# DerekGloudemans/3D-playground

Measured on AMD Instinct MI355X. Metric: training images/sec at 1920x1080, ResNet-50 3D-RetinaNet, higher is better.
Workload: dtype f32; 1 GPU; resnet50 directional 3D-RetinaNet, 1920x1080 synthetic frames, batch 8 per GPU, 10 GT boxes/image, fp32, fwd+loss+bwd+clip+Adam (BASELINE configs[1]); global_batch=8, parallelism=dp1

## Files before the change

3d-playground_amd/csrc/conv_wino.hip:

```cpp
#include "common.h"
#include "mfma_split.h"

__device__ __forceinline__ float4 f4(float s) { return make_float4(s, s, s, s); }
typedef float nt_f4 __attribute__((ext_vector_type(4)));
__device__ __forceinline__ float4 ld_stream(const float *p) {
    const nt_f4 v = __builtin_nontemporal_load(reinterpret_cast<const nt_f4 *>(p));
    return make_float4(v.x, v.y, v.z, v.w);
}
__device__ __forceinline__ void st_stream(float *p, float4 v) { *reinterpret_cast<float4 *>(p) = v; }
__device__ __forceinline__ float4 operator+(float4 a, float4 b) { return make_float4(a.x + b.x, a.y + b.y, a.z + b.z, a.w + b.w); }
__device__ __forceinline__ float4 operator-(float4 a, float4 b) { return make_float4(a.x - b.x, a.y - b.y, a.z - b.z, a.w - b.w); }
__device__ __forceinline__ float4 operator*(float s, float4 a) { return make_float4(s * a.x, s * a.y, s * a.z, s * a.w); }

__device__ __forceinline__ void bt6(const float4 d[6], float4 o[6]) {
    o[0] = 4.f * d[0] - 5.f * d[2] + d[4];
    o[1] = d[3] + d[4] - 4.f * (d[1] + d[2]);
    o[2] = 4.f * (d[1] - d[2]) - d[3] + d[4];
    o[3] = 2.f * (d[3] - d[1]) - d[2] + d[4];
    o[4] = 2.f * (d[1] - d[3]) - d[2] + d[4];
    o[5] = 4.f * d[1] - 5.f * d[3] + d[5];
}
__device__ __forceinline__ void at6(const float4 m[6], float4 o[4]) {
    const float4 s12 = m[1] + m[2], d12 = m[1] - m[2], s34 = m[3] + m[4], d34 = m[3] - m[4];
    o[0] = m[0] + s12 + s34;
    o[1] = d12 + 2.f * d34;
    o[2] = s12 + 4.f * s34;
    o[3] = d12 + 8.f * d34 + m[5];
}


struct WinoProblem { int N, H, W, TH, TW; };
struct WinoTable {
    int n;
    int64_t tile_end[RN_MAX_GROUP];
    WinoProblem p[RN_MAX_GROUP];
    const float *src[RN_MAX_GROUP];
    float *dst[RN_MAX_GROUP];
    const float *add[RN_MAX_GROUP];
    const float *mask[RN_MAX_GROUP];
    unsigned *sign[RN_MAX_GROUP];
    unsigned *amax[RN_MAX_GROUP];
};

#define WINO_GAIN_BT 7
#define WINO_GAIN_A 8
__device__ __forceinline__ void wino_tensor_word(const WinoTable &g, unsigned *tensor_amax, int gain) {
    if (tensor_amax == nullptr || blockIdx.x != 0 || threadIdx.x >= 64) return;
    int e = 0;
#pragma unroll
    for (int i = 0; i < RN_MAX_GROUP; ++i)
        if (i < g.n && g.amax[i] != nullptr) { const int ei = rn_amax_exp_all(g.amax[i], g.p[i].N); e = ei > e ? ei : e; }
    if (threadIdx.x == 0) atomicMax(tensor_amax, rn_amax_word_of_exp(e, gain));
}
__device__ __forceinline__ int wino_locate(const WinoTable &g, int64_t gt, int64_t &local) {
    int q = 0;
#pragma unroll
    for (int i = 0; i < RN_MAX_GROUP - 1; ++i) q += (i + 1 < g.n && gt >= g.tile_end[i]) ? 1 : 0;
    int64_t first = 0;
#pragma unroll
    for (int i = 1; i < RN_MAX_GROUP; ++i)
        if (q == i) first = g.tile_end[i - 1];
    local = gt - first;
    return q;
}

#define WINO_SELECT(q, g, pr, EXTRA)                          \
    WinoProblem pr = g.p[0];                                   \
    _Pragma("unroll") for (int i_ = 1; i_ < RN_MAX_GROUP; ++i_) \
        if (q == i_) { pr = g.p[i_]; EXTRA }

__global__ __launch_bounds__(256) void wino_in_kernel(const WinoTable g, float *__restrict__ V, int C, int64_t t0, int64_t Tpad,
                                                      unsigned *__restrict__ row_amax, unsigned *__restrict__ tensor_amax) {
    wino_tensor_word(g, tensor_amax, WINO_GAIN_BT);
    const int cq = C >> 2;
    const int64_t id = (int64_t)xcd_remap(blockIdx.x, gridDim.x) * 256 + threadIdx.x;
    const int64_t gt_raw = id / cq, t_last = g.tile_end[g.n - 1];
    const int64_t gt = gt_raw < t_last ? gt_raw : t_last - 1;
    const int c4 = (int)(id - gt_raw * cq) * 4;
    int64_t tile;
    const int q = wino_locate(g, gt, tile);
    const float *x = g.src[0];
    const unsigned *xw = g.amax[0];
    WINO_SELECT(q, g, pr, x = g.src[i_]; xw = g.amax[i_];)
    const int H = pr.H, W = pr.W, TW = pr.TW;
    const int n = (int)(tile / (pr.TH * TW));
    const int r = (int)(tile - (int64_t)n * pr.TH * TW);
    const int th = r / TW, tw = r - th * TW;
    const int h0 = 4 * th - 1, w0 = 4 * tw - 1;
    const float *xb = x + (int64_t)n * H * W * C + c4;
    if (row_amax != nullptr) {
        const int e_img = rn_amax_exp_lanes(xw != nullptr ? reinterpret_cast<const unsigned char *>(xw) + (int64_t)n * RN_AMAX_BYTES : nullptr);
        if (gt_raw < t_last && c4 == 0) row_amax[t0 + gt] = rn_amax_word_of_exp(e_img, WINO_GAIN_BT);
    }
    if (gt_raw >= t_last) return;
    float4 t[6][6];
#pragma unroll
    for (int j = 0; j < 6; ++j) {
        float4 d[6], o[6];
        const int w = w0 + j;
#pragma unroll
        for (int i = 0; i < 6; ++i) {
            const int h = h0 + i;
#ifdef RN_WINO_ABL
            const bool ok = (unsigned)h < (unsigned)H && (unsigned)w < (unsigned)W && i >= 1 && i <= 4 && j >= 1 && j <= 4;
#else
            const bool ok = (unsigned)h < (unsigned)H && (unsigned)w < (unsigned)W;
#endif
            d[i] = ok ? *reinterpret_cast<const float4 *>(xb + ((int64_t)h * W + w) * C) : f4(0.f);
        }
        bt6(d, o);
#pragma unroll
        for (int i = 0; i < 6; ++i) t[i][j] = o[i];
    }
    float *vb = V + (t0 + gt) * C + c4;
#pragma unroll
    for (int i = 0; i < 6; ++i) {
        float4 o[6];
        bt6(t[i], o);
#pragma unroll
        for (int j = 0; j < 6; ++j) st_stream(vb + (int64_t)(i * 6 + j) * Tpad * C, o[j]);
    }
}

template <bool PBITS, bool PADD, bool FLAGS = false>
__global__ __launch_bounds__(256, 2) void wino_out_kernel(const WinoTable g, const float *__restrict__ M, int Cout, int64_t t0,
                                                       int64_t Tpad, const float *__restrict__ scale,
                                                       const float *__restrict__ shift, int mask_mode, int act, int64_t y_bs,
                                                       const unsigned char *__restrict__ fin = nullptr,
                                                       unsigned char *__restrict__ fout = nullptr) {
    const int cq = Cout >> 2;
    const int64_t id = (int64_t)blockIdx.x * 256 + threadIdx.x;
    const int64_t gt = id / cq;
    float am = 0.f;
    unsigned *yam = nullptr;
    int n_img = 0;
    bool live = false;
    do {
    if (gt >= g.tile_end[g.n - 1]) break;
    live = true;
    const int c4 = (int)(id - gt * cq) * 4;
    int64_t tile;
    const int q = wino_locate(g, gt, tile);
    float *y = g.dst[0];
    const float *add = g.add[0], *mask = g.mask[0];
    unsigned *sign = g.sign[0];
    yam = g.amax[0];
    WINO_SELECT(q, g, pr, y = g.dst[i_]; add = g.add[i_]; mask = g.mask[i_]; sign = g.sign[i_]; yam = g.amax[i_];)
    n_img = (int)(tile / (pr.TH * pr.TW));
    const bool mbits = (mask_mode & RN_MASK_BITS) != 0;
    mask_mode &= 3;
    const int H = pr.H, W = pr.W, TW = pr.TW;
    const int n = (int)(tile / (pr.TH * TW));
    const int r = (int)(tile - (int64_t)n * pr.TH * TW);
    const int th = r / TW, tw = r - th * TW;
    const float *mb = M + (t0 + gt) * Cout + c4;
    float4 t[4][6];
    bool active = true;
    if constexpr (FLAGS) active = fin == nullptr || fin[t0 + gt] != 0;
    if (active) {
#pragma unroll
        for (int j = 0; j < 6; ++j) {
            float4 m[6], o[4];
#pragma unroll
            for (int i = 0; i < 6; ++i) m[i] = ld_stream(mb + (int64_t)(i * 6 + j) * Tpad * Cout);
            at6(m, o);
#pragma unroll
            for (int i = 0; i < 4; ++i) t[i][j] = o[i];
        }
    } else {
#pragma unroll
        for (int j = 0; j < 6; ++j)
#pragma unroll
            for (int i = 0; i < 4; ++i) t[i][j] = f4(0.f);
    }
    unsigned wake = 0u;
    float4 sc = f4(1.f), sh = f4(0.f);
    if (scale) sc = *reinterpret_cast<const float4 *>(scale + c4);
    if (shift) sh = *reinterpret_cast<const float4 *>(shift + c4);
    const int64_t ybs = y_bs ? y_bs : (int64_t)H * W * Cout;
#pragma unroll
    for (int i = 0; i < 4; ++i) {
        float4 o[4];
        at6(t[i], o);
        const int oh = 4 * th + i;
        if (oh >= H) break;
        unsigned mkw[4];
        float4 adv[4];
        if constexpr (PBITS || PADD) {
#pragma unroll
            for (int j = 0; j < 4; ++j) {
                const int owc = 4 * tw + j < W ? 4 * tw + j : W - 1;
                const int64_t off = (((int64_t)n * H + oh) * W + owc) * Cout + c4;
                if constexpr (PBITS) mkw[j] = reinterpret_cast<const unsigned *>(mask)[off >> 5] >> ((unsigned)off & 28u);
                if constexpr (PADD) adv[j] = *reinterpret_cast<const float4 *>(add + off);
            }
        }
#pragma unroll
        for (int j = 0; j < 4; ++j) {
            const int ow = 4 * tw + j;
            if (ow >= W) break;
            const int64_t off = (((int64_t)n * H + oh) * W + ow) * Cout + c4;
            const int64_t yoff = (int64_t)n * ybs + ((int64_t)oh * W + ow) * Cout + c4;
            float v[4] = {sc.x * o[j].x + sh.x, sc.y * o[j].y + sh.y, sc.z * o[j].z + sh.z, sc.w * o[j].w + sh.w};
            float mk[4] = {1.f, 1.f, 1.f, 1.f}, ad[4] = {0.f, 0.f, 0.f, 0.f};
            if constexpr (PBITS) {
                const unsigned nb = mkw[j];
                mk[0] = (nb & 1u) ? 1.f : 0.f; mk[1] = (nb & 2u) ? 1.f : 0.f; mk[2] = (nb & 4u) ? 1.f : 0.f; mk[3] = (nb & 8u) ? 1.f : 0.f;
            } else if (mask_mode != 0) { const float4 q4 = rn_mask_load4(mask, off, mbits); mk[0] = q4.x; mk[1] = q4.y; mk[2] = q4.z; mk[3] = q4.w; }
            if constexpr (PADD) { const float4 q4 = adv[j]; ad[0] = q4.x; ad[1] = q4.y; ad[2] = q4.z; ad[3] = q4.w; }
            else if (add) { const float4 q4 = *reinterpret_cast<const float4 *>(add + off); ad[0] = q4.x; ad[1] = q4.y; ad[2] = q4.z; ad[3] = q4.w; }
#pragma unroll
            for (int k = 0; k < 4; ++k) {
                float u = v[k];
                if (mask_mode == 1) u = mk[k] > 0.f ? u : 0.f;
                u += ad[k];
                if (act == 1) u = fmaxf(u, 0.f);
                else if (act == 2) u = 1.0f / (1.0f + expf(-u));
                if (mask_mode == 2) u = mk[k] > 0.f ? u : 0.f;
                v[k] = u;
            }
            *reinterpret_cast<float4 *>(y + yoff) = make_float4(v[0], v[1], v[2], v[3]);
            if (sign != nullptr) rn_sign_store(sign, off, v[0], v[1], v[2], v[3]);
            am = fmaxf(fmaxf(am, fmaxf(fabsf(v[0]), fabsf(v[1]))), fmaxf(fabsf(v[2]), fabsf(v[3])));
            if constexpr (FLAGS) {
                if (v[0] != 0.f || v[1] != 0.f || v[2] != 0.f || v[3] != 0.f) {
                    const unsigned rows = 2u | (i == 0 ? 1u : 0u) | (i == 3 ? 4u : 0u);
                    const unsigned cols = 2u | (j == 0 ? 1u : 0u) | (j == 3 ? 4u : 0u);
#pragma unroll
                    for (int a = 0; a < 3; ++a)
                        if (rows & (1u << a)) wake |= cols << (3 * a);
                }
            }
        }
    }
    if constexpr (FLAGS) {
        if (fout != nullptr && wake != 0u) {
#pragma unroll
            for (int a = 0; a < 3; ++a)
#pragma unroll
                for (int b = 0; b < 3; ++b) {
                    const int th2 = th + a - 1, tw2 = tw + b - 1;
                    if ((wake & (1u << (3 * a + b))) && (unsigned)th2 < (unsigned)pr.TH && (unsigned)tw2 < (unsigned)TW)
                        fout[t0 + gt + (int64_t)(a - 1) * TW + (b - 1)] = 1;
                }
        }
    }
    } while (0);
    if (live) rn_amax_note(yam, n_img, am);
}

__global__ void wino_weight_kernel(const float *__restrict__ w, float *__restrict__ U, int Cout, int Cin, int mode,
                                   const float *__restrict__ scale, int rows, int Kpad) {
    const int64_t id = (int64_t)blockIdx.x * 256 + threadIdx.x;
    if (id >= (int64_t)rows * Kpad) return;
    const int row = (int)(id / Kpad), k = (int)(id - (int64_t)row * Kpad);
    const int kdim = mode == 0 ? Cin : Cout;
    float g[3][3];
#pragma unroll
    for (int r = 0; r < 3; ++r)
#pragma unroll
        for (int s = 0; s < 3; ++s) {
            float v = 0.f;
            if (k < kdim) {
                if (mode == 0) v = w[(((int64_t)row * Cin + k) * 3 + r) * 3 + s];
                else v = w[(((int64_t)k * Cin + row) * 3 + (2 - r)) * 3 + (2 - s)] * (scale ? scale[k] : 1.f);
            }
            g[r][s] = v;
        }
    float t[6][3];
#pragma unroll
    for (int s = 0; s < 3; ++s) {
        const float a = g[0][s], b = g[1][s], c = g[2][s];
        t[0][s] = a * (1.f / 4.f);
        t[1][s] = -(a + b + c) * (1.f / 6.f);
        t[2][s] = (b - a - c) * (1.f / 6.f);
        t[3][s] = a * (1.f / 24.f) + b * (1.f / 12.f) + c * (1.f / 6.f);
        t[4][s] = a * (1.f / 24.f) - b * (1.f / 12.f) + c * (1.f / 6.f);
        t[5][s] = c;
    }
#pragma unroll
    for (int i = 0; i < 6; ++i) {
        const float a = t[i][0], b = t[i][1], c = t[i][2];
        const float o[6] = {a * (1.f / 4.f), -(a + b + c) * (1.f / 6.f), (b - a - c) * (1.f / 6.f),
                            a * (1.f / 24.f) + b * (1.f / 12.f) + c * (1.f / 6.f),
                            a * (1.f / 24.f) - b * (1.f / 12.f) + c * (1.f / 6.f), c};
#pragma unroll
        for (int j = 0; j < 6; ++j) U[((int64_t)(i * 6 + j) * rows + row) * Kpad + k] = o[j];
    }
}

__device__ __forceinline__ void a6(const float4 v[4], float4 o[6]) {
    const float4 s02 = v[0] + v[2], s13 = v[1] + v[3];
    o[0] = v[0];
// ... 96 lines not shown
            return;
        }
    }
    float4 t[6][6];
    float4 tz[6][4];
#pragma unroll
    for (int j = 0; j < 6; ++j) {
        float4 d[6], o[6];
        const int w = w0 + j;
#pragma unroll
        for (int i = 0; i < 6; ++i) {
            const int h = h0 + i;
            const bool ok = (unsigned)h < (unsigned)H && (unsigned)w < (unsigned)W;
            d[i] = ok ? *reinterpret_cast<const float4 *>(xb + ((int64_t)h * W + w) * C) : f4(0.f);
        }
        bt6(d, o);
#pragma unroll
        for (int i = 0; i < 6; ++i) t[i][j] = o[i];
        if (j >= 1 && j <= 4) {
            float4 oz[6];
            a6(d + 1, oz);
#pragma unroll
            for (int a = 0; a < 6; ++a) tz[a][j - 1] = oz[a];
        }
    }
    float *zb = Z + (t0 + gt) * C + c4;
#pragma unroll
    for (int a = 0; a < 6; ++a) {
        float4 o[6];
        a6(tz[a], o);
#pragma unroll
        for (int b = 0; b < 6; ++b) st_stream(zb + (int64_t)(a * 6 + b) * Tpad * C, o[b]);
    }
    float *vb = V + (t0 + gt) * C + c4;
#pragma unroll
    for (int i = 0; i < 6; ++i) {
        float4 o[6];
        bt6(t[i], o);
#pragma unroll
        for (int j = 0; j < 6; ++j) st_stream(vb + (int64_t)(i * 6 + j) * Tpad * C, o[j]);
    }
}

__device__ __forceinline__ unsigned nz_bytes(unsigned w) {
    const unsigned t = (w | ((w & 0x7f7f7f7fu) + 0x7f7f7f7fu)) & 0x80808080u;
    return ((t >> 7) & 1u) | ((t >> 14) & 2u) | ((t >> 21) & 4u) | ((t >> 28) & 8u);
}
__global__ __launch_bounds__(256) void tile_lists_kernel(const unsigned char *__restrict__ flags, int Tpad, int *__restrict__ counts,
                                                         int *__restrict__ tiles, int *__restrict__ units, int *__restrict__ blocks) {
    __shared__ unsigned long long wsum[4];
    const int tid = threadIdx.x, lane = tid & 63, wave = tid >> 6;
    const int nb = Tpad >> 7;
    unsigned m[8];
    unsigned long long c = 0ull;
#pragma unroll
    for (int j = 0; j < 8; ++j) m[j] = 0u;
    if (tid < nb) {
        const uint4 *p = reinterpret_cast<const uint4 *>(flags) + 8 * tid;
        int ct = 0, cu = 0;
#pragma unroll
        for (int j = 0; j < 8; ++j) {
            const uint4 v = p[j];
            m[j] = nz_bytes(v.x) | (nz_bytes(v.y) << 4) | (nz_bytes(v.z) << 8) | (nz_bytes(v.w) << 12);
            ct += __builtin_popcount(m[j]);
            cu += m[j] != 0u;
        }
        c = (unsigned long long)ct | ((unsigned long long)cu << 20) | ((unsigned long long)(cu != 0) << 40);
    }
    unsigned long long s = c;
#pragma unroll
    for (int off = 1; off < 64; off <<= 1) {
        const unsigned long long t = __shfl_up(s, off, 64);
        if (lane >= off) s += t;
    }
    if (lane == 63) wsum[wave] = s;
    __syncthreads();
    unsigned long long base = 0ull, total = 0ull;
#pragma unroll
    for (int w = 0; w < 4; ++w) { base += w < wave ? wsum[w] : 0ull; total += wsum[w]; }
    s = s - c + base;
    if (tid == 0) {
        counts[0] = (int)(total & 0xfffffu); counts[1] = (int)((total >> 20) & 0xfffffu); counts[2] = (int)((total >> 40) & 0xfffffu);
    }
    int ot = (int)(s & 0xfffffu), ou = (int)((s >> 20) & 0xfffffu);
    const int ob = (int)((s >> 40) & 0xfffffu);
    if ((c >> 40) != 0ull) blocks[ob] = tid;
#pragma unroll
    for (int j = 0; j < 8; ++j) {
        unsigned mm = m[j];
        if (mm != 0u) units[ou++] = 8 * tid + j;
        while (mm != 0u) {
            tiles[ot++] = 128 * tid + 16 * j + __builtin_ctz(mm);
            mm &= mm - 1u;
        }
    }
}

__global__ void wino_dw_kernel(const float *__restrict__ dU, float *__restrict__ dw, int Cout, int Cin, int Ku, int Kpad) {
    const int64_t id = (int64_t)blockIdx.x * 256 + threadIdx.x;
    if (id >= (int64_t)Cout * Cin) return;
    const int co = (int)(id / Cin), ci = (int)(id - (int64_t)co * Cin);
    const float *u = dU + (int64_t)co * Ku + ci;
    const int64_t ps = (int64_t)Cout * Ku;
    float t[3][6];
#pragma unroll
    for (int j = 0; j < 6; ++j) {
        float v[6];
#pragma unroll
        for (int i = 0; i < 6; ++i) v[i] = u[(i * 6 + j) * ps];
        t[0][j] = v[0] * (1.f / 4.f) - (v[1] + v[2]) * (1.f / 6.f) + (v[3] + v[4]) * (1.f / 24.f);
        t[1][j] = (v[2] - v[1]) * (1.f / 6.f) + (v[3] - v[4]) * (1.f / 12.f);
        t[2][j] = (v[3] + v[4] - v[1] - v[2]) * (1.f / 6.f) + v[5];
    }
    float *o = dw + (int64_t)co * Kpad + ci;
#pragma unroll
    for (int r = 0; r < 3; ++r) {
        const float *v = t[r];
        o[(r * 3 + 0) * Cin] += v[0] * (1.f / 4.f) - (v[1] + v[2]) * (1.f / 6.f) + (v[3] + v[4]) * (1.f / 24.f);
        o[(r * 3 + 1) * Cin] += (v[2] - v[1]) * (1.f / 6.f) + (v[3] - v[4]) * (1.f / 12.f);
        o[(r * 3 + 2) * Cin] += (v[3] + v[4] - v[1] - v[2]) * (1.f / 6.f) + v[5];
    }
}

static int wino_table(const rn_wino_group *g, WinoTable &t) {
    if (!g || g->n < 1 || g->n > RN_MAX_GROUP) return RN_EINVAL;
    t.n = g->n;
    int64_t end = 0;
    for (int i = 0; i < RN_MAX_GROUP; ++i) {
        const int k = i < g->n ? i : g->n - 1;
        if (g->N[k] <= 0 || g->H[k] <= 0 || g->W[k] <= 0) return RN_EINVAL;
        t.p[i].N = g->N[k]; t.p[i].H = g->H[k]; t.p[i].W = g->W[k];
        t.p[i].TH = (g->H[k] + 3) / 4; t.p[i].TW = (g->W[k] + 3) / 4;
        if (i < g->n) end += (int64_t)g->N[k] * t.p[i].TH * t.p[i].TW;
        t.tile_end[i] = end;
        t.src[i] = g->src[k]; t.dst[i] = g->dst[k]; t.add[i] = g->add[k]; t.mask[i] = g->mask[k];
        t.sign[i] = reinterpret_cast<unsigned *>(g->sign[k]);
        t.amax[i] = reinterpret_cast<unsigned *>(g->amax[k]);
    }
    return RN_OK;
}

extern "C" int rn_wino_input_group(const rn_wino_group *g, float *V, int C, int64_t tile_offset, int64_t Tpad, int dy_form,
                                   void *row_amax, void *tensor_amax, void *stream) {
    WinoTable t;
    const int rc = wino_table(g, t);
    if (rc) return rc;
    if (C <= 0 || (C & 3) || tile_offset < 0 || tile_offset + t.tile_end[t.n - 1] > Tpad) return RN_EINVAL;
    for (int i = 0; i < t.n; ++i)
        if (!t.src[i]) return RN_EINVAL;
    const dim3 grid(rn_blocks(t.tile_end[t.n - 1] * (C >> 2), 256));
    if (dy_form && row_amax != nullptr) return RN_EINVAL;
    if (dy_form) hipLaunchKernelGGL(wino_dy_kernel, grid, dim3(256), 0, (hipStream_t)stream, t, V, C, tile_offset, Tpad,
                                    reinterpret_cast<unsigned *>(tensor_amax));
    else hipLaunchKernelGGL(wino_in_kernel, grid, dim3(256), 0, (hipStream_t)stream, t, V, C, tile_offset, Tpad,
                            reinterpret_cast<unsigned *>(row_amax), reinterpret_cast<unsigned *>(tensor_amax));
    RN_LAUNCH_CHECK();
    return RN_OK;
}

extern "C" int rn_wino_input_both_group_flags(const rn_wino_group *g, float *V, float *Z, int C, int64_t tile_offset, int64_t Tpad,
                                              void *v_row_amax, void *z_tensor_amax, const void *flags, void *stream) {
    WinoTable t;
    const int rc = wino_table(g, t);
    if (rc) return rc;
    if (!V || !Z || C <= 0 || (C & 3) || tile_offset < 0 || tile_offset + t.tile_end[t.n - 1] > Tpad) return RN_EINVAL;
    if (flags != nullptr && (((uintptr_t)flags & 15) || (Tpad & 15))) return RN_EINVAL;
    for (int i = 0; i < t.n; ++i)
        if (!t.src[i]) return RN_EINVAL;
    const dim3 grid(rn_blocks(t.tile_end[t.n - 1] * (C >> 2), 256));
    if (flags != nullptr)
        hipLaunchKernelGGL(wino_in_both_kernel<true>, grid, dim3(256), 0, (hipStream_t)stream, t, V, Z, C, tile_offset, Tpad,
                           reinterpret_cast<unsigned *>(v_row_amax), reinterpret_cast<unsigned *>(z_tensor_amax),
                           reinterpret_cast<const unsigned char *>(flags));
    else
        hipLaunchKernelGGL(wino_in_both_kernel<false>, grid, dim3(256), 0, (hipStream_t)stream, t, V, Z, C, tile_offset, Tpad,
                           reinterpret_cast<unsigned *>(v_row_amax), reinterpret_cast<unsigned *>(z_tensor_amax),
                           (const unsigned char *)nullptr);
    RN_LAUNCH_CHECK();
    return RN_OK;
}
extern "C" int rn_tile_lists(const void *flags, int64_t Tpad, void *counts, void *tiles, void *units, void *blocks, void *stream) {
    if (!flags || !counts || !tiles || !units || !blocks || Tpad <= 0 || (Tpad & 255) || Tpad > 256 * 128) return RN_EINVAL;
    if (((uintptr_t)flags & 15) || (((uintptr_t)counts | (uintptr_t)tiles | (uintptr_t)units | (uintptr_t)blocks) & 3)) return RN_EINVAL;
    hipLaunchKernelGGL(tile_lists_kernel, dim3(1), dim3(256), 0, (hipStream_t)stream, reinterpret_cast<const unsigned char *>(flags), (int)Tpad,
                       reinterpret_cast<int *>(counts), reinterpret_cast<int *>(tiles), reinterpret_cast<int *>(units),
                       reinterpret_cast<int *>(blocks));
    RN_LAUNCH_CHECK();
    return RN_OK;
}

extern "C" int rn_wino_input_both_group_lists(const rn_wino_group *g, float *V, float *Z, int C, int64_t tile_offset, int64_t Tpad,
                                              void *v_row_amax, void *z_tensor_amax, const void *flags, const void *units,
                                              const void *n_units, void *stream) {
    WinoTable t;
    const int rc = wino_table(g, t);
    if (rc) return rc;
    if (!V || !Z || C <= 0 || (C & 3) || tile_offset < 0 || tile_offset + t.tile_end[t.n - 1] > Tpad) return RN_EINVAL;
    if (!flags || !units || !n_units || ((uintptr_t)flags & 15) || ((uintptr_t)units & 3) || (Tpad & 15)) return RN_EINVAL;
    for (int i = 0; i < t.n; ++i)
        if (!t.src[i]) return RN_EINVAL;
    const dim3 gl(rn_blocks(t.tile_end[t.n - 1] * (C >> 2), 256));
    hipLaunchKernelGGL((wino_in_both_kernel<true, true>), gl, dim3(256), 0, (hipStream_t)stream, t, V, Z, C, tile_offset, Tpad,
                       reinterpret_cast<unsigned *>(v_row_amax), reinterpret_cast<unsigned *>(z_tensor_amax),
                       reinterpret_cast<const unsigned char *>(flags), reinterpret_cast<const int *>(units),
                       reinterpret_cast<const int *>(n_units));
    RN_LAUNCH_CHECK();
    return RN_OK;
}

extern "C" int rn_wino_input_both_group(const rn_wino_group *g, float *V, float *Z, int C, int64_t tile_offset, int64_t Tpad,
                                        void *v_row_amax, void *z_tensor_amax, void *stream) {
    return rn_wino_input_both_group_flags(g, V, Z, C, tile_offset, Tpad, v_row_amax, z_tensor_amax, nullptr, stream);
}

extern "C" int rn_wino_output_group_flags(const rn_wino_group *g, const float *M, int Cout, int64_t tile_offset, int64_t Tpad,
                                          const float *scale, const float *shift, int mask_mode, int act, int64_t y_batch_stride,
                                          const void *flags_in, void *flags_out, void *stream) {
    WinoTable t;
    const int rc = wino_table(g, t);
    if (rc) return rc;
    if (Cout <= 0 || (Cout & 3) || tile_offset < 0 || tile_offset + t.tile_end[t.n - 1] > Tpad) return RN_EINVAL;
    if (mask_mode < 0 || (mask_mode & ~(3 | RN_MASK_BITS)) || (mask_mode & 3) == 3 || mask_mode == RN_MASK_BITS) return RN_EINVAL;
    if (act < 0 || act > 2 || y_batch_stride < 0 || (y_batch_stride & 3)) return RN_EINVAL;
    for (int i = 0; i < t.n; ++i) {
        if (!t.dst[i] || (mask_mode != 0) != (t.mask[i] != nullptr)) return RN_EINVAL;
        if (((mask_mode & RN_MASK_BITS) || t.sign[i]) && (Cout & 31)) return RN_EINVAL;
        if (y_batch_stride && y_batch_stride < (int64_t)t.p[i].H * t.p[i].W * Cout) return RN_EINVAL;
    }
    const bool pbits = (mask_mode & RN_MASK_BITS) != 0;
    bool padd = true;
    for (int i = 0; i < t.n; ++i) padd = padd && t.add[i] != nullptr;
    const dim3 grid(rn_blocks(t.tile_end[t.n - 1] * (Cout >> 2), 256));
    const unsigned char *fin = reinterpret_cast<const unsigned char *>(flags_in);
    unsigned char *fout = reinterpret_cast<unsigned char *>(flags_out);
#define RN_WINO_OUT(B, A, F) hipLaunchKernelGGL((wino_out_kernel<B, A, F>), grid, dim3(256), 0, (hipStream_t)stream, t, M, Cout, tile_offset, Tpad, \
                                                scale, shift, mask_mode, act, y_batch_stride, fin, fout)
    if (fin != nullptr || fout != nullptr) {
        if (pbits && padd) RN_WINO_OUT(true, true, true);
        else if (pbits) RN_WINO_OUT(true, false, true);
        else if (padd) RN_WINO_OUT(false, true, true);
        else RN_WINO_OUT(false, false, true);
    } else if (pbits && padd) RN_WINO_OUT(true, true, false);
    else if (pbits) RN_WINO_OUT(true, false, false);
    else if (padd) RN_WINO_OUT(false, true, false);
    else RN_WINO_OUT(false, false, false);
#undef RN_WINO_OUT
    RN_LAUNCH_CHECK();
    return RN_OK;
}
extern "C" int rn_wino_output_group(const rn_wino_group *g, const float *M, int Cout, int64_t tile_offset, int64_t Tpad,
                                    const float *scale, const float *shift, int mask_mode, int act, int64_t y_batch_stride,
                                    void *stream) {
    return rn_wino_output_group_flags(g, M, Cout, tile_offset, Tpad, scale, shift, mask_mode, act, y_batch_stride, nullptr, nullptr, stream);
}

static rn_wino_group wino_single(const float *src, float *dst, const float *add, const float *mask, int N, int H, int W) {
    rn_wino_group g = {};
    g.n = 1; g.N[0] = N; g.H[0] = H; g.W[0] = W; g.src[0] = src; g.dst[0] = dst; g.add[0] = add; g.mask[0] = mask;
    return g;
}
extern "C" int rn_wino_input(const float *x, float *V, int N, int H, int W, int C, int64_t tile_offset, int64_t Tpad,
                             void *stream) {
    const rn_wino_group g = wino_single(x, nullptr, nullptr, nullptr, N, H, W);
    return rn_wino_input_group(&g, V, C, tile_offset, Tpad, 0, nullptr, nullptr, stream);
}
extern "C" int rn_wino_dy(const float *dy, float *Z, int N, int H, int W, int C, int64_t tile_offset, int64_t Tpad, void *stream) {
    const rn_wino_group g = wino_single(dy, nullptr, nullptr, nullptr, N, H, W);
    return rn_wino_input_group(&g, Z, C, tile_offset, Tpad, 1, nullptr, nullptr, stream);
}
extern "C" int rn_wino_output(const float *M, float *y, int N, int H, int W, int Cout, int64_t tile_offset, int64_t Tpad,
                              const float *scale, const float *shift, const float *add, const float *mask, int mask_mode,
                              int act, int64_t y_batch_stride, void *stream) {
    const rn_wino_group g = wino_single(nullptr, y, add, mask, N, H, W);
    return rn_wino_output_group(&g, M, Cout, tile_offset, Tpad, scale, shift, mask_mode, act, y_batch_stride, stream);
}

extern "C" int rn_wino_weights(const float *w, float *U, int Cout, int Cin, int mode, const float *scale, void *stream) {
    if (Cout <= 0 || Cin <= 0 || mode < 0 || mode > 1) return RN_EINVAL;
    const int rows = mode == 0 ? Cout : Cin;
    const int Kpad = ((mode == 0 ? Cin : Cout) + 31) / 32 * 32;
    hipLaunchKernelGGL(wino_weight_kernel, dim3(rn_blocks((int64_t)rows * Kpad, 256)), dim3(256), 0, (hipStream_t)stream, w, U,
                       Cout, Cin, mode, scale, rows, Kpad);
    RN_LAUNCH_CHECK();
    return RN_OK;
}

extern "C" int rn_wino_dw(const float *dU, float *dw, int Cout, int Cin, void *stream) {
    if (Cout <= 0 || Cin <= 0) return RN_EINVAL;
    const int Ku = (Cin + 31) / 32 * 32, Kpad = (9 * Cin + 31) / 32 * 32;
    hipLaunchKernelGGL(wino_dw_kernel, dim3(rn_blocks((int64_t)Cout * Cin, 256)), dim3(256), 0, (hipStream_t)stream, dU, dw, Cout,
                       Cin, Ku, Kpad);
    RN_LAUNCH_CHECK();
    return RN_OK;
}
```

3d-playground_amd/csrc/focal_loss.hip:

```cpp
#include <math.h>
#include <stdlib.h>

#include "common.h"

#ifndef FOCAL_NTHR
#define FOCAL_NTHR 256
#endif
#define NTHR FOCAL_NTHR
#define APT 4
#define TILE (NTHR * APT)
#define NWAVES (NTHR / 64)
#define UAPT 2
#define UNIT (64 * UAPT)
#define QCAP 256
#ifndef RN_FOCAL_WAVES_PER_SIMD
#define RN_FOCAL_WAVES_PER_SIMD 4
#endif
#define RN_FOCAL_WAVES_NOTE 4
#define RN_FOCAL_RESIDENT 768

static inline int focal_resident() {
    static const int v = [] { const char *e = getenv("RN_FOCAL_RESIDENT"); const int x = e ? atoi(e) : 0; return x >= 8 ? x : RN_FOCAL_RESIDENT; }();
    return v;
}
// ... 664 lines not shown
            un = u + stride;
            issue(un < units ? un : u, avA, xvA);
            process(u, avB, xvB);
            u = un;
            if (u >= units || qn > QCAP - UNIT) break;
        }
        drain();
    }
    if (!BWD) {
        sums[0] += (-0.75f * RN_LN2) * (neg2.x + neg2.y);
        block_sum4<NWAVES>(sums, s_red);
        if (threadIdx.x == 0) {
            unsigned long long *p64 = reinterpret_cast<unsigned long long *>(partials) + 2 * ((int64_t)j * G + g);
            const unsigned long long lo = ((unsigned long long)__float_as_uint(sums[1]) << 32) | __float_as_uint(sums[0]);
            const unsigned long long hi = ((unsigned long long)__float_as_uint(sums[3]) << 32) | __float_as_uint(sums[2]);
            (void)__hip_atomic_exchange(p64, lo, __ATOMIC_RELAXED, __HIP_MEMORY_SCOPE_AGENT);
            (void)__hip_atomic_exchange(p64 + 1, hi, __ATOMIC_RELAXED, __HIP_MEMORY_SCOPE_AGENT);
            asm volatile("s_waitcnt vmcnt(0)" ::: "memory");
            s_last = atomicAdd(counter + RN_WS_HEAD / 4 + j, 1u) == (unsigned)G - 1;
        }
        __syncthreads();
        if (s_last) {
            double *s_red = reinterpret_cast<double *>(&s_q[0][0][0]);
            const int B = (int)(gridDim.x / G);
            focal_finalize_image<DIR>(reinterpret_cast<const float4 *>(partials), G, j, ann, N, terms, s_red);
            if (threadIdx.x == 0) {
                __hip_atomic_store(counter + RN_WS_HEAD / 4 + j, 0u, __ATOMIC_RELAXED, __HIP_MEMORY_SCOPE_AGENT);
                s_last = atomicAdd(counter, 1u) == (unsigned)B - 1;
            }
            __syncthreads();
            if (s_last) {
                focal_finalize_batch<DIR>(B, terms, stats, losses, s_red, s_red + NWAVES * 4);
                if (threadIdx.x == 0) __hip_atomic_store(counter, 0u, __ATOMIC_RELAXED, __HIP_MEMORY_SCOPE_AGENT);
            }
        }
    }
}

static int check_args(int B, int64_t A, int C, int N) {
    if (B <= 0 || A <= 0 || C <= 0 || N < 0) return RN_EINVAL;
    if (N > RN_MAX_GT) return RN_ETOOMANY;
    if (B > 1024) return RN_EINVAL;
    if (A > 0x7fffffffLL) return RN_EINVAL;
    return RN_OK;
}

struct FocalWs {
    unsigned *counter;
    ImageStats *stats;
    double *terms;
    float *partials;
};
static inline FocalWs focal_ws(void *workspace, int B) {
    char *w = reinterpret_cast<char *>(workspace);
    FocalWs r;
    r.counter = reinterpret_cast<unsigned *>(w);
    const size_t head = RN_WS_HEAD + (size_t)focal_counter_bytes(B);
    r.stats = reinterpret_cast<ImageStats *>(w + head);
    r.terms = reinterpret_cast<double *>(w + head + (size_t)B * sizeof(ImageStats));
    r.partials = reinterpret_cast<float *>(w + head + (size_t)B * sizeof(ImageStats) + (size_t)B * RN_TERMS * sizeof(double));
    return r;
}

extern "C" int rn_focal_loss_fwd(const float *cls, const float *reg, const float *anchors, const float *ann, int B,
                                 int64_t A, int C, int N, int directional, void *workspace, float *losses,
                                 void *stream) {
    const int rc = check_args(B, A, C, N);
    if (rc) return rc;
    hipStream_t s = (hipStream_t)stream;
    const int G = focal_groups(B, A);
    const int units = (int)((A + UNIT - 1) / UNIT);
    const FocalWs ws = focal_ws(workspace, B);
    const dim3 grid((unsigned)(B * G)), block(NTHR);
    const float4 *anc = reinterpret_cast<const float4 *>(anchors);
    const int cq = C == 4 ? 1 : (C == 8 ? 2 : 0);
    const size_t raw_bytes = (size_t)(N > 0 ? N : 1) * (directional ? 27 : 5) * sizeof(float);
#define RN_FOCAL_FWD(DIR_, CQ_)                                                                                        \
    hipLaunchKernelGGL((focal_kernel<DIR_, false, CQ_>), grid, block, raw_bytes, s, cls, reg, anc, ann, A, C, N,        \
                       ws.partials, ws.stats, (float *)nullptr, (float *)nullptr, G, units, ws.counter, ws.terms, losses, \
                       (const float *)nullptr)
    if (directional) {
        if (cq == 2) RN_FOCAL_FWD(true, 2); else if (cq == 1) RN_FOCAL_FWD(true, 1); else RN_FOCAL_FWD(true, 0);
    } else {
        if (cq == 2) RN_FOCAL_FWD(false, 2); else if (cq == 1) RN_FOCAL_FWD(false, 1); else RN_FOCAL_FWD(false, 0);
    }
#undef RN_FOCAL_FWD
    RN_LAUNCH_CHECK();
    return RN_OK;
}

extern "C" int rn_focal_loss_bwd(const float *cls, const float *reg, const float *anchors, const float *ann, int B,
                                 int64_t A, int C, int N, int directional, const void *workspace,
                                 const float *grad_losses, float *dcls, float *dreg, void *stream) {
    const int rc = check_args(B, A, C, N);
    if (rc) return rc;
    hipStream_t s = (hipStream_t)stream;
    const int G = focal_groups(B, A);
    const int units = (int)((A + UNIT - 1) / UNIT);
    const FocalWs ws = focal_ws(const_cast<void *>(workspace), B);
    const dim3 grid((unsigned)(B * G)), block(NTHR);
    const float4 *anc = reinterpret_cast<const float4 *>(anchors);
    const int cq = C == 4 ? 1 : (C == 8 ? 2 : 0);
    const size_t raw_bytes = (size_t)(N > 0 ? N : 1) * (directional ? 27 : 5) * sizeof(float);
#define RN_FOCAL_BWD(DIR_, CQ_)                                                                                      \
    hipLaunchKernelGGL((focal_kernel<DIR_, true, CQ_>), grid, block, raw_bytes, s, cls, reg, anc, ann, A, C, N,       \
                       (float *)nullptr, ws.stats, dcls, dreg, G, units, (unsigned *)nullptr, (double *)nullptr,      \
                       (float *)nullptr, grad_losses)
    if (directional) {
        if (cq == 2) RN_FOCAL_BWD(true, 2); else if (cq == 1) RN_FOCAL_BWD(true, 1); else RN_FOCAL_BWD(true, 0);
    } else {
        if (cq == 2) RN_FOCAL_BWD(false, 2); else if (cq == 1) RN_FOCAL_BWD(false, 1); else RN_FOCAL_BWD(false, 0);
    }
#undef RN_FOCAL_BWD
    RN_LAUNCH_CHECK();
    return RN_OK;
}

template <bool DIR>
__global__ __launch_bounds__(NTHR) void assign_kernel(const float4 *__restrict__ anchors, const float *__restrict__ ann,
                                                      int64_t A, int N, float *__restrict__ iou_max,
                                                      int32_t *__restrict__ argmax, int32_t *__restrict__ state) {
    constexpr int COLS = DIR ? 27 : 5;
    __shared__ LabelLds L;
    const int j = blockIdx.y;
    load_labels<DIR>(ann + (int64_t)j * N * COLS, N, L);
    const int64_t ai = (int64_t)blockIdx.x * NTHR + threadIdx.x;
    if (ai >= A) return;
    float best = 0.f; int arg = -1; int st = 0;
    if (L.count > 0) {
        match_anchor(anchors[ai], L, best, arg);
        st = -1;
        if (best < 0.4f) st = 0;
        if (best >= 0.5f) st = 1;
    }
    iou_max[(int64_t)j * A + ai] = best;
    argmax[(int64_t)j * A + ai] = arg;
    state[(int64_t)j * A + ai] = st;
}

extern "C" int rn_assign(const float *anchors, const float *ann, int B, int64_t A, int N, int directional,
                         float *iou_max, int32_t *argmax, int32_t *state, void *stream) {
    const int rc = check_args(B, A, 1, N);
    if (rc) return rc;
    const dim3 grid((unsigned)((A + NTHR - 1) / NTHR), B), block(NTHR);
    const float4 *anc = reinterpret_cast<const float4 *>(anchors);
    if (directional)
        hipLaunchKernelGGL(assign_kernel<true>, grid, block, 0, (hipStream_t)stream, anc, ann, A, N, iou_max, argmax, state);
    else
        hipLaunchKernelGGL(assign_kernel<false>, grid, block, 0, (hipStream_t)stream, anc, ann, A, N, iou_max, argmax, state);
    RN_LAUNCH_CHECK();
    return RN_OK;
}

__global__ void pairwise_iou_kernel(const float4 *__restrict__ a, const float4 *__restrict__ b, float *__restrict__ out,
                                    int64_t A, int N) {
    const int64_t i = (int64_t)blockIdx.x * 256 + threadIdx.x;
    if (i >= A * N) return;
    const int64_t ai = i / N;
    const int n = (int)(i - ai * N);
    const float4 p = a[ai], q = b[n];
    const float area_b = (q.z - q.x) * (q.w - q.y);
    float iw = fminf(p.z, q.z) - fmaxf(p.x, q.x);
    float ih = fminf(p.w, q.w) - fmaxf(p.y, q.y);
    iw = fmaxf(iw, 0.f);
    ih = fmaxf(ih, 0.f);
    float ua = ((p.z - p.x) * (p.w - p.y) + area_b) - iw * ih;
    ua = fmaxf(ua, 1e-8f);
    out[i] = (iw * ih) / ua;
}

extern "C" int rn_pairwise_iou(const float *a, const float *b, float *iou, int64_t A, int N, void *stream) {
    if (A <= 0 || N <= 0) return RN_EINVAL;
    hipLaunchKernelGGL(pairwise_iou_kernel, dim3(rn_blocks(A * N, 256)), dim3(256), 0, (hipStream_t)stream,
                       reinterpret_cast<const float4 *>(a), reinterpret_cast<const float4 *>(b), iou, A, N);
    RN_LAUNCH_CHECK();
    return RN_OK;
}
```

3d-playground_amd/retinanet_mi355x/_hip.py:

```python
import ctypes
import os

import torch

_HERE = os.path.dirname(os.path.abspath(__file__))
LIB_PATH = os.environ.get("RN_LIB_PATH") or os.path.join(_HERE, "lib", "libretinanet_mi355x.so")
_lib = None

c_i32, c_i64, c_f32, c_f64, c_vp = ctypes.c_int, ctypes.c_int64, ctypes.c_float, ctypes.c_double, ctypes.c_void_p

SIGNATURES = {
    "rn_version": (ctypes.c_char_p, []),
    "rn_check_device": (c_i32, []),
    "rn_get_fp32_mfma": (c_i32, []),
    "rn_set_fp32_mfma": (c_i32, [c_i32]),
    "rn_get_option": (c_i32, [c_i32]),
    "rn_set_option": (c_i32, [c_i32, c_i32]),
    "rn_fp32_split_min_k": (c_i32, []),
    "rn_split_weights": (c_i32, [c_vp, c_vp, c_i64, c_i32, c_vp]),
    "rn_split_weights_f16": (c_i32, [c_vp, c_vp, c_vp, c_i64, c_i32, c_vp]),
    "rn_amax": (c_i32, [c_vp, c_i64, c_i32, c_vp, c_vp]),
    "rn_stream_capture_id": (c_i32, [c_vp, ctypes.POINTER(ctypes.c_ulonglong)]),
    "rn_anchor_count": (c_i64, [c_i32, c_i32]),
    "rn_anchor_base_boxes": (None, [c_vp]),
# ... 16 lines not shown
    "rn_space_to_state": (c_i32, [c_vp, c_vp, c_i64, c_vp]),
    "rn_state_to_im": (c_i32, [c_vp, c_vp, c_vp, c_vp, c_vp, c_i64, c_vp]),
    "rn_space_to_im": (c_i32, [c_vp, c_vp, c_vp, c_vp, c_vp, c_i64, c_vp]),
    "rn_im_to_space": (c_i32, [c_vp, c_vp, c_vp, c_vp, c_vp, c_vp, c_i64, c_vp]),
    "rn_im_to_state": (c_i32, [c_vp, c_vp, c_vp, c_vp, c_vp, c_vp, c_i64, c_vp]),
    "rn_parse_workspace_bytes": (c_i64, [c_i64]),
    "rn_parse_detections": (c_i32, [c_vp, c_vp, c_vp, c_vp, c_i64, c_vp, c_vp, c_vp, c_vp, c_i32, c_vp, c_f32, c_f32, c_f32,
                                    c_i32, c_i32, c_vp, c_vp, c_vp, c_vp, c_vp, c_vp, c_vp]),
    "rn_md_iou": (c_i32, [c_vp, c_vp, c_vp, c_i64, c_vp]),
    "rn_crop_boxes": (c_i32, [c_vp, c_vp, c_i32, c_f64, c_vp, c_vp, c_vp]),
    "rn_roi_align": (c_i32, [c_vp, c_i32, c_i32, c_i32, c_i32, c_vp, c_i32, c_i32, c_i32, c_vp, c_i32, c_vp]),
    "rn_crop_select": (c_i32, [c_vp] * 9 + [c_i32] * 4 + [c_f64, c_i32, c_f32, c_vp, c_vp, c_vp, c_vp]),
    "rn_kf_view": (c_i32, [c_vp, c_vp, c_vp, c_vp, c_i32, c_i32, c_vp, c_i32, c_vp]),
    "rn_kf_predict": (c_i32, [c_vp, c_vp, c_vp, c_vp, c_vp, c_vp, c_vp, c_i32, c_f64, c_i32, c_vp]),
    "rn_kf_update": (c_i32, [c_vp, c_vp, c_vp, c_vp, c_vp, c_vp, c_vp, c_i32, c_vp]),
    "rn_track_cost": (c_i32, [c_vp, c_i64, c_vp, c_i64, c_i64, c_i64, c_vp, c_vp]),
    "rn_lsap_workspace_bytes": (c_i64, [c_i64, c_i64]),
    "rn_linear_sum_assignment": (c_i32, [c_vp, c_i64, c_i64, c_f64, c_vp, c_vp, c_vp, c_vp, c_vp]),
    "rn_ts_bias_workspace_bytes": (c_i64, [c_i64, c_i64]),
    "rn_estimate_ts_bias": (c_i32, [c_vp, c_i64, c_vp, c_i64, c_vp, c_vp, c_i64, c_i64, c_vp, c_vp, c_i32, c_f64, c_f64, c_f32,
                                    c_vp, c_i64, c_vp, c_vp, c_vp, c_vp]),
    "rn_track_crop_prior": (c_i32, [c_vp] * 7 + [c_i32, c_vp, c_vp, c_vp, c_i32, c_vp]),
    "rn_fit_nearest": (c_i32, [c_vp, c_vp, c_vp, c_i64, c_i64, c_vp, c_vp, c_vp, c_vp]),
    "rn_residual_moments": (c_i32, [c_vp, c_i64, c_i32, c_vp, c_i32, c_vp, c_vp, c_vp, c_vp]),
    "rn_eval_select": (c_i32, [c_vp, c_vp, c_vp, c_i64, c_i64, c_i64, c_f32, c_i32, c_i32, c_i64, c_i32, c_vp, c_i64, c_vp, c_vp, c_vp]),
    "rn_eval_match": (c_i32, [c_vp, c_i64, c_vp, c_i64, c_i32, c_vp, c_vp, c_i64, c_f64, c_vp, c_vp, c_vp, c_vp]),
    "rn_eval_ap_workspace_bytes": (c_i64, [c_i64]),
    "rn_eval_ap": (c_i32, [c_vp, c_i64, c_vp, c_vp, c_vp, c_i32, c_vp, c_vp, c_vp, c_vp]),
    "rn_eval_corners": (c_i32, [c_vp, c_i64, c_i64, c_i32, c_i64, c_vp, c_vp, c_i64, c_vp, c_vp]),
    "rn_eval_cuboid_overlap": (c_i32, [c_vp, c_i64, c_vp, c_i64, c_i32, c_vp, c_vp, c_vp, c_i64, c_i32, c_vp, c_vp, c_vp]),
    "rn_eval_cuboid_assign": (c_i32, [c_vp, c_i64, c_vp, c_i64, c_i32, c_vp, c_i64, c_vp, c_vp, c_vp, c_i32, c_vp, c_vp, c_vp,
                                      c_vp, c_vp]),
    "rn_eval_cuboid_errors": (c_i32, [c_vp, c_i64, c_vp, c_i64, c_i32, c_vp, c_vp, c_vp, c_i64, c_vp, c_vp, c_vp, c_vp, c_vp,
                                      c_vp]),
    "rn_frame_ingest": (c_i32, [c_vp, c_i32, c_i32, c_i32, c_i32] + [c_f32] * 6 + [c_i32, c_vp, c_vp]),
    "rn_frame_ingest_half": (c_i32, [c_vp, c_i32, c_i32, c_i32, c_i32] + [c_f32] * 6 + [c_i32, c_vp, c_vp, c_vp]),
    "rn_parse_frame_timestamps": (c_i32, [c_vp, c_i32, c_i32, c_i32, c_i64, c_i64, c_i32, c_vp, c_i32] + [c_vp] * 9),
    "rn_augment_workspace_bytes": (c_i64, [c_i32, c_i32, c_i32]),
    "rn_augment_frames": (c_i32, [c_vp, c_i32, c_i32, c_i32, c_vp, c_vp, c_vp, c_vp, ctypes.c_uint64] + [c_f32] * 6 + [c_vp, c_vp, c_vp]),
    "rn_augment_crops_workspace_bytes": (c_i64, [c_i32, c_i32, c_i32]),
    "rn_augment_crops": (c_i32, [c_vp, c_i32, c_i32, c_i32, c_vp, c_vp, c_vp, c_vp, c_vp, c_i32, c_i32, c_i32, c_vp, c_vp, ctypes.c_uint64]
                         + [c_f32] * 6 + [c_vp, c_vp, c_vp]),
    "rn_mot_prepare": (c_i32, [c_vp, c_vp, c_vp, c_i64, c_vp, c_i64] + [c_vp] * 7),
    "rn_mot_iou": (c_i32, [c_vp] * 5 + [c_i64, c_i64, c_vp, c_vp]),
    "rn_mot_assign": (c_i32, [c_vp] * 5 + [c_i64] * 4 + [c_vp] * 5),
    "rn_mot_frame_metrics": (c_i32, [c_vp] * 5 + [c_i64, c_i64, c_vp, c_vp, c_vp, c_f64] + [c_vp] * 19),
    "rn_mot_workspace_bytes": (c_i64, [c_i64, c_i64]),
    "rn_mot_reduce": (c_i32, [c_i64, c_i64] + [c_vp] * 16 + [c_i64, c_i64, c_vp, c_vp, c_vp]),
    "rn_mot_assoc_workspace_bytes": (c_i64, [c_i64, c_i64]),
    "rn_mot_id_counts": (c_i32, [c_vp] * 5 + [c_i64] * 6 + [c_vp, c_vp, c_i64, c_i64, c_f64] + [c_vp] * 5),
    "rn_mot_id_assign": (c_i32, [c_vp, c_i64, c_i64, c_vp, c_vp, c_vp, c_vp]),
    "rn_mot_hota_align": (c_i32, [c_vp] * 5 + [c_i64] * 6 + [c_vp] * 5 + [c_i64] * 3 + [c_vp] * 5),
    "rn_mot_hota_assign": (c_i32, [c_vp] * 5 + [c_i64] * 6 + [c_vp, c_vp, c_i64, c_i64] + [c_vp] * 11),
    "rn_mot_hota_reduce": (c_i32, [c_vp] * 4 + [c_i64] * 6 + [c_vp] * 9 + [c_i64, c_i64, c_vp, c_vp, c_vp]),
    "rn_vanishing_points": (c_i32, [c_vp, c_i64, c_vp, c_i64, c_vp, c_vp, c_vp, c_vp]),
    "rn_hg_reproj_error": (c_i32, [c_vp, c_vp, c_vp, c_vp, c_vp, c_i64, c_i64, c_vp, c_vp]),
    "rn_hg_scale_z": (c_i32, [c_vp, c_vp, c_vp, c_vp, c_i64, c_f64, c_f64, c_i32, c_vp, c_vp, c_vp, c_vp]),
    "rn_fit_homography": (c_i32, [c_vp, c_vp, c_i64, c_vp, c_i64, c_i32, c_vp, c_vp, c_vp]),
    "rn_reinterp_mate": (c_i32, [c_vp, c_vp, c_i64, c_i64, c_vp, c_vp, c_vp]),
    "rn_reinterp_offsets": (c_i32, [c_vp, c_vp, c_i64, c_i64, c_vp, c_i64] + [c_vp] * 5),
    "rn_reinterp_rows": (c_i32, [c_vp] * 7 + [c_i64] * 4 + [c_vp] * 5),
    "rn_track_rows": (c_i32, [c_vp] * 5 + [c_i64, c_i64] + [c_vp] * 7),
    "rn_render_edges": (c_i32, [c_vp, c_vp, c_i64, c_i32, c_i32, c_vp, c_i32, c_i32, c_i32, c_vp]),
    "rn_render_rects": (c_i32, [c_vp, c_i64, c_vp, c_i64, c_vp, c_i32, c_i32, c_i32, c_vp]),
    "rn_render_text": (c_i32, [c_vp, c_i64, c_vp, c_i64, c_vp, c_vp, c_i64, c_vp, c_i32, c_i32, c_i32, c_vp]),
    "rn_render_compose": (c_i32, [c_vp] + [c_f32] * 6 + [c_vp, c_i32, c_vp, c_i32, c_i32, c_i32, c_i32, c_vp]),
    "rn_replay_boxes": (c_i32, [c_vp, c_i64, c_vp, c_vp, c_vp, c_i32, c_vp, c_vp, c_vp, c_vp, c_vp]),
    "rn_replay_compose": (c_i32, [c_vp, c_i32, c_vp, c_vp] + [c_i32] * 6 + [c_vp]),
    "rn_frame_absdiff": (c_i32, [c_vp, c_vp] + [c_i32] * 6 + [c_vp, c_vp, c_vp]),
    "rn_running_frame": (c_i32, [c_vp, c_vp, c_i64, c_i32, c_vp]),
    "rn_label_pair_samples": (c_i32, [c_vp, c_vp, c_i64, c_i32, c_i64, c_i32, c_i32, c_i32, c_vp, c_vp, c_vp, c_vp]),
    "rn_label_outliers": (c_i32, [c_vp, c_vp, c_vp, c_i64, c_i64, c_i64, c_i64, c_vp, c_vp, c_vp]),
    "rn_label_interpolate_workspace_bytes": (c_i64, [c_i64, c_i64]),
    "rn_label_interpolate": (c_i32, [c_vp] * 4 + [c_i64] * 3 + [c_i32, c_i64] + [c_vp] * 7),
    "rn_label_rebase": (c_i32, [c_vp, c_vp, c_i64] + [c_vp] * 4 + [c_i32, c_vp, c_i32, c_i32] + [c_vp] * 5),
    "rn_label_offset_y": (c_i32, [c_vp] * 4 + [c_i64, c_i32, c_vp, c_vp]),
    "rn_label_crop_windows": (c_i32, [c_vp, c_vp, c_i64, c_vp, c_vp, c_i32, c_f32, c_f32, c_f32] + [c_vp] * 6),
    "rn_label_best_anchor": (c_i32, [c_vp, c_vp, c_vp, c_i64, c_i32, c_i32, c_f32] + [c_vp] * 5),
    "rn_label_fit_box2d": (c_i32, [c_vp] * 5 + [c_i64, c_vp, c_vp, c_i32, c_vp, c_i32, c_i32] + [c_vp] * 5),
    "rn_spline_fit_workspace_bytes": (c_i64, [c_i64, c_i32]),
    "rn_label_box_weights": (c_i32, [c_vp, c_vp, c_i64, c_vp, c_vp, c_i32, c_vp, c_vp, c_vp]),
    "rn_spline_fit": (c_i32, [c_vp, c_i64, c_vp, c_i64, c_vp, c_vp, c_vp, c_i64, c_vp, c_i64, c_i32] + [c_vp] * 7),
    "rn_spline_select": (c_i32, [c_vp, c_i64] + [c_vp] * 4 + [c_i64, c_i64, c_i64, c_i32] + [c_vp] * 4 + [c_i32] + [c_vp] * 7),
    "rn_spline_eval": (c_i32, [c_vp, c_vp, c_vp, c_i64, c_i32, c_vp, c_vp, c_i64, c_vp, c_vp]),
    "rn_label_ts_shift": (c_i32, [c_vp, c_vp, c_vp, c_i64, c_i32, c_vp, c_vp, c_vp, c_i64, c_i64, c_vp, c_vp, c_vp, c_i32, c_i32,
                                  c_i32] + [c_vp] * 5),
    "rn_label_series_workspace_bytes": (c_i64, [c_i64]),
    "rn_label_series": (c_i32, [c_vp, c_vp, c_i64, c_i32, c_i64, c_i32, c_f64, c_f64, c_i32] + [c_vp] * 8),
    "rn_label_group_rmse": (c_i32, [c_vp, c_vp, c_i64, c_i64] + [c_vp] * 5),
    "rn_stitch_endpoints": (c_i32, [c_vp, c_vp, c_vp, c_i64, c_i64, c_i32, c_vp, c_vp, c_vp]),
    "rn_stitch_costs": (c_i32, [c_vp, c_i64] + [c_f64] * 7 + [c_vp, c_vp]),
    "rn_stitch_candidates": (c_i32, [c_vp, c_i64] + [c_f64] * 7 + [c_vp] * 4),
    "rn_stitch_compact": (c_i32, [c_vp, c_i64] + [c_f64] * 7 + [c_vp, c_vp, c_i64, c_vp, c_vp, c_vp]),
    "rn_stitch_assign_workspace_bytes": (c_i64, [c_i64]),
    "rn_stitch_assign": (c_i32, [c_vp, c_i64] + [c_f64] * 7 + [c_vp, c_vp, c_vp, c_i64] + [c_vp] * 6),
    "rn_stitch_chains": (c_i32, [c_vp, c_vp, c_i64] + [c_vp] * 6),
    "rn_stitch_fill_count": (c_i32, [c_vp, c_vp, c_i64, c_f64] + [c_vp] * 4),
    "rn_stitch_fill_rows": (c_i32, [c_vp, c_vp, c_vp, c_i64, c_i64, c_f64] + [c_vp] * 6),
    "rn_smooth_filter": (c_i32, [c_vp] * 5 + [c_f64, c_f64, c_i64, c_i64] + [c_vp] * 5),
    "rn_smooth_rts": (c_i32, [c_vp] * 5 + [c_f64, c_i64, c_i64] + [c_vp] * 4),
}

class ConvDesc(ctypes.Structure):
    _fields_ = [("N", c_i32), ("Hi", c_i32), ("Wi", c_i32), ("Cin", c_i32),
                ("Ho", c_i32), ("Wo", c_i32), ("Cout", c_i32),
                ("kh", c_i32), ("kw", c_i32),
                ("a", c_i32), ("b", c_i32), ("p", c_i32), ("p_w", c_i32), ("div_shift", c_i32),
                ("act", c_i32), ("add_mode", c_i32), ("Ha", c_i32), ("Wa", c_i32),
                ("mask_mode", c_i32), ("in_relu", c_i32),
                ("os", c_i32), ("oo_h", c_i32), ("oo_w", c_i32), ("Hy", c_i32), ("Wy", c_i32),
                ("add2_mode", c_i32), ("Ha2", c_i32), ("Wa2", c_i32), ("add2_batch_stride", c_i64),
                ("x_batch_stride", c_i64), ("y_batch_stride", c_i64), ("add_batch_stride", c_i64),
                ("w_batch_stride", c_i64), ("w_format", c_i32), ("sign_out", c_vp),
                ("x_amax", c_vp), ("y_amax", c_vp), ("w_unscale", c_vp), ("x_amax_img_stride", c_i32), ("x_amax_row_stride", c_i32),
                ("row_active", c_vp), ("row_list", c_vp), ("row_list_n", c_vp), ("row_list_grid", c_i32)]


RN_MAX_GROUP = 5


class ConvGroup(ctypes.Structure):
    _fields_ = [("n", c_i32), ("tile_end", c_i32 * RN_MAX_GROUP), ("d", ConvDesc * RN_MAX_GROUP),
                ("x", c_vp * RN_MAX_GROUP), ("y", c_vp * RN_MAX_GROUP), ("add", c_vp * RN_MAX_GROUP),
                ("mask", c_vp * RN_MAX_GROUP)]


class PrepJob(ctypes.Structure):
    _fields_ = [("kind", c_i32)] + [(n, c_i32) for n in ("Cout", "Cin", "kh", "kw", "kw_pad", "c_pad", "mode", "r0", "nr", "s0",
                                                          "ns", "rows", "Kpad")] + \
               [("eps", c_f32), ("src", c_vp), ("dst", c_vp), ("scale", c_vp), ("gamma", c_vp), ("beta", c_vp), ("mean", c_vp),
                ("var", c_vp), ("bn_scale", c_vp), ("bn_shift", c_vp), ("bn_rstd", c_vp)]


class UnpackJob(ctypes.Structure):
    _fields_ = [("dw", c_vp), ("w_packed", c_vp), ("dweight", c_vp)] + \
               [(n, c_i32) for n in ("Cout", "Cin", "kh", "kw", "kw_pad", "c_pad", "Kpad")] + \
               [("scale", c_vp), ("mean", c_vp), ("rstd", c_vp), ("colsum", c_vp), ("dgamma", c_vp), ("dbeta", c_vp)]


class WinoGroup(ctypes.Structure):
    _fields_ = [("n", c_i32), ("N", c_i32 * RN_MAX_GROUP), ("H", c_i32 * RN_MAX_GROUP), ("W", c_i32 * RN_MAX_GROUP),
                ("src", c_vp * RN_MAX_GROUP), ("dst", c_vp * RN_MAX_GROUP), ("add", c_vp * RN_MAX_GROUP),
                ("mask", c_vp * RN_MAX_GROUP), ("sign", c_vp * RN_MAX_GROUP), ("amax", c_vp * RN_MAX_GROUP)]


SIGNATURES.update({
    "rn_unpack_batched": (c_i32, [c_vp, c_vp, c_i32, c_vp]),
    "rn_prep_batched": (c_i32, [c_vp, c_vp, c_i32, c_vp]),
    "rn_wino_input_group": (c_i32, [ctypes.POINTER(WinoGroup), c_vp, c_i32, c_i64, c_i64, c_i32, c_vp, c_vp, c_vp]),
    "rn_wino_input_both_group": (c_i32, [ctypes.POINTER(WinoGroup), c_vp, c_vp, c_i32, c_i64, c_i64, c_vp, c_vp, c_vp]),
    "rn_wino_input_both_group_flags": (c_i32, [ctypes.POINTER(WinoGroup), c_vp, c_vp, c_i32, c_i64, c_i64, c_vp, c_vp, c_vp, c_vp]),
    "rn_tile_lists": (c_i32, [c_vp, c_i64, c_vp, c_vp, c_vp, c_vp, c_vp]),
    "rn_wino_input_both_group_lists": (c_i32, [ctypes.POINTER(WinoGroup), c_vp, c_vp, c_i32, c_i64, c_i64, c_vp, c_vp, c_vp, c_vp, c_vp, c_vp]),
    "rn_wino_output_group_flags": (c_i32, [ctypes.POINTER(WinoGroup), c_vp, c_i32, c_i64, c_i64, c_vp, c_vp, c_i32, c_i32, c_i64, c_vp, c_vp, c_vp]),
    "rn_wino_output_group": (c_i32, [ctypes.POINTER(WinoGroup), c_vp, c_i32, c_i64, c_i64, c_vp, c_vp, c_i32, c_i32, c_i64, c_vp]),
    "rn_conv_igemm_grouped": (c_i32, [ctypes.POINTER(ConvGroup), c_vp, c_vp, c_vp, c_vp]),
    "rn_conv_igemm": (c_i32, [ctypes.POINTER(ConvDesc), c_vp, c_vp, c_vp, c_vp, c_vp, c_vp, c_vp, c_vp, c_vp]),
    "rn_conv_splitk_workspace_bytes": (c_i64, [ctypes.POINTER(ConvDesc)]),
    "rn_conv_igemm_wants_f16": (c_i32, [ctypes.POINTER(ConvDesc)]),
    "rn_conv_igemm_splitk": (c_i32, [ctypes.POINTER(ConvDesc)] + [c_vp] * 10),
    "rn_conv_wgrad": (c_i32, [c_vp, c_i32, c_vp, c_vp, c_vp] + [c_i32] * 12 + [c_vp]),
    "rn_pack_weights": (c_i32, [c_vp, c_vp] + [c_i32] * 7 + [c_vp] + [c_i32] * 4 + [c_vp]),
    "rn_unpack_wgrad": (c_i32, [c_vp, c_vp, c_vp] + [c_i32] * 6 + [c_vp] * 7),
    "rn_bn_fold": (c_i32, [c_vp, c_vp, c_vp, c_vp, c_f32, c_i32, c_vp, c_vp, c_vp, c_vp]),
    "rn_nchw_to_nhwc4": (c_i32, [c_vp, c_vp, c_i32, c_i32, c_i32, c_vp, c_vp]),
    "rn_maxpool_fwd": (c_i32, [c_vp, c_vp, c_vp] + [c_i32] * 6 + [c_vp]),
    "rn_maxpool_bwd": (c_i32, [c_vp, c_vp, c_vp, c_vp] + [c_i32] * 7 + [c_vp, c_vp]),
    "rn_colsum": (c_i32, [c_vp, c_i64, c_i32, c_i32, c_vp, c_i32, c_vp, c_vp]),
    "rn_colsum_workspace_bytes": (c_i64, [c_i64, c_i32]),
    "rn_upsample_add_bwd": (c_i32, [c_vp, c_vp] + [c_i32] * 6 + [c_vp, c_vp]),
    "rn_relu_mask": (c_i32, [c_vp, c_vp, c_i64, c_vp]),
    "rn_sigmoid_bwd_pad": (c_i32, [c_vp, c_vp, c_vp, c_i32, c_i64, c_i32, c_i32, c_i64, c_vp, c_vp]),
    "rn_sigmoid_bwd_pad_flags": (c_i32, [c_vp, c_vp, c_vp, c_i32, c_i32, c_i32, c_i32, c_i32, c_i64, c_vp, c_vp, c_vp]),
    "rn_add_inplace": (c_i32, [c_vp, c_vp, c_i64, c_i64, c_vp, c_vp]),
    "rn_wino_input": (c_i32, [c_vp, c_vp, c_i32, c_i32, c_i32, c_i32, c_i64, c_i64, c_vp]),
    "rn_wino_output": (c_i32, [c_vp, c_vp, c_i32, c_i32, c_i32, c_i32, c_i64, c_i64, c_vp, c_vp, c_vp, c_vp, c_i32, c_i32, c_i64, c_vp]),
    "rn_wino_weights": (c_i32, [c_vp, c_vp, c_i32, c_i32, c_i32, c_vp, c_vp]),
    "rn_wino_dy": (c_i32, [c_vp, c_vp, c_i32, c_i32, c_i32, c_i32, c_i64, c_i64, c_vp]),
    "rn_wino_dw": (c_i32, [c_vp, c_vp, c_i32, c_i32, c_vp]),
    "rn_conv_wgrad_batched": (c_i32, [c_vp, c_i32, c_vp, c_vp, c_vp, c_i32, c_i64, c_i64, c_i64, c_i32] + [c_i32] * 12 + [c_vp, c_i32, c_vp, c_i32, c_vp]),
    "rn_conv_wgrad_batched_det": (c_i32, [c_vp, c_i32, c_vp, c_vp, c_vp, c_i32, c_i64, c_i64, c_i64, c_i32] + [c_i32] * 12 + [c_vp, c_i32, c_vp, c_i32, c_vp, c_i64, c_vp]),
    "rn_conv_wgrad_batched_flags": (c_i32, [c_vp, c_i32, c_vp, c_vp, c_vp, c_i32, c_i64, c_i64, c_i64, c_i32] + [c_i32] * 12 + [c_vp, c_i32, c_vp, c_i32, c_vp, c_vp, c_i64, c_vp]),
    "rn_conv_wgrad_det_workspace_bytes": (c_i64, [c_i32, c_i32, c_i64] + [c_i32] * 9),
    "rn_conv_wgrad_plan": (c_i32, [c_i32, c_i32, c_i64, c_i64, c_i64, c_i32] + [c_i32] * 12 + [c_i32, c_i32, c_i32, c_vp]),
    "rn_f32_to_bf16": (c_i32, [c_vp, c_vp, c_i64, c_vp]),
    "rn_bf16_to_f32": (c_i32, [c_vp, c_vp, c_i64, c_vp]),
    "rn_conv_igemm_bf16": (c_i32, [ctypes.POINTER(ConvDesc), c_vp, c_vp, c_vp, c_i32, c_vp, c_vp, c_vp, c_vp, c_vp]),
    "rn_conv_igemm_bf16_grouped": (c_i32, [ctypes.POINTER(ConvGroup), c_vp, c_i32, c_vp, c_vp, c_vp]),
    "rn_conv_igemm_bf16_tile_rows": (c_i32, [ctypes.POINTER(ConvGroup), c_i32]),
    "rn_maxpool_fwd_fp8out": (c_i32, [c_vp, c_vp] + [c_i32] * 6 + [c_f32, c_vp]),
    "rn_conv_igemm_fp8_tile_rows": (c_i32, [ctypes.POINTER(ConvGroup), c_i32]),
    "rn_conv_igemm_fp8_tile": (c_i32, [ctypes.POINTER(ConvDesc), c_i32]),
    "rn_conv_igemm_bf16_tile": (c_i32, [ctypes.POINTER(ConvDesc), c_i32]),
    "rn_fp8_quantize": (c_i32, [c_vp, c_vp, c_i64, c_f32, c_vp]),
    "rn_fp8_dequantize": (c_i32, [c_vp, c_vp, c_i64, c_f32, c_vp]),
    "rn_fp8_to_bf16": (c_i32, [c_vp, c_vp, c_i64, c_f32, c_vp]),
    "rn_bf16_to_fp8": (c_i32, [c_vp, c_vp, c_i64, c_f32, c_vp]),
    "rn_fp8_quantize_rows": (c_i32, [c_vp, c_vp, c_vp, c_i64, c_i32, c_vp]),
    "rn_conv_igemm_fp8": (c_i32, [ctypes.POINTER(ConvDesc), c_vp, c_vp, c_vp, c_i32, c_vp, c_vp, c_vp, c_f32, c_f32, c_vp]),
    "rn_conv_igemm_fp8_grouped": (c_i32, [ctypes.POINTER(ConvGroup), c_vp, c_i32, c_vp, c_vp, c_f32, c_f32, c_vp]),
    "rn_conv_wgrad_bf16": (c_i32, [c_vp, c_i32, c_vp, c_vp, c_vp] + [c_i32] * 11 + [c_vp]),
    "rn_conv_wgrad_bf16_grouped": (c_i32, [c_i32, ctypes.POINTER(c_vp), c_i32, ctypes.POINTER(c_vp), c_vp, c_vp, c_i32,
                                           ctypes.POINTER(c_i32), ctypes.POINTER(c_i32)] + [c_i32] * 6 + [c_vp]),
    "rn_maxpool_fwd_bf16out": (c_i32, [c_vp, c_vp, c_vp] + [c_i32] * 6 + [c_vp]),
    "rn_maxpool_bwd_bf16in": (c_i32, [c_vp, c_vp, c_vp, c_vp] + [c_i32] * 7 + [c_vp]),
    "rn_upsample_add_bwd_bf16": (c_i32, [c_vp, c_vp] + [c_i32] * 6 + [c_vp]),
    "rn_sigmoid_bwd_pad_bf16": (c_i32, [c_vp, c_vp, c_vp, c_i32, c_i64, c_i32, c_i32, c_i64, c_vp]),
    "rn_relu_bf16": (c_i32, [c_vp, c_vp, c_i64, c_vp]),
    "rn_opt_workspace_bytes": (c_i64, [c_i32]),
    "rn_opt_clip_adam": (c_i32, [c_vp, c_vp, c_i32, c_f32, c_f32, c_f32, c_f32, c_f32, c_i32, c_i32, c_vp, c_vp, c_vp]),
    "rn_opt_clip_adam_dev": (c_i32, [c_vp, c_vp, c_i32, c_f32, c_f32, c_f32, c_f32, c_f32, c_vp, c_i32, c_vp, c_vp, c_vp]),
    "rn_opt_clip_adam_hp": (c_i32, [c_vp, c_vp, c_i32, c_vp, c_vp, c_i32, c_vp, c_vp, c_vp]),
})


RN_ERRORS = {10001: "RN_EINVAL (bad size / unsupported shape)",
             10002: "RN_ETOOMANY (more than RN_MAX_GT=256 label rows per image)"}


def load():
    global _lib
    if _lib is None:
        if not os.path.exists(LIB_PATH):
            raise RuntimeError(
                "libretinanet_mi355x.so is missing (%s): build it with `python -c 'import __graft_entry__ as g; "
                "g.build()'` or `make -C 3d-playground_amd/csrc`.  There is no CPU fallback." % LIB_PATH)
        lib = ctypes.CDLL(LIB_PATH)
        for name, (res, args) in SIGNATURES.items():
            fn = getattr(lib, name)
            fn.restype = res
            fn.argtypes = args
        _lib = lib
    return _lib


def check(rc, what):
    if rc != 0:
        raise RuntimeError("%s failed: %s" % (what, RN_ERRORS.get(rc, "hipError_t %d" % rc)))


def need_gpu(*tensors):
    for t in tensors:
        if t is not None and not t.is_cuda:
            raise RuntimeError("retinanet_mi355x ops run on an MI355X only: got a %s tensor (no CPU fallback)" % t.device)


def ptr(t):
    return None if t is None else t.data_ptr()


def stream():
    return torch.cuda.current_stream().cuda_stream


def call(name, *args, device=None):
    fn = getattr(load(), name)
    args = [a.data_ptr() if isinstance(a, torch.Tensor) else a for a in args]
    if device is None:
        return check(fn(*args, stream()), name)
    with torch.cuda.device(device):
        check(fn(*args, stream()), name)


def f32c(t):
    if t.dtype != torch.float32:
        t = t.float()
    return t if t.is_contiguous() else t.contiguous()
```

3d-playground_amd/retinanet_mi355x/conv.py:

```python
import ctypes
import os

import torch

from . import _hip, prof

ConvDesc = _hip.ConvDesc

ACT_NONE, ACT_RELU, ACT_SIGMOID = 0, 1, 2


def kpad(kh, kw, c):
    return (kh * kw * c + 31) // 32 * 32


def out_size(n, k, stride, pad):
    return (n + 2 * pad - k) // stride + 1


def pack_weights(weight, mode=0, scale=None, kw_pad=None, c_pad=None, taps=None, presplit=True):
    lib = _hip.load()
    w = _hip.f32c(weight.detach())
    _hip.need_gpu(w, scale)
    cout, cin, kh, kw = w.shape
# ... 199 lines not shown
    cid = ctypes.c_ulonglong(0)
    _hip.check(_hip.load().rn_stream_capture_id(stream, ctypes.byref(cid)), "rn_stream_capture_id")
    return cid.value


def _amax_chunk_key(device):
    stream = torch.cuda.current_stream(device).cuda_stream
    return (device, stream, capture_id(stream) if stream else 0)


def _amax_alloc(device, nwords):
    key = _amax_chunk_key(device)
    nwords = (nwords + 7) // 8 * 8
    c = _AMAX_CHUNK.get(key)
    if c is None:
        for k in [k for k in _AMAX_CHUNK if k[:2] == key[:2] and k[2] not in (0, key[2])]:
            del _AMAX_CHUNK[k]
    if c is None or c[1] + nwords > c[0].numel():
        c = _AMAX_CHUNK[key] = [torch.zeros(max(1 << 18, nwords), dtype=torch.int32, device=device), 0]
    c[1] += nwords
    return c[0][c[1] - nwords:c[1]]


def amax_slot(device, n=1):
    return _amax_alloc(device, n * AMAX_SUB)


def amax_single(device):
    return _amax_alloc(device, 1)[:1]


def amax_attach(t, words):
    t._rn_amax = (words, t._version)
    return words


def amax_words(t):
    a = getattr(t, "_rn_amax", None)
    if a is not None and a[1] == t._version and a[0].numel() == t.shape[0] * AMAX_SUB:
        return a[0]
    assert t.is_contiguous() and t.dtype == torch.float32
    words = amax_slot(t.device, t.shape[0])
    if t.numel():
        _hip.check(_hip.load().rn_amax(t.data_ptr(), t.numel() // t.shape[0], t.shape[0], words.data_ptr(), _hip.stream()), "rn_amax")
    return amax_attach(t, words)


def amax_carry(view, src):
    w = getattr(src, "_rn_amax_words", None)
    if w is not None and w.numel() == view.shape[0] * AMAX_SUB:
        amax_attach(view, w)
    return view


def amax_drop(t):
    if hasattr(t, "_rn_amax"):
        del t._rn_amax


def want_amax():
    return get_fp32_mfma() == "split3"


OPT_SPLITK, OPT_DETERMINISTIC, OPT_MF16, OPT_MF16_MIN, OPT_WGRAD_ONCE, OPT_BF16_P8, OPT_FP8_P8 = range(7)


def set_option(option, value):
    _hip.check(_hip.load().rn_set_option(option, int(value)), "rn_set_option")


def get_option(option):
    return int(_hip.load().rn_get_option(option))


def set_deterministic(on=True):
    set_option(OPT_DETERMINISTIC, on)


def _wgrad_call(lib, dev, dy_ptr, ldy, x_ptr, dw_ptr, cs_ptr, nbatch, dy_bs, x_bs, dw_bs, cs_batch, geom, amax=(None, None), flags=None):
    cnt = lambda a: 0 if a is None else (-1 if a.numel() == 1 else a.numel() // AMAX_SUB)
    am = (_hip.ptr(amax[0]), cnt(amax[0]), _hip.ptr(amax[1]), cnt(amax[1]))
    if flags is not None:
        ws, nb = None, 0
        if lib.rn_get_option(OPT_DETERMINISTIC):
            N, Hi, Wi, Cin, Ho, Wo, Cout, kh, kw = geom[:9]
            nb = lib.rn_conv_wgrad_det_workspace_bytes(ldy, nbatch, dw_bs, N, Hi, Wi, Cin, Ho, Wo, Cout, kh, kw)
            if nb < 0:
                return 1
            ws = torch.empty(nb, dtype=torch.uint8, device=dev)
        return lib.rn_conv_wgrad_batched_flags(dy_ptr, ldy, x_ptr, dw_ptr, cs_ptr, nbatch, dy_bs, x_bs, dw_bs, cs_batch, *geom, *am,
                                               flags.data_ptr(), _hip.ptr(ws), nb, _hip.stream())
    if not lib.rn_get_option(OPT_DETERMINISTIC):
        return lib.rn_conv_wgrad_batched(dy_ptr, ldy, x_ptr, dw_ptr, cs_ptr, nbatch, dy_bs, x_bs, dw_bs, cs_batch, *geom, *am, _hip.stream())
    N, Hi, Wi, Cin, Ho, Wo, Cout, kh, kw = geom[:9]
    nb = lib.rn_conv_wgrad_det_workspace_bytes(ldy, nbatch, dw_bs, N, Hi, Wi, Cin, Ho, Wo, Cout, kh, kw)
    if nb < 0:
        return 1
    ws = torch.empty(nb, dtype=torch.uint8, device=dev)
    return lib.rn_conv_wgrad_batched_det(dy_ptr, ldy, x_ptr, dw_ptr, cs_ptr, nbatch, dy_bs, x_bs, dw_bs, cs_batch, *geom, *am,
                                         ws.data_ptr(), nb, _hip.stream())


WGRAD_PLAN_FIELDS = ("shape", "tiles", "splits", "per_split", "xcd_map", "grid", "kernel", "arith")


def wgrad_plan(ldy, nbatch, dy_bs, x_bs, dw_bs, cs_batch, geom, have_amax=False, have_flags=False, det=None):
    out = (ctypes.c_int32 * 8)()
    det = get_option(OPT_DETERMINISTIC) if det is None else det
    rc = _hip.load().rn_conv_wgrad_plan(ldy, nbatch, dy_bs, x_bs, dw_bs, cs_batch, *geom, int(have_amax), int(have_flags), int(det), out)
    return dict(zip(WGRAD_PLAN_FIELDS, out)) if rc == 0 else None


def wino_weights(weight, mode=0, scale=None):
    lib = _hip.load()
    w = _hip.f32c(weight.detach())
    _hip.need_gpu(w, scale)
    cout, cin, kh, kw = w.shape
    assert kh == 3 and kw == 3
    rows, k = (cout, cin) if mode == 0 else (cin, cout)
    U = torch.empty((36, rows, (k + 31) // 32 * 32), dtype=torch.float32, device=w.device)
    _hip.check(lib.rn_wino_weights(w.data_ptr(), U.data_ptr(), cout, cin, mode, _hip.ptr(scale), _hip.stream()),
               "rn_wino_weights")
    return _maybe_split(U, rows=rows, cin=U.shape[2], taps=1)


_WINO_WS = {}
_WINO_ODD_PLANES = os.environ.get("RN_WINO_ODD_PLANES", "1") != "0"


def wino_tpad(T):
    n = (T + 255) // 256
    if _WINO_ODD_PLANES and n % 2 == 0:
        n += 1
    return n * 256


def _wino_group(xs, srcs=None, dsts=None, adds=None, masks=None, mask_bits=False, signs=None, amaxs=None):
    g = _hip.WinoGroup()
    g.n = len(xs)
    for i, x in enumerate(xs):
        g.N[i], g.H[i], g.W[i] = x.shape[0], x.shape[1], x.shape[2]
        g.src[i] = None if srcs is None else srcs[i].data_ptr()
        g.dst[i] = None if dsts is None else dsts[i].data_ptr()
        g.add[i] = None if adds is None or adds[i] is None else adds[i].data_ptr()
        if masks is None or masks[i] is None:
            g.mask[i] = None
        else:
            g.mask[i] = masks[i]._rn_sign.data_ptr() if mask_bits else masks[i].data_ptr()
        g.sign[i] = None if signs is None or signs[i] is None else signs[i].data_ptr()
        g.amax[i] = None if amaxs is None or amaxs[i] is None else amaxs[i].data_ptr()
    return g


def _wino_transform_in(xs, V, C, Tpad, dy_form, want_rows=False, want_tensor=False):
    lib = _hip.load()
    off = 0
    am = want_amax() and (want_rows or want_tensor)
    rows = torch.zeros(Tpad, dtype=torch.int32, device=V.device) if am and want_rows else None
    tword = amax_single(V.device) if am and want_tensor else None
    for k in range(0, len(xs), _hip.RN_MAX_GROUP):
        part = xs[k:k + _hip.RN_MAX_GROUP]
        t = sum(x.shape[0] * ((x.shape[1] + 3) // 4) * ((x.shape[2] + 3) // 4) for x in part)
        g = _wino_group(part, srcs=part, amaxs=[amax_words(x) for x in part] if am else None)
        nb = 4.0 * (sum(x.numel() for x in part) + 36 * t * C)
        _hip.check(prof.timed("wino_input", nb, lambda: lib.rn_wino_input_group(
            ctypes.byref(g), V.data_ptr(), C, off, Tpad, dy_form, _hip.ptr(rows), _hip.ptr(tword), _hip.stream())), "rn_wino_input_group")
        off += t
    return rows, tword


def _wino_workspace(device, floats_v, floats_m):
    key = (device, torch.cuda.current_stream(device).cuda_stream)
    ws = _WINO_WS.get(key)
    if ws is None or ws[0].numel() < floats_v or ws[1].numel() < floats_m:
        ws = (torch.empty(max(floats_v, ws[0].numel() if ws else 0), dtype=torch.float32, device=device),
              torch.empty(max(floats_m, ws[1].numel() if ws else 0), dtype=torch.float32, device=device))
        _WINO_WS[key] = ws
    return ws


def tile_flags(device, T):
    return torch.zeros(wino_tpad(T), dtype=torch.uint8, device=device)


class TileLists:
    __slots__ = ("flags", "buf", "counts", "tiles", "units", "blocks", "grid")

    def lengths(self):
        return tuple(int(v) for v in self.counts[:3].tolist())


def tile_lists_numel(Tpad):
    return 4 + Tpad + Tpad // 16 + Tpad // 128


def tile_lists(flags, Tpad=None, buf=None, grid=0):
    lib = _hip.load()
    Tpad = flags.numel() if Tpad is None else Tpad
    assert flags.dtype == torch.uint8 and flags.numel() >= Tpad and Tpad % 256 == 0
    n = tile_lists_numel(Tpad)
    if buf is None:
        buf = torch.empty(n, dtype=torch.int32, device=flags.device)
    assert buf.dtype == torch.int32 and buf.numel() >= n and buf.is_contiguous()
    tl = TileLists()
    tl.flags, tl.buf, tl.grid = flags, buf, int(grid)
    nb, nu = Tpad // 128, Tpad // 16
    tl.counts, tl.blocks, tl.units, tl.tiles = buf[:4], buf[4:4 + nb], buf[4 + nb:4 + nb + nu], buf[4 + nb + nu:n]
    _hip.check(lib.rn_tile_lists(flags.data_ptr(), Tpad, tl.counts.data_ptr(), tl.tiles.data_ptr(), tl.units.data_ptr(),
                                 tl.blocks.data_ptr(), _hip.stream()), "rn_tile_lists")
    return tl


def wino_flags_ok(T, C, cout):
    lib = _hip.load()
    return bool(get_fp32_mfma() != "native" and lib.rn_get_option(OPT_WGRAD_ONCE) and C > 64 and cout > 64 and T < 32000)


def wino_conv_group(xs, U, outs=None, scale=None, shift=None, act=ACT_NONE, adds=None, masks=None, mask_mode=2,
                    flops=0.0, keep_v=False, y_batch_stride=0, V_in=None, V_ready=None, sign=False, flags_out=None):
    lib = _hip.load()
    dev = xs[0].device
    C = xs[0].shape[3]
    cout = U.shape[1]
    tiles = [x.shape[0] * ((x.shape[1] + 3) // 4) * ((x.shape[2] + 3) // 4) for x in xs]
    T = sum(tiles)
    Tpad = wino_tpad(T)
    V, M = _wino_workspace(dev, 0 if keep_v else 36 * Tpad * C, 36 * Tpad * cout)
    shapes = tuple(tuple(x.shape) for x in xs)
    reuse = keep_v and V_in is not None and V_in[1] == shapes and V_in[0].numel() == 36 * Tpad * C
    ready = not keep_v and isinstance(V_ready, tuple) and V_ready[1] == shapes and V_ready[0].numel() >= 36 * Tpad * C
    if ready:
        V, reuse = V_ready[0], True
    elif reuse:
        V = V_in[0]
    elif keep_v:
        V = torch.empty(36 * Tpad * C, dtype=torch.float32, device=dev)
    assert all(x.is_contiguous() for x in xs)
    v_am = (None, None)
    if reuse:
        src = V_ready if ready else V_in
        v_am = src[2] if len(src) > 2 and src[2] is not None else (None, None)
    else:
        v_am = _wino_transform_in(xs, V, C, Tpad, 0, want_rows=True, want_tensor=keep_v)
    flags = V_ready[3] if ready and len(V_ready) > 3 else None
    lists = V_ready[4] if ready and len(V_ready) > 4 else None
    if flags_out is not None:
        assert flags_out.dtype == torch.uint8 and flags_out.numel() >= Tpad and len(xs) <= _hip.RN_MAX_GROUP
    Vv = V[:36 * Tpad * C].view(36, 1, Tpad, C)
    Mv = M[:36 * Tpad * cout].view(36, 1, Tpad, cout)
    Uv = _carry_split(U, U.view(36 * cout, U.shape[2]))
    if want_amax() and v_am[0] is None:
        Uv = U.view(36 * cout, U.shape[2])
    conv_igemm(Vv, Uv, Mv, (1, Tpad, cout, 1, 1, 1, 1, 0, 0), flops=2.0 * 36 * T * cout * C, w_batch_stride=cout * U.shape[2],
               x_amax=v_am[0], x_amax_rows=True, row_active=flags, row_list=lists)
    if outs is None:
        outs = [torch.empty((x.shape[0], x.shape[1], x.shape[2], cout), dtype=torch.float32, device=dev) for x in xs]
    off = 0
    for k in range(0, len(xs), _hip.RN_MAX_GROUP):
        sl = slice(k, k + _hip.RN_MAX_GROUP)
        part, t = xs[sl], sum(tiles[sl])
        pa = None if adds is None else adds[sl]
        pm = None if masks is None else masks[sl]
        has_mask = pm is not None and pm[0] is not None
        mbits = has_mask and BITMASKS and all(getattr(m, "_rn_sign", None) is not None for m in pm)
        for o in outs[sl]:
            amax_drop(o)
        signs = [_sign_words(o, sign and not y_batch_stride) for o in outs[sl]]
        yams = [amax_slot(dev, o.shape[0]) for o in outs[sl]] if want_amax() and not y_batch_stride else None
        g = _wino_group(part, dsts=outs[sl], adds=pa, masks=pm, mask_bits=mbits, signs=signs, amaxs=yams)
        nops = 1 + (pa is not None and pa[0] is not None) + (1.0 / 32 if mbits else 1.0) * has_mask + (1.0 / 32 if signs[0] is not None else 0.0)
        nb = 4.0 * (36 * t * cout + nops * sum(x.shape[0] * x.shape[1] * x.shape[2] for x in part) * cout)
        mm = (mask_mode | (MASK_BITS if mbits else 0)) if has_mask else 0
        if flags is not None or flags_out is not None:
            _hip.check(prof.timed("wino_output", nb, lambda: lib.rn_wino_output_group_flags(
                ctypes.byref(g), M.data_ptr(), cout, off, Tpad, _hip.ptr(scale), _hip.ptr(shift), mm,
                act, y_batch_stride, _hip.ptr(flags), _hip.ptr(flags_out), _hip.stream())), "rn_wino_output_group_flags")
        else:
            _hip.check(prof.timed("wino_output", nb, lambda: lib.rn_wino_output_group(
                ctypes.byref(g), M.data_ptr(), cout, off, Tpad, _hip.ptr(scale), _hip.ptr(shift), mm,
                act, y_batch_stride, _hip.stream())), "rn_wino_output_group")
        if yams is not None:
            for o, w_ in zip(outs[sl], yams):
                amax_attach(o, w_)
        off += t
    return (outs, (V, tuple(tuple(x.shape) for x in xs), v_am)) if keep_v else outs


_WINO_Z = {}
SIDE_HELD = {}


def side_release(side=None):
    if side is None:
        SIDE_HELD.clear()
    else:
        SIDE_HELD.pop(side.cuda_stream, None)


def _wino_z_buffer(device, floats):
    cur = torch.cuda.current_stream(device)
    st = _WINO_Z.setdefault((device, cur.cuda_stream), {"bufs": [None, None], "ev": [None, None], "i": 0})
    k = st["i"]
    st["i"] ^= 1
    if st["bufs"][k] is None or st["bufs"][k].numel() < floats:
        st["bufs"][k] = torch.empty(floats, dtype=torch.float32, device=device)
    if st["ev"][k] is not None:
        cur.wait_event(st["ev"][k])
    return st, k


def wino_wgrad_group(gs, xs, dw, colsum, flops=0.0, V=None, dU=None, fuse_dgrad_input=False, side=None, flags=None, lists=None):
    lib = _hip.load()
    dev = xs[0].device
    C, cout = xs[0].shape[3], gs[0].shape[3]
    zst = None
    tiles = [x.shape[0] * ((x.shape[1] + 3) // 4) * ((x.shape[2] + 3) // 4) for x in xs]
    T = sum(tiles)
    Tpad = wino_tpad(T)
    have_v = V is not None and V[1] == tuple(tuple(x.shape) for x in xs) and V[0].numel() == 36 * Tpad * C
    v_tw = V[2][1] if have_v and len(V) > 2 and V[2] is not None else None
    V = V[0] if have_v else None
    Vw, Z = _wino_workspace(dev, 0 if have_v else 36 * Tpad * C, 36 * Tpad * cout)
    if not have_v:
        V = Vw
    assert all(g.shape[:3] == x.shape[:3] and g.is_contiguous() and x.is_contiguous() for g, x in zip(gs, xs))
    if not have_v:
        v_tw = _wino_transform_in(xs, V, C, Tpad, 0, want_tensor=True)[1]
    v_dy, z_tw = None, None
    if fuse_dgrad_input and have_v and len(gs) <= _hip.RN_MAX_GROUP:
        Vd, Z = _wino_workspace(dev, 36 * Tpad * cout, 36 * Tpad * cout)
        if side is not None:
            zst, zk = _wino_z_buffer(dev, 36 * Tpad * cout)
            Z = zst["bufs"][zk]
        am_on = want_amax()
        g = _wino_group(gs, srcs=gs, amaxs=[amax_words(t) for t in gs] if am_on else None)
        vd_rows = torch.zeros(Tpad, dtype=torch.int32, device=dev) if am_on else None
        z_tw = amax_single(dev) if am_on else None
        nb = 4.0 * (sum(t.numel() for t in gs) + 2 * 36 * T * cout)
        if flags is not None and not wino_flags_ok(T, C, cout):
            flags = None
        if flags is not None:
            assert flags.dtype == torch.uint8 and flags.numel() >= Tpad
        if flags is None or lists is None or lists is False:
            lists = None
        elif not isinstance(lists, TileLists):
            lists = tile_lists(flags, Tpad, buf=None if lists is True else lists)
        if lists is not None:
            assert lists.flags.data_ptr() == flags.data_ptr()
            _hip.check(prof.timed("wino_input", nb, lambda: lib.rn_wino_input_both_group_lists(
                ctypes.byref(g), Vd.data_ptr(), Z.data_ptr(), cout, 0, Tpad, _hip.ptr(vd_rows), _hip.ptr(z_tw), flags.data_ptr(),
                lists.units.data_ptr(), lists.counts.data_ptr() + 4, _hip.stream())), "rn_wino_input_both_group_lists")
        else:
            _hip.check(prof.timed("wino_input", nb, lambda: lib.rn_wino_input_both_group_flags(
                ctypes.byref(g), Vd.data_ptr(), Z.data_ptr(), cout, 0, Tpad, _hip.ptr(vd_rows), _hip.ptr(z_tw), _hip.ptr(flags),
                _hip.stream())), "rn_wino_input_both_group_flags")
        v_dy = (Vd, tuple(tuple(t.shape) for t in gs), (vd_rows, None)) + ((flags,) if flags is not None else ()) \
            + ((lists,) if lists is not None else ())
    else:
        flags = None
        z_tw = _wino_transform_in(gs, Z, cout, Tpad, 1, want_tensor=True)[1]
    am = (z_tw, v_tw) if (want_amax() and z_tw is not None and v_tw is not None) else (None, None)
    ku = (C + 31) // 32 * 32
    if dU is None or tuple(dU.shape) != (36, cout, ku):
        dU = torch.zeros((36, cout, ku), dtype=torch.float32, device=dev)
    def reductions():
        rc = prof.timed("conv_wgrad" + (" winograd T%d %d->%d" % (T, C, cout) if prof.BY_SHAPE else ""), 2.0 * 36 * T * cout * C, lambda: _wgrad_call(
            lib, dev, Z.data_ptr(), cout, V.data_ptr(), dU.data_ptr(), _hip.ptr(colsum), 36, Tpad * cout, Tpad * C, cout * ku, 7,
            (1, 1, T, C, 1, T, cout, 1, 1, 1, 0, 0), amax=am, flags=flags))
        _hip.check(rc, "rn_conv_wgrad_batched")
        _hip.check(lib.rn_wino_dw(dU.data_ptr(), dw.data_ptr(), cout, C, _hip.stream()), "rn_wino_dw")
    if zst is None:
        reductions()
    else:
        side.wait_event(torch.cuda.current_stream(dev).record_event())
        with torch.cuda.stream(side):
            reductions()
            zst["ev"][zk] = side.record_event()
        SIDE_HELD.setdefault(side.cuda_stream, []).append((V, dU, flags, lists) + tuple(am))
    return v_dy


def conv_igemm_grouped(problems, w_packed, scale=None, shift=None, act=ACT_NONE, flops=0.0):
    lib = _hip.load()
    g = _hip.ConvGroup()
    g.n = len(problems)
    total = 0
    wptr, wfmt, wus = None, None, None
    yams = []
    for i, pr in enumerate(problems):
        x, geom = pr["x"], pr["geom"]
        add, mask = pr.get("add"), pr.get("mask")
        mask_ptr, mmode = _mask_operand(mask, pr.get("mask_mode", 2))
        d = _make_desc(x, geom, act, 1 if add is not None else 0, (0, 0), mmode, False, None, pr.get("y_batch_stride"), None, None)
        if wfmt is None:
            wptr, wfmt, wus = _w_operand(w_packed, d)
        d.w_format, d.w_unscale = wfmt, wus
        if wfmt == 3:
            d.x_amax, d.x_amax_img_stride, d.x_amax_row_stride = amax_words(x).data_ptr(), 1, 0
        amax_drop(pr["y"])
        bits = _sign_words(pr["y"], pr.get("sign", False) and pr.get("y_batch_stride") is None)
        d.sign_out = None if bits is None else bits.data_ptr()
        yam = amax_slot(x.device, x.shape[0]) if want_amax() and pr.get("y_batch_stride") is None else None
        yams.append(yam)
        d.y_amax = None if yam is None else yam.data_ptr()
        g.d[i] = d
        M = d.N * d.Ho * d.Wo
        total += (M + 255) // 256 if d.Cout <= 64 else ((M + 127) // 128) * ((d.Cout + 127) // 128)
        g.tile_end[i] = total
        g.x[i], g.y[i], g.add[i], g.mask[i] = x.data_ptr(), pr["y"].data_ptr(), _hip.ptr(add), mask_ptr
    kind = "conv_igemm_4x1" if problems[0]["geom"][2] <= 64 else "conv_igemm_2x2"
    if prof.BY_SHAPE:
        kind += " grouped %d->%d k%d" % (g.d[0].Cin, g.d[0].Cout, g.d[0].kh)
    nb = 0.0
    if prof.ACTIVE is not None:
        nb = {0: 4.0, 1: 6.0, 3: 4.0}[wfmt] * w_packed.numel()
        for pr in problems:
            dd = pr["geom"]
            out_el = pr["x"].shape[0] * dd[0] * dd[1] * dd[2]
            nb += 4.0 * (pr["x"].numel() + out_el * (1 + (pr.get("add") is not None) + (pr.get("mask") is not None)))
    rc = prof.timed(kind, flops, lambda: lib.rn_conv_igemm_grouped(
        ctypes.byref(g), wptr, _hip.ptr(scale), _hip.ptr(shift), _hip.stream()), nb)
    _hip.check(rc, "rn_conv_igemm_grouped")
    for pr, yam in zip(problems, yams):
        if yam is not None:
            amax_attach(pr["y"], yam)


def fprop(x, w_packed, cout, k, stride, pad, kw_pad=None, **kw):
    N, Hi, Wi, _ = x.shape
    Ho, Wo = out_size(Hi, k, stride, pad), out_size(Wi, k, stride, pad)
    y = torch.empty((N, Ho, Wo, cout), dtype=torch.float32, device=x.device)
    return conv_igemm(x, w_packed, y, (Ho, Wo, cout, k, k if kw_pad is None else kw_pad, stride, 1, -pad, 0), **kw)


def dgrad(dy, w_packed_dgrad, in_hw, cin, k, stride, pad, **kw):
    N = dy.shape[0]
    Hi, Wi = in_hw
    dx = torch.empty((N, Hi, Wi, cin), dtype=torch.float32, device=dy.device)
    return conv_igemm(dy, w_packed_dgrad, dx, (Hi, Wi, cin, k, k, 1, -1, pad, stride.bit_length() - 1), **kw)


def s2_classes(k, pad):
    out = []
    for ph in (0, 1):
        r0 = (ph + pad) % 2
        nr = len(range(r0, k, 2))
        for pw in (0, 1):
            s0 = (pw + pad) % 2
            ns = len(range(s0, k, 2))
            if nr and ns:
                out.append((ph, pw, (r0, nr, s0, ns), ((ph + pad - r0) // 2, (pw + pad - s0) // 2)))
    return out


def dgrad_s2_classes(dy, class_weights, in_hw, cin, k, pad, flops=0.0, **kw):
    N, Ho, Wo, _ = dy.shape
    Hi, Wi = in_hw
    dx = torch.empty((N, Hi, Wi, cin), dtype=torch.float32, device=dy.device)
    classes = s2_classes(k, pad)
    if len(classes) < 4:
        dx.zero_()
    total_taps = sum(c[2][1] * c[2][3] for c in classes)
    slot = amax_slot(dy.device, N) if want_amax() else None
    for (ph, pw, (r0, nr, s0, ns), (dh0, dw0)), wc in zip(classes, class_weights):
        gh, gw = (Hi - ph + 1) // 2, (Wi - pw + 1) // 2
        if gh <= 0 or gw <= 0:
            continue
        conv_igemm(dy, wc, dx, (gh, gw, cin, nr, ns, 1, -1, (dh0, dw0), 0), out_map=(2, ph, pw, Hi, Wi),
                   flops=flops * nr * ns / total_taps, amax=slot, **kw)
    if slot is not None:
        amax_attach(dx, slot)
    return dx


def wgrad(dy, x, dw, cout, k, stride, pad, kw_pad=None, in_relu=False, flops=0.0, colsum=None):
    lib = _hip.load()
    N, Ho, Wo, ldy = dy.shape
    _, Hi, Wi, Cin = x.shape
    kind = "conv_wgrad" + (" %dx%dx%d %d->%d k%d s%d" % (N, Ho, Wo, Cin, cout, k, stride) if prof.BY_SHAPE else "")
    am = (amax_words(dy), amax_words(x)) if want_amax() and dy.is_contiguous() and x.is_contiguous() else (None, None)
    rc = prof.timed(kind, flops, lambda: _wgrad_call(
        lib, dy.device, dy.data_ptr(), ldy, x.data_ptr(), dw.data_ptr(), _hip.ptr(colsum), 1, 0, 0, 0, 0,
        (N, Hi, Wi, Cin, Ho, Wo, cout, k, k if kw_pad is None else kw_pad, stride, pad, int(in_relu)), amax=am))
    _hip.check(rc, "rn_conv_wgrad")
    return dw


def unpack_wgrad(dw, w_packed, weight_shape, kw_pad=None, c_pad=None, scale=None, mean=None, rstd=None, colsum=None,
                 want_bn=False, out=None):
    lib = _hip.load()
    cout, cin, kh, kw = weight_shape
    kw_pad = kw if kw_pad is None else kw_pad
    c_pad = (cin + 3) // 4 * 4 if c_pad is None else c_pad
    if out is not None:
        dweight, dgamma, dbeta = out
        assert tuple(dweight.shape) == tuple(weight_shape) and dweight.is_contiguous() and dweight.dtype == torch.float32
        assert (dgamma is not None) == bool(want_bn) and (dbeta is not None) == (colsum is not None)
    else:
        dweight = torch.empty(weight_shape, dtype=torch.float32, device=dw.device)
        dgamma = torch.empty(cout, dtype=torch.float32, device=dw.device) if want_bn else None
        dbeta = torch.empty(cout, dtype=torch.float32, device=dw.device) if colsum is not None else None
    _hip.check(lib.rn_unpack_wgrad(dw.data_ptr(), _hip.ptr(w_packed), dweight.data_ptr(), cout, cin, kh, kw, kw_pad,
                                   c_pad, _hip.ptr(scale), _hip.ptr(mean), _hip.ptr(rstd), _hip.ptr(colsum),
                                   _hip.ptr(dgamma), _hip.ptr(dbeta), _hip.stream()), "rn_unpack_wgrad")
    return dweight, dgamma, dbeta


def bn_fold(gamma, beta, mean, var, eps=1e-5):
    lib = _hip.load()
    C = gamma.numel()
    out = torch.empty((3, C), dtype=torch.float32, device=gamma.device)
# ... 407 lines not shown
```

3d-playground_amd/retinanet_mi355x/engine.py:

```python
import os

import torch

from . import _hip, arch, conv as cv, ops, prof


FUSE_DY = os.environ.get("RN_WINO_FUSE_DY", "1") != "0"
SPARSE_REG = os.environ.get("RN_SPARSE_REG", "1") != "0"
SPARSE_REG_LISTS = os.environ.get("RN_SPARSE_REG_LISTS", "1") != "0"
GROUPED_WGRAD_BF16 = os.environ.get("RN_GROUPED_WGRAD_BF16", "1") != "0"
S2_SHORTCUT_COMPACT = os.environ.get("RN_S2_SHORTCUT_COMPACT", "1") != "0"
STEM_BF16_PRODUCTS = os.environ.get("RN_STEM_BF16_PRODUCTS", "1") != "0"


def _qscale(t):
    return getattr(t, "_rn_scale", None) or getattr(t, "_rn_qscale", None)


def _as_fp8(t):
    if t is None or t.dtype == torch.uint8:
        return t
    q = getattr(t, "_rn_q8", None)
    if q is None:
        sc = _qscale(t)
        assert sc, "a tensor entering an fp8 layer needs its calibrated scale (Layer.fwd tags its outputs)"
        q = t._rn_q8 = cv.fp8_quantize(t, sc) if t.dtype == torch.float32 else cv.bf16_to_fp8(t, sc)
    return q


def _as_f32(t):
    if t is None or t.dtype == torch.float32:
        return t
    y = cv.fp8_dequantize(t) if t.dtype == torch.uint8 else cv.to_f32(t)
    y._rn_qscale = _qscale(t)
    return y


def _as_bf16(t):
    if t is None or t.dtype == torch.bfloat16:
        return t
    y = cv.fp8_to_bf16(t) if t.dtype == torch.uint8 else cv.to_bf16(t)
    y._rn_qscale = _qscale(t)
    return y


_AS = {"fp8": _as_fp8, "bf16": _as_bf16, "fp32": _as_f32}


class Layer:

    def __init__(self, spec, kw_pad=None, cin_pad=None, bf16=False, fp8=False):
        self.spec = spec
        self.bf16 = bf16
        self.fp8 = fp8
        self.out_scale = 1.0
        self.calib = None
        self.kw_pad = spec.k if kw_pad is None else kw_pad
        self.cin_pad = spec.cin if cin_pad is None else cin_pad
        self.cout_pad = (spec.cout + 31) // 32 * 32 if spec.cout % (8 if bf16 else 4) else spec.cout
        self.wino_ok = spec.k == 3 and spec.stride == 1 and spec.pad == 1 and spec.cin % 4 == 0 and spec.cout % 4 == 0
        self.wino_layer = self.wino_ok and min(spec.cin, spec.cout) >= 64 and max(spec.cin, spec.cout) >= 128 and not bf16
        self.wino_active = False
        self.sign = False
        self.keep_v = True
        self._cache = None
        self.reset()

    def reset(self):
        self.wf = self.wd = self.scale = self.shift = self.rstd = self.mean = None
        self.dw = self.cs = None
        self.uf = self.ud = None
        self.wf16 = self.wd16 = None
        self.saved_v = None
        self.dy_v = None

    def prepare(self, P, cache):
        s = self.spec
        self._cache = cache
        w = P[s.name + ".weight"]
        self.weight = w
        self.wf = cache.get(("wf", s.name), w, lambda: cv.pack_weights(w, 0, kw_pad=self.kw_pad, c_pad=self.cin_pad))
        if s.bn:
            g, b = P[s.bn + ".weight"], P[s.bn + ".bias"]
            self.mean = P[s.bn + ".running_mean"]
            self.scale, self.shift, self.rstd = cache.get(
                ("bn", s.bn), (g, b), lambda: cv.bn_fold(g, b, self.mean, P[s.bn + ".running_var"], arch.BN_EPS))
        else:
            self.scale = self.rstd = self.mean = None
            self.shift = P[s.name + ".bias"].detach() if s.bias else None
        self.wd = None
        self.dw = self.cs = None
        self.uf = self.ud = None
        self.wd16 = None
        self.wf16 = cache.get(("wf16", s.name), w, lambda: cv.to_bf16(self.wf)) if self.bf16 else None
        if self.fp8:
            self.wq, sw = cache.get(("wq", s.name), w, lambda: cv.fp8_quantize_weights(self.wf))
            self.wscale = cache.get(("wqs", s.name), (w,) + ((P[s.bn + ".weight"], P[s.bn + ".running_var"]) if s.bn else ()),
                                    lambda: (sw * self.scale) if self.scale is not None else sw)
            self._fp8_scales = {}

    def adopt(self, P, cache, wf, bn, wd, wino=None, wf16=None, wd16=None):
        s = self.spec
        self._cache = cache
        self.weight = P[s.name + ".weight"]
        self.wf = wf
        if s.bn:
            self.mean = P[s.bn + ".running_mean"]
            self.scale, self.shift, self.rstd = bn[0], bn[1], bn[2]
        else:
            self.scale = self.rstd = self.mean = None
            self.shift = P[s.name + ".bias"].detach() if s.bias else None
        self.wd = wd
        self.dw = self.cs = None
        self.uf, self.ud = wino if wino is not None else (None, None)
        self.wd16 = wd16
        self.wf16 = wf16 if wf16 is not None else (cv.to_bf16(self.wf) if self.bf16 else None)
        if self.fp8:
            self.wq, sw = cv.fp8_quantize_weights(self.wf)
            self.wscale = (sw * self.scale) if self.scale is not None else sw
            self._fp8_scales = {}

    def wino_weights(self, mode):
        if mode == 0:
            if self.uf is None:
                self.uf = self._cache.get(("uf", self.spec.name), self.weight, lambda: cv.wino_weights(self.weight, 0)) \
                    if self._cache is not None else cv.wino_weights(self.weight, 0)
            return self.uf
        if self.ud is None:
            self.ud = cv.wino_weights(self.weight, 1, scale=self.scale)
        return self.ud

    def dgrad_weights16(self):
        if self.wd16 is None:
            wd = self.dgrad_weights()
            self.wd16 = [cv.to_bf16(t) for t in wd] if isinstance(wd, list) else cv.to_bf16(wd)
        return self.wd16

    def dgrad_weights(self):
        if self.wd is None:
            s = self.spec
            if s.stride == 2 and s.k > 1:
                self.wd = [cv.pack_weights(self.weight, 1, scale=self.scale, c_pad=self.cout_pad, taps=c[2])
                           for c in cv.s2_classes(s.k, s.pad)]
            else:
                self.wd = cv.pack_weights(self.weight, 1, scale=self.scale, c_pad=self.cout_pad)
        return self.wd

    def fwd(self, x, act=cv.ACT_NONE, add=None, add_mode=0, add_hw=(0, 0), out=None, y_batch_stride=None, in_relu=False, sign=None):
        s = self.spec
        sign = (self.sign and act == cv.ACT_RELU) if sign is None else (sign and self.sign)
        N, Hi, Wi, _ = x.shape
        Ho, Wo = cv.out_size(Hi, s.k, s.stride, s.pad), cv.out_size(Wi, s.k, s.stride, s.pad)
        mode = self.mode()
        if self.fp8:
            x, add = _AS[mode](x), _AS[mode](add)
        if mode == "fp8":
            assert not in_relu, "fp8: the caller applies the input ReLU"
            return self._fwd_fp8(x, (Ho, Wo), act, add, add_mode, add_hw, out, y_batch_stride)
        if mode == "bf16":
            assert not in_relu, "bf16: the caller applies the input ReLU (cv.relu_bf16)"
            if out is None:
                out = torch.empty((N, Ho, Wo, s.cout), dtype=torch.bfloat16, device=x.device)
            cv.conv_igemm_bf16(x, self.wf16, out, (Ho, Wo, s.cout, s.k, self.kw_pad, s.stride, 1, -s.pad, 0),
                               scale=self.scale, shift=self.shift, add=add, add_mode=add_mode, add_hw=add_hw, act=act,
                               y_batch_stride=y_batch_stride, flops=self.flops(N, Ho, Wo), sign=sign)
            out._rn_qscale = self.out_scale
            return out
        if self.wino_active and out is None and add is None and not in_relu and y_batch_stride is None \
                and act in (cv.ACT_NONE, cv.ACT_RELU) and x.is_contiguous():
            r = cv.wino_conv_group([x], self.wino_weights(0), scale=self.scale, shift=self.shift, act=act, keep_v=self.keep_v, sign=sign)
            ys, self.saved_v = r if self.keep_v else (r, None)
            return ys[0]
        if out is None:
            out = torch.empty((N, Ho, Wo, s.cout), dtype=torch.float32, device=x.device)
        cv.conv_igemm(x, self.wf, out, (Ho, Wo, s.cout, s.k, self.kw_pad, s.stride, 1, -s.pad, 0), scale=self.scale,
                      shift=self.shift, add=add, add_mode=add_mode, add_hw=add_hw, act=act,
                      y_batch_stride=y_batch_stride, in_relu=in_relu, flops=self.flops(N, Ho, Wo), sign=sign,
                      bf16_products=getattr(self, "bf16_products", False))
        self._tap(out if y_batch_stride is None else None)
        out._rn_qscale = self.out_scale
        return out

    def mode(self):
        return getattr(self, "fwd_mode", None) or ("fp8" if self.fp8 else ("bf16" if self.bf16 else "fp32"))

    def _tap(self, out):
        if self.calib is not None and out is not None:
            self.calib[self.spec.name] = max(self.calib.get(self.spec.name, 0.0), float(out.abs().max()))

    def _fwd_fp8(self, x, out_hw, act, add, add_mode, add_hw, out, y_batch_stride):
        s = self.spec
        Ho, Wo = out_hw
        sx = float(x._rn_scale)
        scale = self._fp8_scales.get(sx)
        if scale is None:
            scale = self._fp8_scales[sx] = (self.wscale * sx).contiguous()
        if out is None:
            out = torch.empty((x.shape[0], Ho, Wo, s.cout), dtype=torch.uint8, device=x.device)
        return cv.conv_igemm_fp8(x, self.wq, out, (Ho, Wo, s.cout, s.k, self.kw_pad, s.stride, 1, -s.pad, 0), scale, shift=self.shift,
                                 add=add, add_mode=add_mode, add_hw=add_hw, act=act, y_batch_stride=y_batch_stride,
                                 out_scale=self.out_scale, flops=self.flops(x.shape[0], Ho, Wo))

    def fwd_group(self, xs, act=cv.ACT_NONE, outs=None, y_batch_stride=None, wino=False, shared_v=None):
        s = self.spec
        mode = self.mode()
        if self.fp8:
            xs = [_AS[mode](x) for x in xs]
        if mode == "fp8":
            scales = {float(x._rn_scale) for x in xs}
            if len(scales) > 1 or len(xs) > _hip.RN_MAX_GROUP:
                return [self._fwd_fp8(x, (x.shape[1], x.shape[2]), act, None, 0, (0, 0), None if outs is None else outs[i], y_batch_stride)
                        for i, x in enumerate(xs)]
            sx = scales.pop()
            scale = self._fp8_scales.get(sx)
            if scale is None:
                scale = self._fp8_scales[sx] = (self.wscale * sx).contiguous()
            probs, ys, fl = [], [], 0.0
            for i, x in enumerate(xs):
                N, Hi, Wi, _ = x.shape
                y = outs[i] if outs is not None else torch.empty((N, Hi, Wi, s.cout), dtype=torch.uint8, device=x.device)
                ys.append(y)
                fl += self.flops(N, Hi, Wi)
                probs.append({"x": x, "y": y, "geom": (Hi, Wi, s.cout, s.k, self.kw_pad, 1, 1, -s.pad, 0), "y_batch_stride": y_batch_stride})
            cv.conv_igemm_fp8_grouped(probs, self.wq, scale, shift=self.shift, act=act, out_scale=self.out_scale, flops=fl)
            return ys
        if mode == "bf16":
            probs, ys, fl = [], [], 0.0
            for i, x in enumerate(xs):
                N, Hi, Wi, _ = x.shape
                y = outs[i] if outs is not None else torch.empty((N, Hi, Wi, s.cout), dtype=torch.bfloat16, device=x.device)
                ys.append(y)
                fl += self.flops(N, Hi, Wi)
                probs.append({"x": x, "y": y, "geom": (Hi, Wi, s.cout, s.k, self.kw_pad, 1, 1, -s.pad, 0),
                              "y_batch_stride": y_batch_stride, "sign": self.sign and act == cv.ACT_RELU})
            cv.conv_igemm_bf16_grouped(probs, self.wf16, scale=self.scale, shift=self.shift, act=act, flops=fl)
            for y in ys:
                y._rn_qscale = self.out_scale
            return ys
        if (wino or self.wino_active) and self.wino_ok and (outs is None or y_batch_stride is not None):
            fl = sum(self.flops(x.shape[0], x.shape[1], x.shape[2]) for x in xs)
            r = cv.wino_conv_group(xs, self.wino_weights(0), outs=outs, scale=self.scale, shift=self.shift, act=act, flops=fl,
                                   keep_v=self.keep_v, y_batch_stride=y_batch_stride or 0, V_in=shared_v if self.keep_v else None,
                                   sign=self.sign and act == cv.ACT_RELU)
            ys, self.saved_v = r if self.keep_v else (r, None)
            return ys
        probs, ys, fl = [], [], 0.0
        for i, x in enumerate(xs):
            N, Hi, Wi, _ = x.shape
            Ho, Wo = cv.out_size(Hi, s.k, s.stride, s.pad), cv.out_size(Wi, s.k, s.stride, s.pad)
            y = outs[i] if outs is not None else torch.empty((N, Ho, Wo, s.cout), dtype=torch.float32, device=x.device)
            ys.append(y)
            fl += self.flops(N, Ho, Wo)
            probs.append({"x": x, "y": y, "geom": (Ho, Wo, s.cout, s.k, self.kw_pad, s.stride, 1, -s.pad, 0),
                          "y_batch_stride": y_batch_stride, "sign": self.sign and act == cv.ACT_RELU})
        cv.conv_igemm_grouped(probs, self.wf, scale=self.scale, shift=self.shift, act=act, flops=fl)
        if outs is None:
            for y in ys:
                self._tap(y)
                y._rn_qscale = self.out_scale
        return ys

    def bwd_data_group(self, gs, in_hws, adds=None, masks=None, wino=False, flags_out=None):
        s = self.spec
        assert s.stride == 1
        self.flags_out_done = False
        if self.bf16:
            probs, outs, fl = [], [], 0.0
            for i, g in enumerate(gs):
                Hi, Wi = in_hws[i]
                dx = torch.empty((g.shape[0], Hi, Wi, s.cin), dtype=torch.bfloat16, device=g.device)
                outs.append(dx)
                fl += self.flops(g.shape[0], g.shape[1], g.shape[2])
                probs.append({"x": g, "y": dx, "geom": (Hi, Wi, s.cin, s.k, s.k, 1, -1, s.pad, 0),
                              "add": None if adds is None else adds[i], "mask": None if masks is None else masks[i]})
            cv.conv_igemm_bf16_grouped(probs, self.dgrad_weights16(), flops=fl)
            return outs
        if (wino or self.wino_active) and self.wino_ok and all(g.shape[3] == s.cout for g in gs):
            fl = sum(self.flops(g.shape[0], g.shape[1], g.shape[2]) for g in gs)
            ready, self.dy_v = getattr(self, "dy_v", None), None
            self.flags_out_done = flags_out is not None
            return cv.wino_conv_group(gs, self.wino_weights(1), adds=adds, masks=masks, mask_mode=2, flops=fl, V_ready=ready,
                                      flags_out=flags_out)
        probs, outs, fl = [], [], 0.0
        for i, g in enumerate(gs):
            N = g.shape[0]
            Hi, Wi = in_hws[i]
            dx = torch.empty((N, Hi, Wi, s.cin), dtype=torch.float32, device=g.device)
            outs.append(dx)
            fl += self.flops(N, g.shape[1], g.shape[2])
            probs.append({"x": g, "y": dx, "geom": (Hi, Wi, s.cin, s.k, s.k, 1, -1, s.pad, 0),
                          "add": None if adds is None else adds[i], "mask": None if masks is None else masks[i]})
        cv.conv_igemm_grouped(probs, self.dgrad_weights(), flops=fl)
        return outs

    def flops(self, N, Ho, Wo):
        s = self.spec
        return 2.0 * N * Ho * Wo * s.cout * s.cin * s.k * s.k

    def bwd_params(self, g, x, in_relu=False, side=None):
        s = self.spec
        if self.dw is None:
            self.dw = torch.zeros_like(self.wf)
            self.cs = torch.zeros(s.cout, dtype=torch.float32, device=g.device)
        if self.bf16:
            assert not in_relu
            cv.wgrad_bf16(g, x, self.dw, s.cout, s.k, s.stride, s.pad, flops=self.flops(g.shape[0], g.shape[1], g.shape[2]),
                          colsum=self.cs)
            return
        if self.wino_active and not in_relu and g.shape[3] == s.cout and g.is_contiguous() and x.is_contiguous():
            du, self.du = getattr(self, "du", None), None
            self.dy_v = cv.wino_wgrad_group([g], [x], self.dw, self.cs, V=self.saved_v, dU=du, fuse_dgrad_input=FUSE_DY, side=side)
            self.saved_v = None
            return
        cv.wgrad(g, x, self.dw, s.cout, s.k, s.stride, s.pad, kw_pad=self.kw_pad, in_relu=in_relu,
                 flops=self.flops(g.shape[0], g.shape[1], g.shape[2]), colsum=self.cs)

    def bwd_params_group(self, gs, xs, wino=False, side=None, flags=None, lists=None):
        s = self.spec
        if (wino or self.wino_active) and self.wino_ok and all(g.shape[3] == s.cout and g.is_contiguous() for g in gs):
            if self.dw is None:
                self.dw = torch.zeros_like(self.wf)
                self.cs = torch.zeros(s.cout, dtype=torch.float32, device=gs[0].device)
            fl = sum(self.flops(g.shape[0], g.shape[1], g.shape[2]) for g in gs)
            du, self.du = getattr(self, "du", None), None
            self.dy_v = cv.wino_wgrad_group(gs, xs, self.dw, self.cs, flops=fl, V=self.saved_v, dU=du, fuse_dgrad_input=FUSE_DY, side=side,
                                            flags=flags, lists=lists)
            self.saved_v = None
            return
        if self.bf16 and GROUPED_WGRAD_BF16 and 1 < len(gs) <= 5 and all(g.is_contiguous() and x.is_contiguous() for g, x in zip(gs, xs)) \
                and len({g.shape[3] for g in gs}) == 1:
            if self.dw is None:
                self.dw = torch.zeros_like(self.wf)
                self.cs = torch.zeros(s.cout, dtype=torch.float32, device=gs[0].device)
            fl = sum(self.flops(g.shape[0], g.shape[1], g.shape[2]) for g in gs)
            cv.wgrad_bf16_grouped(gs, xs, self.dw, s.cout, s.k, s.stride, s.pad, flops=fl, colsum=self.cs)
            return
        for g, x in zip(gs, xs):
            self.bwd_params(g, x)

    def bwd_data(self, g, in_hw, add=None, mask=None, mask_mode=2, add2=None):
        s = self.spec
        if self.bf16:
            assert add2 is None
            kw = dict(add=add, add_mode=1 if add is not None else 0, mask=mask, mask_mode=mask_mode,
                      flops=self.flops(g.shape[0], g.shape[1], g.shape[2]))
            if s.stride == 2 and s.k > 1:
                return cv.dgrad_s2_classes_bf16(g, self.dgrad_weights16(), in_hw, s.cin, s.k, s.pad, **kw)
            if s.stride == 2 and s.k == 1 and s.pad == 0 and mask is None and S2_SHORTCUT_COMPACT:
                Hi, Wi = in_hw
                N, Ho, Wo, _ = g.shape
                if add is None:
                    dx = torch.zeros((N, Hi, Wi, s.cin), dtype=torch.bfloat16, device=g.device)
                else:
                    assert add.shape == (N, Hi, Wi, s.cin) and add.dtype == torch.bfloat16 and add.is_contiguous()
                    dx = add
                return cv.conv_igemm_bf16(g, self.dgrad_weights16(), dx, (Ho, Wo, s.cin, 1, 1, 1, -1, 0, 0), out_map=(2, 0, 0, Hi, Wi),
                                          add=add, add_mode=1 if add is not None else 0, flops=kw["flops"])
            return cv.dgrad_any_bf16(g, self.dgrad_weights16(), in_hw, s.cin, s.k, s.stride, s.pad, **kw)
        if self.wino_active and add2 is None and g.shape[3] == s.cout and g.is_contiguous():
            ready, self.dy_v = getattr(self, "dy_v", None), None
            return cv.wino_conv_group([g], self.wino_weights(1), adds=None if add is None else [add],
                                      masks=None if mask is None else [mask], mask_mode=mask_mode, V_ready=ready)[0]
        kw = dict(add=add, add_mode=1 if add is not None else 0, mask=mask, mask_mode=mask_mode,
                  flops=self.flops(g.shape[0], g.shape[1], g.shape[2]))
        if s.stride == 2 and s.k > 1:
            assert add2 is None
            return cv.dgrad_s2_classes(g, self.dgrad_weights(), in_hw, s.cin, s.k, s.pad, **kw)
        return cv.dgrad(g, self.dgrad_weights(), in_hw, s.cin, s.k, s.stride, s.pad, add2=add2, **kw)

    def bwd_data_compact(self, g):
        s = self.spec
        assert s.k == 1 and s.stride == 2
        N, Ho, Wo, _ = g.shape
        out = torch.empty((N, Ho, Wo, s.cin), dtype=torch.float32, device=g.device)
        return cv.conv_igemm(g, self.dgrad_weights(), out, (Ho, Wo, s.cin, 1, 1, 1, -1, 0, 0), flops=self.flops(N, Ho, Wo))

    def grad_names(self):
        s = self.spec
        if s.bn:
            return [s.name + ".weight", s.bn + ".weight", s.bn + ".bias"]
        return [s.name + ".weight"] + ([s.name + ".bias"] if s.bias else [])

    def finish(self, out=None):
        s = self.spec
        dst = None
        if out is not None:
            names = self.grad_names()
            dst = (out[names[0]], out[names[1]] if s.bn else None, out[names[-1]] if len(names) > 1 else None)
        dweight, dgamma, dbeta = cv.unpack_wgrad(
            self.dw, self.wf, tuple(self.weight.shape), kw_pad=self.kw_pad, c_pad=self.cin_pad, scale=self.scale,
            mean=self.mean, rstd=self.rstd, colsum=self.cs, want_bn=bool(s.bn), out=dst)
        out = {s.name + ".weight": dweight}
        if s.bn:
            out[s.bn + ".weight"] = dgamma
            out[s.bn + ".bias"] = dbeta
        elif s.bias:
# ... 258 lines not shown

        for name, L in self.layers.items():
            s = L.spec
            w = P[s.name + ".weight"]
            assert w.dtype == torch.float32 and w.is_contiguous() and w.is_cuda
            cout, cin, kh, kw = w.shape
            b = bufs[name] = {}
            b["wf"] = torch.empty((cout, (kh * L.kw_pad * L.cin_pad + 31) // 32 * 32), dtype=torch.float32, device=dev)
            add(0, pack_job(w, b["wf"], 0, L.kw_pad, L.cin_pad, None), b["wf"].numel())
            split_job(b["wf"], force=getattr(L, "bf16_products", False), f16=(cout, L.cin_pad, kh * L.kw_pad))
            if L.bf16:
                b["wf16"] = cast_job(b["wf"])
            scale = None
            if s.bn:
                bn = b["bn"] = torch.empty((3, cout), dtype=torch.float32, device=dev)
                j = _hip.PrepJob()
                j.kind, j.Cout, j.eps = 0, cout, arch.BN_EPS
                j.gamma, j.beta = P[s.bn + ".weight"].data_ptr(), P[s.bn + ".bias"].data_ptr()
                j.mean, j.var = P[s.bn + ".running_mean"].data_ptr(), P[s.bn + ".running_var"].data_ptr()
                j.bn_scale, j.bn_shift, j.bn_rstd = bn[0].data_ptr(), bn[1].data_ptr(), bn[2].data_ptr()
                add(0, j, cout)
                scale = bn[0]
            if self.use_wino and L.wino_layer:
                uf = torch.empty((36, cout, (cin + 31) // 32 * 32), dtype=torch.float32, device=dev)
                ud = torch.empty((36, cin, (cout + 31) // 32 * 32), dtype=torch.float32, device=dev)
                for which, mode, dst in ((0, 0, uf), (1, 1, ud)):
                    j = _hip.PrepJob()
                    j.kind, j.Cout, j.Cin, j.mode = 2, cout, cin, mode
                    j.rows, j.Kpad = dst.shape[1], dst.shape[2]
                    j.src, j.dst, j.scale = w.data_ptr(), dst.data_ptr(), None if (mode == 0 or scale is None) else scale.data_ptr()
                    add(which, j, dst.shape[1] * dst.shape[2])
                    split_job(dst, f16=(dst.shape[1], dst.shape[2], 1))
                b["wino"] = (uf, ud)
                continue
            if name == "conv1":
                continue
            if s.stride == 2 and s.k > 1:
                b["wd"] = []
                for c in cv.s2_classes(s.k, s.pad):
                    r0, nr, s0, ns = c[2]
                    d = torch.empty((cin, (nr * ns * L.cout_pad + 31) // 32 * 32), dtype=torch.float32, device=dev)
                    add(1, pack_job(w, d, 2, kw, L.cout_pad, scale, c[2]), d.numel())
                    split_job(d, f16=(cin, L.cout_pad, nr * ns))
                    b["wd"].append(d)
                if L.bf16:
                    b["wd16"] = [cast_job(d) for d in b["wd"]]
            else:
                d = b["wd"] = torch.empty((cin, (kh * kw * L.cout_pad + 31) // 32 * 32), dtype=torch.float32, device=dev)
                add(1, pack_job(w, d, 1, kw, L.cout_pad, scale), d.numel())
                split_job(d, f16=(cin, L.cout_pad, kh * kw))
                if L.bf16:
                    b["wd16"] = cast_job(d)
        out = []
        for jobs, chunks in launches:
            if not jobs:
                continue
            arr = (_hip.PrepJob * len(jobs))(*jobs)
            jt = torch.frombuffer(bytearray(bytes(arr)), dtype=torch.uint8).to(dev)
            ct = torch.tensor(chunks, dtype=torch.int32).to(dev)
            out.append((jt, ct, len(chunks)))
        return {"key": key, "launches": out, "bufs": bufs}

    def _unpack_bucket(self, index, layers, views):
        key = tuple((L.dw.data_ptr(), L.wf.data_ptr(), views[L.grad_names()[0]].data_ptr(), _hip.ptr(L.scale) or 0, _hip.ptr(L.mean) or 0)
                    for L in layers)
        cache = self.__dict__.setdefault("_unpack_tables", {})
        hit = cache.get(index)
        if hit is None or hit[0] != key:
            jobs, chunks = [], []
            for L in layers:
                s, names = L.spec, L.grad_names()
                cout, cin, kh, kw = L.weight.shape
                j = _hip.UnpackJob()
                j.dw, j.w_packed, j.dweight = L.dw.data_ptr(), L.wf.data_ptr(), views[names[0]].data_ptr()
                j.Cout, j.Cin, j.kh, j.kw, j.kw_pad, j.c_pad, j.Kpad = cout, cin, kh, kw, L.kw_pad, L.cin_pad, L.wf.shape[1]
                j.scale, j.mean, j.rstd, j.colsum = _hip.ptr(L.scale), _hip.ptr(L.mean), _hip.ptr(L.rstd), L.cs.data_ptr()
                j.dgamma = views[names[1]].data_ptr() if s.bn else None
                j.dbeta = views[names[-1]].data_ptr() if len(names) > 1 else None
                chunks.extend((len(jobs), co) for co in range(cout))
                jobs.append(j)
            arr = (_hip.UnpackJob * len(jobs))(*jobs)
            dev = layers[0].dw.device
            hit = cache[index] = (key, torch.frombuffer(bytearray(bytes(arr)), dtype=torch.uint8).to(dev),
                                  torch.tensor(chunks, dtype=torch.int32).to(dev), len(chunks))
        _hip.check(_hip.load().rn_unpack_batched(hit[1].data_ptr(), hit[2].data_ptr(), hit[3], _hip.stream()), "rn_unpack_batched")
        for L in layers:
            L.dw = L.cs = L.wd = L.uf = L.ud = L.saved_v = L.dy_v = None

    def _zero_grad_accumulators(self, device, flag_bytes=0, flag_arrays=0):
        wino = self.use_wino and not self.bwd16
        sizes = []
        for L in self.layers.values():
            s = L.spec
            du = 36 * s.cout * ((s.cin + 31) // 32 * 32) if (wino and L.wino_layer) else 0
            sizes.append((L, L.wf.numel(), (s.cout + 3) // 4 * 4, du))
        total = (sum(a + b + c for _, a, b, c in sizes) + 3) // 4 * 4
        acc_floats = total
        total += flag_arrays * flag_bytes // 4
        arena = getattr(self, "_arena", None)
        if arena is None or arena.numel() != total or arena.device != device:
            arena = self._arena = torch.empty(total, dtype=torch.float32, device=device)
        arena.zero_()
        o = 0
        for L, a, b, c in sizes:
            L.dw = arena[o:o + a].view_as(L.wf)
            L.cs = arena[o + a:o + a + L.spec.cout]
            L.du = arena[o + a + b:o + a + b + c].view(36, L.spec.cout, -1) if c else None
            o += a + b + c
        fb = arena[acc_floats:].view(torch.uint8)
        self._reg_flags = [fb[i * flag_bytes:(i + 1) * flag_bytes] for i in range(flag_arrays)]
        n = cv.tile_lists_numel(flag_bytes) if flag_arrays else 0
        bufs = getattr(self, "_reg_list_bufs", None)
        if flag_arrays and (bufs is None or len(bufs) != flag_arrays or bufs[0].numel() != n or bufs[0].device != device):
            bufs = self._reg_list_bufs = [torch.empty(n, dtype=torch.int32, device=device) for _ in range(flag_arrays)]
        self._reg_lists = bufs if flag_arrays else []

    def calibrate(self, P, frames, margin=1.0):
        if self.fp8 or self.bf16:
            raise RuntimeError("calibrate with the fp32 engine (ResNet.calibrate_fp8 switches to it): the magnitudes are recorded "
                               "by the fp32 direct kernels' path only")
        rec = {}
        wino_eval, self.wino_eval = self.wino_eval, False
        for L in self.layers.values():
            L.calib = rec
        self.calib = rec
        try:
            with torch.no_grad():
                self.forward(P, frames, save=False)
        finally:
            for L in self.layers.values():
                L.calib = None
            self.calib = None
            self.wino_eval = wino_eval
        missing = [n for n in self.fp8_scale_names() if n not in rec]
        assert not missing, "calibration pass did not record %s" % missing
        return {k: v * margin for k, v in rec.items()}

    def fp8_scale_names(self):
        return ["pool"] + [n for n in self.layers if n != "conv1" and not n.endswith(".output")]

    def set_fp8_layers(self, fp8=None, other="fp32"):
        assert self.fp8 and other in ("fp32", "bf16")
        pick = (lambda n: True) if fp8 is None else (fp8 if callable(fp8) else (lambda n, names=set(fp8): n in names))
        self._fp8_explicit = True
        on = []
        for n, L in self.layers.items():
            if n == "conv1":
                continue
            L.fwd_mode = "fp8" if pick(n) else other
            if L.fwd_mode == "fp8":
                on.append(n)
        return on

    def forward(self, P, img, save, x4=None):
        Ls = self.layers
        if save and os.environ.get("RN_BATCHED_PREP", "1") != "0":
            self._prepare_training(P)
        else:
            self._prepare(P)
        if self.fp8:
            if save and not self.fp8_trainable:
                raise RuntimeError("the fp8 training step (fp8 forward, bf16 gradients) is built for the bottleneck networks "
                                   "(resnet50/101/152), like the bf16 schedule")
            if not self.fp8_scales:
                raise RuntimeError("the fp8 engine needs activation scales: net.calibrate_fp8(frames) first")
            missing = [n_ for n_ in self.fp8_scale_names() if not self.fp8_scales.get(n_, 0.0) > 0.0]
            if missing:
                raise RuntimeError("fp8 activation scales are missing (or zero) for %d tensors, e.g. %s: run net.calibrate_fp8(frames) "
                                   "on representative frames" % (len(missing), ", ".join(missing[:4])))
            if getattr(self, "_fp8_explicit", None) is None:
                stream = (lambda n_: n_.endswith(".conv3") or ".downsample." in n_ or n_.startswith("fpn.") or n_ == "regressionModel.conv4") \
                    if self.fp8_policy == "stream_bf16" else (lambda n_: False)
                for n_, L in Ls.items():
                    if n_ != "conv1":
                        L.fwd_mode = "bf16" if stream(n_) else "fp8"
            if save and any(L.mode() == "fp32" for n_, L in Ls.items() if n_ != "conv1"):
                raise RuntimeError("the fp8 training step saves e4m3 / bf16 activations for the bf16 gradient kernels: no fp32-format layers")
            for n_, L in Ls.items():
                L.out_scale = max(self.fp8_scales.get(n_, 0.0), 1e-30) / cv.FP8_MAX
            pyr = ("fpn.P3_2", "fpn.P4_2", "fpn.P5_2", "fpn.P6", "fpn.P7_2")
            common = max(Ls[n_].out_scale for n_ in pyr)
            for n_ in pyr:
                Ls[n_].out_scale = common
        for L in Ls.values():
            L.wino_active = bool((save or self.wino_eval) and self.use_wino and L.wino_layer and not self.bf16 and not self.fp8)
            L.keep_v = bool(save)
            L.sign = bool(save) and not L.fp8 and (not L.bf16 or cv.BITMASKS_BF16)
        if x4 is None:
            _hip.need_gpu(img)
            x4 = cv.nchw_to_nhwc4(img)
        else:
            _hip.need_gpu(x4)
        B, H, W, _ = x4.shape
        S = {} if save else None
        stem = Ls["conv1"].fwd(x4, act=cv.ACT_RELU)
        pool = cv.maxpool_fwd_bf16 if self.bf16 else cv.maxpool_fwd
        if self.fp8 and not save and getattr(self, "calib", None) is None:
            x = cv.maxpool_fwd_fp8(stem, max(self.fp8_scales.get("pool", 0.0), 1e-30) / cv.FP8_MAX)
        else:
            if save:
                x, pool_arg = pool(stem, want_argmax=True)
                S["x4"], S["stem"], S["pool_arg"] = x4, stem, pool_arg
            else:
                x = pool(stem)
            if getattr(self, "calib", None) is not None:
                self.calib["pool"] = max(self.calib.get("pool", 0.0), float(x.abs().max()))
            if self.fp8:
                x = cv.fp8_quantize(x, max(self.fp8_scales.get("pool", 0.0), 1e-30) / cv.FP8_MAX)
        if save:
            S["blocks"] = []
        feats = {}
        for pre, roles in self.blocks:
            xin = x
            t1 = roles["conv1"].fwd(xin, act=cv.ACT_RELU)
            res = roles["down"].fwd(xin) if "down" in roles else xin
            if self.kind == "basic":
                t2 = None
                x = roles["conv2"].fwd(t1, act=cv.ACT_RELU, add=res, add_mode=1)
            else:
                t2 = roles["conv2"].fwd(t1, act=cv.ACT_RELU)
                x = roles["conv3"].fwd(t2, act=cv.ACT_RELU, add=res, add_mode=1)
            if save:
                S["blocks"].append((xin, t1, t2, x))
            feats[pre.split(".")[0]] = x
        c3, c4, c5 = feats["layer2"], feats["layer3"], feats["layer4"]
        p5lat = Ls["fpn.P5_1"].fwd(c5)
        p5 = Ls["fpn.P5_2"].fwd(p5lat)
        p4sum = Ls["fpn.P4_1"].fwd(c4, add=p5lat, add_mode=2, add_hw=(p5lat.shape[1], p5lat.shape[2]))
        p4 = Ls["fpn.P4_2"].fwd(p4sum)
        p3sum = Ls["fpn.P3_1"].fwd(c3, add=p4sum, add_mode=2, add_hw=(p4sum.shape[1], p4sum.shape[2]))
        p3 = Ls["fpn.P3_2"].fwd(p3sum)
        p6 = Ls["fpn.P6"].fwd(c5, sign=True)
        p6r = cv.relu_bf16(p6) if self.bf16 else None
        if self.fp8:
            p6r = torch.relu(_as_f32(p6))
            p6r._rn_qscale = _qscale(p6)
        p7 = Ls["fpn.P7_2"].fwd(p6r) if (self.bf16 or self.fp8) else Ls["fpn.P7_2"].fwd(p6, in_relu=True)
        pyramid = [p3, p4, p5, p6, p7]
        if save:
            S["fpn"] = (c3, c4, c5, p5lat, p4sum, p3sum, p6)
            S["p6r"] = p6r
            S["pyramid"] = pyramid
        counts = [f.shape[1] * f.shape[2] * arch.NUM_ANCHORS for f in pyramid]
        A = sum(counts)
        reg = torch.empty((B, A, self.n_reg), dtype=torch.float32, device=x4.device)
        cls = torch.empty((B, A, self.num_classes), dtype=torch.float32, device=x4.device)
        if save:
            S["towers"] = {"regressionModel": [], "classificationModel": []}
            S["counts"] = counts
        side = self.tower_streams(x4.device)
        main = torch.cuda.current_stream(x4.device)
        v_ready = None
        if side is not None:
            fork = main.record_event()
        for ti, (prefix, out, width, act) in enumerate((("regressionModel", reg, self.n_reg, cv.ACT_NONE),
                                                        ("classificationModel", cls, self.num_classes, cv.ACT_SIGMOID))):
            if side is not None:
                side[ti].wait_event(fork)
                if ti == 1 and v_ready is not None:
                    side[ti].wait_event(v_ready)
            with torch.cuda.stream(side[ti] if side is not None else main):
                ts = pyramid
                acts = []
                for i in range(1, 5):
                    first = Ls["regressionModel.conv1"]
                    shared = first.saved_v if (i == 1 and prefix == "classificationModel") else None
                    ts = Ls["%s.conv%d" % (prefix, i)].fwd_group(ts, act=cv.ACT_RELU, wino=save and self.use_wino and not self.bf16 and not self.fp8,
                                                                 shared_v=shared)
                    acts.append(ts)
                    if side is not None and ti == 0 and i == 1:
                        v_ready = side[0].record_event()
                views, off = [], 0
                for cnt in counts:
                    views.append(out.view(B, -1)[:, off * width:])
                    off += cnt
                Ls[prefix + ".output"].fwd_group(ts, act=act, outs=views, y_batch_stride=A * width)
            if save:
                S["towers"][prefix] = [[acts[i][li] for i in range(4)] for li in range(5)]
        if side is not None:
            main.wait_stream(side[0])
            main.wait_stream(side[1])
        if save:
            S["wino_v"] = {n: L.saved_v for n, L in Ls.items() if L.saved_v is not None}
        for L in Ls.values():
            L.saved_v = None
        return reg, cls, S

    def backward(self, S, dreg, dcls, cls):
        Ls = self.layers
        grads = {}
        sparse_reg = SPARSE_REG and self.use_wino and not self.bwd16 and not self.bf16 and not self.fp8 and dreg.is_cuda
        reg_tiles = [dreg.shape[0] * ((f.shape[1] + 3) // 4) * ((f.shape[2] + 3) // 4) for f in S["pyramid"]]
        self._zero_grad_accumulators(dreg.device, cv.wino_tpad(sum(reg_tiles)) if sparse_reg else 0, 5 if sparse_reg else 0)
        for L in Ls.values():
            L.saved_v = L.dy_v = None
        for n, v in S.pop("wino_v", {}).items():
            Ls[n].saved_v = v

        flat = views = None
        next_bucket = 0
        if self.flat_bucket_bytes:
            flat, views = self._flat_views(dreg.device)
            buckets = self._flat["buckets"]

        batched = flat is not None and self.grad_hook is None and os.environ.get("RN_BATCHED_UNPACK", "1") != "0"
        pending = []

        main0 = torch.cuda.current_stream(dreg.device) if dreg.is_cuda else None
        wss = self.wgrad_streams(dreg.device) if batched else None
        wg_count = 0
        held = []

        def join():
            for ws in wss or ():
                main0.wait_stream(ws)
                cv.side_release(ws)
            held.clear()

        def aside(fn, tensors):
            nonlocal wg_count
            ws = wss[wg_count % len(wss)]
            wg_count += 1
            if cv.want_amax():
                for t in tensors:
                    if t.dtype == torch.float32 and t.is_contiguous():
                        cv.amax_words(t)
            ws.wait_event(torch.cuda.current_stream(dreg.device).record_event())
            with torch.cuda.stream(ws):
                fn()
            held.append(tuple(tensors) + tuple(getattr(t, "_rn_amax", (None,))[0] for t in tensors))

        def wg(L, g, x, in_relu=False):
            if wss is None:
                L.bwd_params(g, x, in_relu=in_relu)
            elif L.wino_active and not L.bf16:
                L.bwd_params(g, x, in_relu=in_relu, side=wss[0] if os.environ.get("RN_WGRAD_WINO", "1") != "0" else None)
            else:
                aside(lambda: L.bwd_params(g, x, in_relu=in_relu), (g, x))

        def wg_group(L, gs, xs, wino=False, flags=None, lists=None):
            if wss is None or os.environ.get("RN_WGRAD_TOWERS", "0") == "0":
                L.bwd_params_group(gs, xs, wino=wino, flags=flags, lists=lists)
            elif wino or L.wino_active:
                L.bwd_params_group(gs, xs, wino=wino, side=wss[0], flags=flags, lists=lists)
            else:
                aside(lambda: L.bwd_params_group(gs, xs), tuple(gs) + tuple(xs))

        def done(layer):
            nonlocal next_bucket
            if batched:
                pending.append(layer)
                grads.update({n: views[n] for n in layer.grad_names()})
            else:
                g = layer.finish(views)
                grads.update(g)
                if self.grad_hook is not None:
                    self.grad_hook(g)
            if flat is not None and layer.spec.name == buckets[next_bucket][2]:
                if batched:
                    join()
                    self._unpack_bucket(next_bucket, pending, views)
                    pending.clear()
                if self.bucket_hook is not None:
                    self.bucket_hook(next_bucket, flat[buckets[next_bucket][0]:buckets[next_bucket][1]])
                next_bucket += 1

        ACT = _as_bf16 if self.fp8 else (lambda t: t)
        pyramid, counts = [ACT(t) for t in S["pyramid"]], S["counts"]
        B = dreg.shape[0]
        A = dreg.shape[1]
        dpyr = [None] * 5
        hws = [(f.shape[1], f.shape[2]) for f in pyramid]
        side = self.tower_streams(dreg.device)
        main = torch.cuda.current_stream(dreg.device)
        if side is not None:
            fork = main.record_event()
        retired = []
        for ti, (prefix, dout, width, sig) in enumerate((("regressionModel", dreg, self.n_reg, None),
                                                         ("classificationModel", dcls, self.num_classes, cls))):
            Lout = Ls[prefix + ".output"]
            tower = [Ls["%s.conv%d" % (prefix, i)] for i in range(1, 5)]
            if side is not None:
                side[ti].wait_event(fork)
            with torch.cuda.stream(side[ti] if side is not None else main):
                acts = [[ACT(t) for t in lvl] for lvl in S["towers"][prefix]]
                F = self._reg_flags if (ti == 0 and sparse_reg and Lout.wino_active) else None
                fl = F[0] if F else None
                LB = self._reg_lists if (F and SPARSE_REG_LISTS) else None
                lb = lambda k, fl_: LB[k] if (LB and fl_ is not None) else None
                gs, off, t_off = [], 0, 0
                for li, ((Hh, Ww), cnt) in enumerate(zip(hws, counts)):
                    byte_off = 4 * off * width
                    g = cv.sigmoid_bwd_pad(dout.data_ptr() + byte_off, None if sig is None else sig.data_ptr() + byte_off,
                                           B, Hh * Ww, arch.NUM_ANCHORS * width, Lout.cout_pad, A * width, dout.device,
                                           bf16=self.bwd16, hw=(Hh, Ww), flags=None if fl is None else fl[t_off:t_off + reg_tiles[li]])
                    gs.append(cv.amax_carry(g.view(B, Hh, Ww, Lout.cout_pad), g))
                    off += cnt
                    t_off += reg_tiles[li]
                wg_group(Lout, gs, [acts[li][3] for li in range(5)], flags=fl, lists=lb(0, fl))
                nxt = F[1] if fl is not None else None
                gs = Lout.bwd_data_group(gs, hws, masks=[acts[li][3] for li in range(5)], flags_out=nxt)
                fl = nxt if Lout.flags_out_done else None
                for i in (3, 2, 1):
                    wg_group(tower[i], gs, [acts[li][i - 1] for li in range(5)], wino=self.use_wino and not self.bwd16, flags=fl,
                             lists=lb(4 - i, fl))
                    nxt = F[5 - i] if fl is not None else None
                    gs = tower[i].bwd_data_group(gs, hws, masks=[acts[li][i - 1] for li in range(5)], wino=self.use_wino and not self.bwd16,
                                                 flags_out=nxt)
                    fl = nxt if tower[i].flags_out_done else None
                wg_group(tower[0], gs, pyramid, wino=self.use_wino and not self.bwd16, flags=fl, lists=lb(4, fl))
                first = dpyr[0] is None
                if side is not None and not first:
                    side[ti].wait_stream(side[0])
                dpyr = tower[0].bwd_data_group(gs, hws, adds=None if first else dpyr, wino=self.use_wino and not self.bwd16)
            S["towers"][prefix] = None
            retired.append(Lout)
            retired.extend(reversed(tower))
        if side is not None:
            main.wait_stream(side[0])
            main.wait_stream(side[1])
        for L in retired:
            done(L)
        c3, c4, c5, p5lat, p4sum, p3sum, p6 = (ACT(t) for t in S["fpn"])
        dp3, dp4, dp5, dp6, dp7 = dpyr
        hw = lambda t: (t.shape[1], t.shape[2])
        L = Ls["fpn.P7_2"]
        if self.bwd16:
            wg(L, dp7, ACT(S["p6r"]))
        else:
            wg(L, dp7, p6, in_relu=True)
        dp6 = L.bwd_data(dp7, hw(p6), add=dp6, mask=p6, mask_mode=1)
        done(L)
        L = Ls["fpn.P6"]
        wg(L, dp6, c5)
        dc5 = L.bwd_data(dp6, hw(c5))
        done(L)
        L = Ls["fpn.P3_2"]
        wg(L, dp3, p3sum)
        dp3sum = L.bwd_data(dp3, hw(p3sum))
        done(L)
        L = Ls["fpn.P3_1"]
        wg(L, dp3sum, c3)
        dc3 = L.bwd_data(dp3sum, hw(c3))
        done(L)
        L = Ls["fpn.P4_2"]
# ... 62 lines not shown
```

3d-playground_amd/retinanet_mi355x/modules.py:

```python
import math

import torch
import torch.nn as nn

from . import _hip, arch, engine, ops, torch_ops


class BasicBlock(nn.Module):
    expansion = 1

    def __init__(self, inplanes, planes, stride=1, downsample=None):
        super().__init__()
        self.conv1 = nn.Conv2d(inplanes, planes, 3, stride, 1, bias=False)
        self.bn1 = nn.BatchNorm2d(planes)
        self.relu = nn.ReLU(inplace=True)
        self.conv2 = nn.Conv2d(planes, planes, 3, 1, 1, bias=False)
        self.bn2 = nn.BatchNorm2d(planes)
        self.downsample = downsample
        self.stride = stride


class Bottleneck(nn.Module):
    expansion = 4

    def __init__(self, inplanes, planes, stride=1, downsample=None):
        super().__init__()
        self.conv1 = nn.Conv2d(inplanes, planes, 1, bias=False)
        self.bn1 = nn.BatchNorm2d(planes)
        self.conv2 = nn.Conv2d(planes, planes, 3, stride, 1, bias=False)
        self.bn2 = nn.BatchNorm2d(planes)
        self.conv3 = nn.Conv2d(planes, planes * 4, 1, bias=False)
        self.bn3 = nn.BatchNorm2d(planes * 4)
        self.relu = nn.ReLU(inplace=True)
        self.downsample = downsample
        self.stride = stride


class PyramidFeatures(nn.Module):
    def __init__(self, C3_size, C4_size, C5_size, feature_size=256):
        super().__init__()
        self.P5_1 = nn.Conv2d(C5_size, feature_size, 1, 1, 0)
        self.P5_upsampled = nn.Upsample(scale_factor=2, mode="nearest")
        self.P5_2 = nn.Conv2d(feature_size, feature_size, 3, 1, 1)
        self.P4_1 = nn.Conv2d(C4_size, feature_size, 1, 1, 0)
        self.P4_upsampled = nn.Upsample(scale_factor=2, mode="nearest")
        self.P4_2 = nn.Conv2d(feature_size, feature_size, 3, 1, 1)
        self.P3_1 = nn.Conv2d(C3_size, feature_size, 1, 1, 0)
        self.P3_2 = nn.Conv2d(feature_size, feature_size, 3, 1, 1)
        self.P6 = nn.Conv2d(C5_size, feature_size, 3, 2, 1)
        self.P7_1 = nn.ReLU()
        self.P7_2 = nn.Conv2d(feature_size, feature_size, 3, 2, 1)


class _Tower(nn.Module):
    def __init__(self, num_features_in, n_out, feature_size):
        super().__init__()
        for i in range(1, 5):
            setattr(self, "conv%d" % i, nn.Conv2d(num_features_in if i == 1 else feature_size, feature_size, 3, padding=1))
            setattr(self, "act%d" % i, nn.ReLU())
        self.output = nn.Conv2d(feature_size, n_out, 3, padding=1)


class RegressionModel(_Tower):
    def __init__(self, num_features_in, num_anchors=9, feature_size=256, n_outputs=8):
        super().__init__(num_features_in, num_anchors * n_outputs, feature_size)
        self.n_outputs = n_outputs


class ClassificationModel(_Tower):
    def __init__(self, num_features_in, num_anchors=9, num_classes=80, prior=0.01, feature_size=256):
        super().__init__(num_features_in, num_anchors * num_classes, feature_size)
        self.num_classes = num_classes
        self.num_anchors = num_anchors
        self.output_act = nn.Sigmoid()


class Anchors(nn.Module):
    def __init__(self, pyramid_levels=None, strides=None, sizes=None, ratios=None, scales=None):
        super().__init__()
        if not (pyramid_levels is None and strides is None and sizes is None and ratios is None and scales is None):
            raise NotImplementedError("the reference ignores every non-default argument except by crashing "
                                      "(D/anchors.py:9-19 only assigns the attributes in the None branches)")
        self.pyramid_levels = [3, 4, 5, 6, 7]
        self.strides = [2 ** x for x in self.pyramid_levels]
        self.sizes = [2 ** (x + 2) for x in self.pyramid_levels]

    def forward(self, image):
        if not image.is_cuda:
            raise RuntimeError("anchors are generated on the MI355X (no CPU fallback); got device %s" % image.device)
        return torch.ops.retinanet_mi355x.anchors(image.shape[2], image.shape[3], image.device)


class BBoxTransform(nn.Module):
    def __init__(self, mean=None, std=None, directional=True):
        super().__init__()
        if mean is not None or std is not None:
            raise NotImplementedError("custom mean/std: the directional transform never reads them (D/utils.py:102-149) "
                                      "and every caller of the 2D one uses the defaults (R/model.py:196)")
        self.directional = directional

    def forward(self, boxes, regression):
        if self.directional:
            return torch.ops.retinanet_mi355x.decode_dir(boxes, regression)
        return torch.ops.retinanet_mi355x.decode_2d(boxes, regression, False, 0, 0)


class ClipBoxes(nn.Module):
    def __init__(self, width=None, height=None):
        super().__init__()

    def forward(self, boxes, img):
        ops.clip_boxes_check(boxes)
        torch.ops.retinanet_mi355x.clip_boxes_(boxes, img.shape[2], img.shape[3])
        return boxes


class FocalLoss(nn.Module):
    def __init__(self, directional=True):
        super().__init__()
        self.directional = directional

    def forward(self, classifications, regressions, anchors, annotations):
        return torch_ops.focal_loss(classifications, regressions, anchors, annotations, self.directional)


def calc_iou(a, b):
    return torch.ops.retinanet_mi355x.pairwise_iou(a, b)


class _NetFn(torch.autograd.Function):

    @staticmethod
    def forward(ctx, net, img, ann, *params):
        eng = net._engine
        P = net._tensor_dict()
        reg, cls, S = eng.forward(P, img, save=True)
        anc = eng.anchors(img.shape[2], img.shape[3], img.device)
        lib = _hip.load()
        ann_c = _hip.f32c(ann)
        B, A, C = cls.shape
        ws = ops.focal_workspace(B, A, img.device)
        losses = torch.empty(3, dtype=torch.float32, device=img.device)
        _hip.check(lib.rn_focal_loss_fwd(cls.data_ptr(), reg.data_ptr(), anc.data_ptr(), _hip.ptr(ann_c), B, A, C,
                                         ann_c.shape[1], int(net.directional), ws.data_ptr(), losses.data_ptr(),
                                         _hip.stream()), "rn_focal_loss_fwd")
        ctx.net, ctx.S, ctx.pack = net, S, (reg, cls, anc, ann_c, ws)
        return losses[0:1], losses[1:2], losses[2:3]

    @staticmethod
    def backward(ctx, g_cls, g_reg, g_vp):
        net, S = ctx.net, ctx.S
        reg, cls, anc, ann_c, ws = ctx.pack
        ctx.S = ctx.pack = None
        lib = _hip.load()
        B, A, C = cls.shape
        g = torch.cat([t.reshape(1).float() for t in (g_cls, g_reg, g_vp)])
        dcls, dreg = torch.empty_like(cls), torch.empty_like(reg)
        _hip.check(lib.rn_focal_loss_bwd(cls.data_ptr(), reg.data_ptr(), anc.data_ptr(), _hip.ptr(ann_c), B, A, C,
                                         ann_c.shape[1], int(net.directional), ws.data_ptr(), g.data_ptr(),
                                         dcls.data_ptr(), dreg.data_ptr(), _hip.stream()), "rn_focal_loss_bwd")
        red = net.__dict__.get("_reducer")
        eng = net._engine
        if red is not None:
            red.backward_begins()
        grads = eng.backward(S, dreg, dcls, cls)
        if red is not None:
            red.finalize_flat(eng._flat["arena"])
        return (None, None, None) + tuple(grads[n] for n in eng.param_names)


class ResNet(nn.Module):

    def __init__(self, num_classes, block, layers, directional=True):
        self.inplanes = 64
        super().__init__()
        self.directional = directional
        self.ingest_swap_rb = False
        self.ingest_mean, self.ingest_std = ops.IMAGENET_MEAN, ops.IMAGENET_STD
        self.conv1 = nn.Conv2d(3, 64, kernel_size=7, stride=2, padding=3, bias=False)
        self.bn1 = nn.BatchNorm2d(64)
        self.relu = nn.ReLU(inplace=True)
        self.maxpool = nn.MaxPool2d(kernel_size=3, stride=2, padding=1)
        self.layer1 = self._make_layer(block, 64, layers[0])
        self.layer2 = self._make_layer(block, 128, layers[1], stride=2)
        self.layer3 = self._make_layer(block, 256, layers[2], stride=2)
        self.layer4 = self._make_layer(block, 512, layers[3], stride=2)
        e = block.expansion
        self.fpn = PyramidFeatures(128 * e, 256 * e, 512 * e)
        n_reg = 12 if directional else 4
        self.regressionModel = RegressionModel(256, n_outputs=n_reg)
        self.classificationModel = ClassificationModel(256, num_classes=num_classes)
        self.anchors = Anchors()
        self.regressBoxes = BBoxTransform(directional=directional)
        self.clipBoxes = ClipBoxes()
        self.focalLoss = FocalLoss(directional=directional)
        for m in self.modules():
            if isinstance(m, nn.Conv2d):
                n = m.kernel_size[0] * m.kernel_size[1] * m.out_channels
                m.weight.data.normal_(0, math.sqrt(2. / n))
            elif isinstance(m, nn.BatchNorm2d):
                m.weight.data.fill_(1)
                m.bias.data.zero_()
        prior = 0.01
        self.classificationModel.output.weight.data.fill_(0)
        self.classificationModel.output.bias.data.fill_(-math.log((1.0 - prior) / prior))
        self.regressionModel.output.weight.data.fill_(0)
        self.regressionModel.output.bias.data.fill_(0)
        self.freeze_bn()
        arch_name = {(BasicBlock, (2, 2, 2, 2)): "resnet18", (BasicBlock, (3, 4, 6, 3)): "resnet34",
                     (Bottleneck, (3, 4, 6, 3)): "resnet50", (Bottleneck, (3, 4, 23, 3)): "resnet101",
                     (Bottleneck, (3, 8, 36, 3)): "resnet152"}.get((block, tuple(layers)))
        if arch_name is None:
            raise ValueError("Block type %s / layers %s not understood" % (block, layers))
        self.__dict__["_arch_name"] = arch_name
        self.__dict__["_engine"] = engine.Engine(arch_name, num_classes, n_reg)

    def _make_layer(self, block, planes, blocks, stride=1):
        downsample = None
        if stride != 1 or self.inplanes != planes * block.expansion:
            downsample = nn.Sequential(
                nn.Conv2d(self.inplanes, planes * block.expansion, kernel_size=1, stride=stride, bias=False),
                nn.BatchNorm2d(planes * block.expansion))
        layers = [block(self.inplanes, planes, stride, downsample)]
        self.inplanes = planes * block.expansion
        for _ in range(1, blocks):
            layers.append(block(self.inplanes, planes))
        return nn.Sequential(*layers)

    def freeze_bn(self):
        for layer in self.modules():
            if isinstance(layer, nn.BatchNorm2d):
                layer.eval()

    def set_gradient_reducer(self, reducer):
        self.__dict__["_reducer"] = reducer
        if reducer is not None:
            reducer.attach(self._engine)
        else:
            self._engine.bucket_hook = None
            self._engine.set_flat_grads(None)

    def set_compute_dtype(self, dtype):
        old = self._engine
        eng = engine.Engine(self._arch_name, old.num_classes, old.n_reg, dtype=dtype)
        eng.set_flat_grads(old.flat_bucket_bytes, old.flat_tail_bytes)
        eng.bucket_hook = old.bucket_hook
        eng.fp8_scales = getattr(old, "fp8_scales", None)
        self.__dict__["_engine"] = eng
        return self

    def calibrate_fp8(self, frames, margin=1.0):
        if self._engine.fp8 or self._engine.bf16:
            self.set_compute_dtype("fp32")
        scales = self._engine.calibrate(self._tensor_dict(), frames, margin)
        self.set_compute_dtype("fp8")
        self._engine.fp8_scales = scales
        return scales

    def use_flat_gradients(self, on=True):
        self._engine.set_flat_grads((32 << 20) if on else None)

    def _replicate_for_data_parallel(self):
        raise RuntimeError(
            "this drop-in does not run under torch.nn.DataParallel: its HIP engine keeps per-device state and would be "
            "shared by the replica threads.  Use one process per GPU instead: retinanet_mi355x.ddp.init_from_env() + "
            "net.set_gradient_reducer(ddp.GradReducer()) (see INTEGRATION.md, 'Multi-GPU').")

    def load_state_dict(self, state_dict, strict=True, **kwargs):
        keys = list(state_dict.keys())
        if keys and all(k.startswith("module.") for k in keys):
            stripped = type(state_dict)()
            for k in keys:
                stripped[k[len("module."):]] = state_dict[k]
            meta = getattr(state_dict, "_metadata", None)
            if meta is not None:
                stripped._metadata = type(meta)((k[len("module."):] if k.startswith("module.") else ("" if k == "module" else k), v)
                                                for k, v in meta.items())
            state_dict = stripped
        return super().load_state_dict(state_dict, strict=strict, **kwargs)

    def _tensor_dict(self):
        d = dict(self.named_parameters())
        d.update(dict(self.named_buffers()))
        return d

    def forward(self, inputs, LOCALIZE=False, MULTI_FRAME=False):
        eng = self._engine
        if self.training:
            img_batch, annotations = inputs
            ops.check_labels(annotations, self.directional)
            P = dict(self.named_parameters())
            params = [P[n] for n in eng.param_names]
# ... 50 lines not shown
```

include/retinanet_mi355x.h:

```cpp
#ifndef RETINANET_MI355X_H
#define RETINANET_MI355X_H

#include <stdint.h>

#ifdef __cplusplus
extern "C" {
#endif

#define RN_OK 0
#define RN_EINVAL 10001
#define RN_ETOOMANY 10002
#define RN_MAX_GT 256
#define RN_LEVELS 5

const char *rn_version(void);
int rn_check_device(void);

int64_t rn_anchor_count(int height, int width);
void rn_anchor_base_boxes(double out[RN_LEVELS * 9 * 4]);
int rn_anchors_fwd(float *out, int height, int width, void *stream);

int rn_pairwise_iou(const float *a, const float *b, float *iou, int64_t A, int N, void *stream);

int64_t rn_focal_workspace_bytes(int B, int64_t A);
// ... 186 lines not shown
    int Ho, Wo, Cout;
    int kh, kw;
    int a, b, p, p_w, div_shift;
    int act;
    int add_mode;
    int Ha, Wa;
    int mask_mode;
    int in_relu;
    int os, oo_h, oo_w, Hy, Wy;
    int add2_mode;
    int Ha2, Wa2;
    int64_t add2_batch_stride;
    int64_t x_batch_stride, y_batch_stride, add_batch_stride;
    int64_t w_batch_stride;
    int w_format;
    void *sign_out;
    const void *x_amax;
    void *y_amax;
    const float *w_unscale;
    int x_amax_img_stride, x_amax_row_stride;
    const void *row_active;
    const void *row_list;
    const void *row_list_n;
    int row_list_grid;
} rn_conv_desc;
#define RN_MASK_BITS 4

#define RN_FP32_NATIVE 0
#define RN_FP32_SPLIT 1
#define RN_FP32_SPLIT3 2
#define RN_FP32_DEFAULT RN_FP32_SPLIT3
int rn_get_fp32_mfma(void);
int rn_set_fp32_mfma(int mode);
#define RN_OPT_SPLITK 0
#define RN_OPT_DETERMINISTIC 1
#define RN_OPT_MF16 2
#define RN_OPT_MF16_MIN 3
#define RN_OPT_WGRAD_ONCE 4
#define RN_OPT_BF16_P8 5
#define RN_OPT_FP8_P8 6
#define RN_OPT_COUNT 7
int rn_get_option(int option);
int rn_set_option(int option, int value);
int rn_fp32_split_min_k(void);
int rn_split_weights(const float *w_packed, void *w_split, int64_t rows, int Kpad, void *stream);
int rn_split_weights_f16(const float *w_packed, void *w_split, float *row_unscale, int64_t rows, int Kpad, void *stream);
int rn_amax(const float *x, int64_t per_image, int n_images, void *amax, void *stream);
int rn_stream_capture_id(void *stream, unsigned long long *id);
int rn_conv_igemm_wants_f16(const rn_conv_desc *d);

int rn_conv_igemm(const rn_conv_desc *d, const float *x, const float *w_packed, float *y,
                  const float *scale, const float *shift, const float *add, const float *mask, const float *add2,
                  void *stream);

int64_t rn_conv_splitk_workspace_bytes(const rn_conv_desc *d);
int rn_conv_igemm_splitk(const rn_conv_desc *d, const float *x, const float *w_packed, float *y, const float *scale,
                         const float *shift, const float *add, const float *mask, const float *add2, void *workspace,
                         void *stream);

#define RN_MAX_GROUP 5
typedef struct rn_conv_group {
    int n;
    int tile_end[RN_MAX_GROUP];
    rn_conv_desc d[RN_MAX_GROUP];
    const float *x[RN_MAX_GROUP];
    float *y[RN_MAX_GROUP];
    const float *add[RN_MAX_GROUP];
    const float *mask[RN_MAX_GROUP];
} rn_conv_group;
int rn_conv_igemm_grouped(const rn_conv_group *g, const float *w_packed, const float *scale, const float *shift,
                          void *stream);

int rn_conv_wgrad(const float *dy, int ldy, const float *x, float *dw, float *colsum, int N, int Hi, int Wi,
                  int Cin, int Ho, int Wo, int Cout, int kh, int kw, int stride, int pad, int in_relu, void *stream);
int rn_conv_wgrad_batched(const float *dy, int ldy, const float *x, float *dw, float *colsum, int nbatch,
                          int64_t dy_bstride, int64_t x_bstride, int64_t dw_bstride, int colsum_batch, int N, int Hi, int Wi,
                          int Cin, int Ho, int Wo, int Cout, int kh, int kw, int stride, int pad, int in_relu,
                          const void *dy_amax, int dy_amax_n, const void *x_amax, int x_amax_n, void *stream);
int64_t rn_conv_wgrad_det_workspace_bytes(int ldy, int nbatch, int64_t dw_bstride, int N, int Hi, int Wi, int Cin, int Ho, int Wo,
                                          int Cout, int kh, int kw);
int rn_conv_wgrad_batched_det(const float *dy, int ldy, const float *x, float *dw, float *colsum, int nbatch,
                              int64_t dy_bstride, int64_t x_bstride, int64_t dw_bstride, int colsum_batch, int N, int Hi, int Wi,
                              int Cin, int Ho, int Wo, int Cout, int kh, int kw, int stride, int pad, int in_relu,
                              const void *dy_amax, int dy_amax_n, const void *x_amax, int x_amax_n, void *workspace, int64_t workspace_bytes,
                              void *stream);
int rn_conv_wgrad_batched_flags(const float *dy, int ldy, const float *x, float *dw, float *colsum, int nbatch,
                                int64_t dy_bstride, int64_t x_bstride, int64_t dw_bstride, int colsum_batch, int N, int Hi, int Wi,
                                int Cin, int Ho, int Wo, int Cout, int kh, int kw, int stride, int pad, int in_relu,
                                const void *dy_amax, int dy_amax_n, const void *x_amax, int x_amax_n, const void *k_active,
                                void *workspace, int64_t workspace_bytes, void *stream);
int rn_conv_wgrad_plan(int ldy, int nbatch, int64_t dy_bstride, int64_t x_bstride, int64_t dw_bstride, int colsum_batch, int N, int Hi,
                       int Wi, int Cin, int Ho, int Wo, int Cout, int kh, int kw, int stride, int pad, int in_relu, int have_amax,
                       int have_flags, int det, int32_t *out);

int rn_f32_to_bf16(const float *src, void *dst, int64_t n, void *stream);
int rn_bf16_to_f32(const void *src, float *dst, int64_t n, void *stream);
int rn_conv_igemm_bf16(const rn_conv_desc *d, const void *x, const void *w_packed, void *y, int y_is_f32,
                       const float *scale, const float *shift, const void *add, const void *mask, void *stream);
int rn_conv_igemm_bf16_grouped(const rn_conv_group *g, const void *w_packed, int y_is_f32, const float *scale,
                               const float *shift, void *stream);
int rn_conv_igemm_bf16_tile_rows(const rn_conv_group *g, int y_is_f32);
int rn_fp8_quantize(const float *src, void *dst, int64_t n, float inv_scale, void *stream);
int rn_maxpool_fwd_fp8out(const float *x, void *y, int N, int H, int W, int C, int Ho, int Wo, float inv_scale, void *stream);
int rn_fp8_dequantize(const void *src, float *dst, int64_t n, float scale, void *stream);
int rn_fp8_to_bf16(const void *src, void *dst, int64_t n, float scale, void *stream);
int rn_bf16_to_fp8(const void *src, void *dst, int64_t n, float inv_scale, void *stream);
int rn_fp8_quantize_rows(const float *w_packed, void *w_q, float *row_scale, int64_t rows, int Kpad, void *stream);
int rn_conv_igemm_fp8(const rn_conv_desc *d, const void *x_q, const void *w_q, void *y, int y_is_f32, const float *scale,
                      const float *shift, const void *add_q, float add_scale, float out_inv_scale, void *stream);
int rn_conv_igemm_fp8_tile_rows(const rn_conv_group *g, int y_is_f32);
int rn_conv_igemm_fp8_tile(const rn_conv_desc *d, int y_is_f32);
int rn_conv_igemm_bf16_tile(const rn_conv_desc *d, int y_is_f32);
int rn_conv_igemm_fp8_grouped(const rn_conv_group *g, const void *w_q, int y_is_f32, const float *scale, const float *shift,
                              float add_scale, float out_inv_scale, void *stream);

int rn_conv_wgrad_bf16(const void *dy, int ldy, const void *x, float *dw, float *colsum, int N, int Hi, int Wi, int Cin,
                       int Ho, int Wo, int Cout, int kh, int kw, int stride, int pad, void *stream);
int rn_conv_wgrad_bf16_grouped(int n, const void *const *dy, int ldy, const void *const *x, float *dw, float *colsum, int N,
                               const int *Hi, const int *Wi, int Cin, int Cout, int kh, int kw, int stride, int pad, void *stream);

int rn_maxpool_fwd_bf16out(const float *x, void *y, uint8_t *argmax, int N, int H, int W, int C, int Ho, int Wo, void *stream);
int rn_maxpool_bwd_bf16in(const float *x, const void *dy, const uint8_t *argmax, float *dx, int N, int H, int W, int C, int Ho,
                          int Wo, int relu_mask, void *stream);
int rn_upsample_add_bwd_bf16(const void *src, void *dst, int N, int Hs, int Ws, int Hd, int Wd, int C, void *stream);
int rn_sigmoid_bwd_pad_bf16(const float *dy, const float *s, void *out, int B, int64_t rows_per_image, int C, int ld,
                            int64_t src_batch_stride, void *stream);
int rn_relu_bf16(const void *src, void *dst, int64_t n, void *stream);

typedef struct rn_wino_group {
    int n;
    int N[RN_MAX_GROUP], H[RN_MAX_GROUP], W[RN_MAX_GROUP];
    const float *src[RN_MAX_GROUP];
    float *dst[RN_MAX_GROUP];
    const float *add[RN_MAX_GROUP];
    const float *mask[RN_MAX_GROUP];
    void *sign[RN_MAX_GROUP];
    void *amax[RN_MAX_GROUP];
} rn_wino_group;
int rn_wino_input_group(const rn_wino_group *g, float *V, int C, int64_t tile_offset, int64_t Tpad, int dy_form,
                        void *row_amax, void *tensor_amax, void *stream);
int rn_wino_input_both_group(const rn_wino_group *g, float *V, float *Z, int C, int64_t tile_offset, int64_t Tpad,
                             void *v_row_amax, void *z_tensor_amax, void *stream);
int rn_wino_output_group(const rn_wino_group *g, const float *M, int Cout, int64_t tile_offset, int64_t Tpad,
                         const float *scale, const float *shift, int mask_mode, int act, int64_t y_batch_stride, void *stream);
int rn_wino_input_both_group_flags(const rn_wino_group *g, float *V, float *Z, int C, int64_t tile_offset, int64_t Tpad,
                                   void *v_row_amax, void *z_tensor_amax, const void *flags, void *stream);
int rn_wino_output_group_flags(const rn_wino_group *g, const float *M, int Cout, int64_t tile_offset, int64_t Tpad,
                               const float *scale, const float *shift, int mask_mode, int act, int64_t y_batch_stride,
                               const void *flags_in, void *flags_out, void *stream);
int rn_tile_lists(const void *flags, int64_t Tpad, void *counts, void *tiles, void *units, void *blocks, void *stream);
int rn_wino_input_both_group_lists(const rn_wino_group *g, float *V, float *Z, int C, int64_t tile_offset, int64_t Tpad,
                                   void *v_row_amax, void *z_tensor_amax, const void *flags, const void *units, const void *n_units,
                                   void *stream);
int rn_wino_input(const float *x, float *V, int N, int H, int W, int C, int64_t tile_offset, int64_t Tpad, void *stream);
int rn_wino_output(const float *M, float *y, int N, int H, int W, int Cout, int64_t tile_offset, int64_t Tpad,
                   const float *scale, const float *shift, const float *add, const float *mask, int mask_mode, int act,
                   int64_t y_batch_stride, void *stream);
int rn_wino_weights(const float *w, float *U, int Cout, int Cin, int mode, const float *scale, void *stream);
int rn_wino_dy(const float *dy, float *Z, int N, int H, int W, int C, int64_t tile_offset, int64_t Tpad, void *stream);
int rn_wino_dw(const float *dU, float *dw, int Cout, int Cin, void *stream);

typedef struct rn_prep_job {
    int kind;
    int Cout, Cin, kh, kw, kw_pad, c_pad, mode, r0, nr, s0, ns, rows, Kpad;
    float eps;
    const float *src;
    float *dst;
    const float *scale;
    const float *gamma, *beta, *mean, *var;
    float *bn_scale, *bn_shift, *bn_rstd;
} rn_prep_job;
int rn_prep_batched(const rn_prep_job *jobs_dev, const int32_t *chunks_dev, int nchunks, void *stream);

int rn_pack_weights(const float *src, float *dst, int Cout, int Cin, int kh, int kw, int kw_pad, int c_pad,
                    int mode, const float *scale, int r0, int nr, int s0, int ns, void *stream);
int rn_unpack_wgrad(const float *dw, const float *w_packed, float *dweight, int Cout, int Cin, int kh, int kw,
                    int kw_pad, int c_pad, const float *scale, const float *mean, const float *rstd,
                    const float *colsum, float *dgamma, float *dbeta, void *stream);

typedef struct rn_unpack_job {
    const float *dw, *w_packed;
    float *dweight;
    int Cout, Cin, kh, kw, kw_pad, c_pad, Kpad;
    const float *scale, *mean, *rstd, *colsum;
    float *dgamma, *dbeta;
} rn_unpack_job;
int rn_unpack_batched(const rn_unpack_job *jobs_dev, const int32_t *chunks_dev, int nchunks, void *stream);

int rn_bn_fold(const float *gamma, const float *beta, const float *mean, const float *var, float eps, int C,
               float *scale, float *shift, float *rstd, void *stream);

int rn_nchw_to_nhwc4(const float *src, float *dst, int N, int H, int W, void *amax, void *stream);
int rn_maxpool_fwd(const float *x, float *y, uint8_t *argmax, int N, int H, int W, int C, int Ho, int Wo, void *stream);
int rn_maxpool_bwd(const float *x, const float *dy, const uint8_t *argmax, float *dx, int N, int H, int W, int C,
                   int Ho, int Wo, int relu_mask, void *amax, void *stream);
int rn_colsum(const float *g, int64_t rows, int C, int ld, float *out, int accumulate, void *workspace, void *stream);
int64_t rn_colsum_workspace_bytes(int64_t rows, int C);
int rn_upsample_add_bwd(const float *src, float *dst, int N, int Hs, int Ws, int Hd, int Wd, int C, void *amax, void *stream);
int rn_relu_mask(float *g, const float *z, int64_t n, void *stream);
int rn_sigmoid_bwd_pad(const float *dy, const float *s, float *out, int B, int64_t rows_per_image, int C, int ld,
                       int64_t src_batch_stride, void *amax, void *stream);
int rn_sigmoid_bwd_pad_flags(const float *dy, const float *s, float *out, int B, int H, int W, int C, int ld,
                             int64_t src_batch_stride, void *amax, void *flags, void *stream);
int rn_add_inplace(float *dst, const float *src, int64_t n, int64_t per_image, void *amax, void *stream);

int64_t rn_opt_workspace_bytes(int n_chunks);
int rn_opt_clip_adam(const void *tensor_table, const void *chunk_table, int n_chunks, float max_norm, float lr,
                     float beta1, float beta2, float eps, int step, int write_clipped, void *workspace,
                     float *total_norm, void *stream);
int rn_opt_clip_adam_dev(const void *tensor_table, const void *chunk_table, int n_chunks, float max_norm, float lr,
                         float beta1, float beta2, float eps, int *step_dev, int write_clipped, void *workspace,
                         float *total_norm, void *stream);
int rn_opt_clip_adam_hp(const void *tensor_table, const void *chunk_table, int n_chunks, const float *hp, int *step_dev,
                        int write_clipped, void *workspace, float *total_norm, void *stream);

#define RN_MOT_MAX 512
#define RN_MOT_MAX_IDS 16384
#define RN_MOT_RESULT 152
#define RN_MOT_OK 0
#define RN_MOT_INVALID 1
#define RN_MOT_INFEASIBLE 2
#define RN_MOT_TOO_LARGE 3
int rn_mot_prepare(const double *gt_im, const float *gt_h0, const float *gt_vel, int64_t G, const float *pred_state,
                   int64_t M, const double *H, const double *P, float *gt_state, float *gt_box, float *pred_box,
                   double *pred_im, void *stream);
int rn_mot_iou(const float *gt_box, const float *pred_box, const int32_t *gt_off, const int32_t *pr_off,
               const int64_t *iou_off, int64_t F, int64_t max_cells, double *iou, void *stream);
int rn_mot_assign(const double *iou, const int32_t *gt_off, const int32_t *pr_off, const int64_t *iou_off,
                  const int32_t *slot_off, int64_t F, int64_t max_n, int64_t S, int64_t M, int32_t *slot_row,
                  int32_t *slot_col, uint8_t *pred_assigned, int32_t *frame_status, void *stream);
int rn_mot_frame_metrics(const double *iou, const int32_t *gt_off, const int32_t *pr_off, const int64_t *iou_off,
                         const int32_t *slot_off, int64_t F, int64_t S, const int32_t *slot_row, const int32_t *slot_col,
                         const int32_t *frame_status, double match_iou, const float *gt_state, const float *pred_state,
                         const double *gt_im, const double *pred_im, const int32_t *gt_cls, const int32_t *pred_cls,
                         const int32_t *gt_id, const int32_t *pred_id, const uint8_t *pred_assigned, double *slot_iou,
                         int32_t *slot_gid, int32_t *slot_pid, float *slot_state_err, double *slot_bot, double *slot_top,
                         uint8_t *slot_cls, int32_t *frame_edge, int32_t *frame_match, void *stream);
int64_t rn_mot_workspace_bytes(int64_t n_gid, int64_t n_pid);
int rn_mot_reduce(int64_t F, int64_t S, const int32_t *gt_off, const int32_t *pr_off, const int32_t *slot_off,
                  const int32_t *frame_status, const int32_t *frame_edge, const int32_t *frame_match,
                  const int32_t *slot_row, const double *slot_iou, const int32_t *slot_gid, const int32_t *slot_pid,
                  const float *slot_state_err, const double *slot_bot, const double *slot_top, const uint8_t *slot_cls,
                  const int32_t *gt_id, const int32_t *pred_id, int64_t n_gid, int64_t n_pid, void *workspace,
                  double *result, void *stream);

#define RN_MOT_ALPHAS 19
#define RN_MOT_ASSOC_RESULT 135
#define RN_MOT_ASSOC_MAX_CELLS 1048576
#define RN_MOT_DUPLICATE_ID 4
#define RN_MOT_BAD_INDEX 5
int64_t rn_mot_assoc_workspace_bytes(int64_t n_gid, int64_t n_pid);
int rn_mot_id_counts(const double *iou, const int32_t *gt_off, const int32_t *pr_off, const int64_t *iou_off,
                     const int32_t *slot_off, int64_t F, int64_t max_n, int64_t n_gt, int64_t n_pr, int64_t cells, int64_t S,
                     const int32_t *gt_id, const int32_t *pred_id, int64_t n_gid, int64_t n_pid, double id_iou, int32_t *gc,
                     int32_t *pc, int32_t *C, int32_t *status, void *stream);
int rn_mot_id_assign(const int32_t *C, int64_t n_gid, int64_t n_pid, void *workspace, int32_t *match, int64_t *info,
                     void *stream);
int rn_mot_hota_align(const double *iou, const int32_t *gt_off, const int32_t *pr_off, const int64_t *iou_off,
                      const int32_t *slot_off, int64_t F, int64_t max_n, int64_t n_gt, int64_t n_pr, int64_t cells, int64_t S,
                      const int32_t *gt_id, const int32_t *pred_id, const int32_t *csr_off, const int32_t *csr_frame,
                      const int32_t *csr_row, int64_t n_csr, int64_t n_gid, int64_t n_pid, double *rowsum, double *colsum,
                      double *pot, int32_t *status, void *stream);
int rn_mot_hota_assign(const double *iou, const int32_t *gt_off, const int32_t *pr_off, const int64_t *iou_off,
                       const int32_t *slot_off, int64_t F, int64_t max_n, int64_t n_gt, int64_t n_pr, int64_t cells, int64_t S,
                       const int32_t *gt_id, const int32_t *pred_id, int64_t n_gid, int64_t n_pid, const int32_t *gc,
                       const int32_t *pc, const double *pot, const double *alphas, double *score, int32_t *slot_row,
                       int32_t *slot_col, double *slot_s, int32_t *slot_n, int32_t *frame_status, void *stream);
int rn_mot_hota_reduce(const int32_t *gt_off, const int32_t *pr_off, const int64_t *iou_off, const int32_t *slot_off,
                       int64_t F, int64_t max_n, int64_t n_gt, int64_t n_pr, int64_t cells, int64_t S,
                       const int32_t *frame_status, const int32_t *slot_row, const int32_t *slot_col, const double *slot_s,
                       const int32_t *slot_n, const int32_t *gt_id, const int32_t *pred_id, const int32_t *gc,
                       const int32_t *pc, int64_t n_gid, int64_t n_pid, void *workspace, double *result, void *stream);

#define RN_VP_MAX_AXIS 32
#define RN_VP_FEW_LINES 1
#define RN_VP_BAD_START 2
#define RN_VP_LONG_AXIS 4
#define RN_VP_BAD_OFFSETS 8
#define RN_SZ_BAD_FIRST_STEP 1
#define RN_SZ_NO_WINNER 2
#define RN_SZ_TOO_MANY 4
#define RN_FIT_FEW_POINTS 1
#define RN_FIT_DEGENERATE 2
#define RN_FIT_NOT_FINITE 4
#define RN_FIT_BAD_OFFSETS 8
int rn_vanishing_points(const double *lines, int64_t rows, const int64_t *offsets, int64_t sets, double *out, double *trace,
                        int32_t *status, void *stream);
int rn_hg_reproj_error(const double *boxes, const float *heights, const double *H, const double *P_orig, const double *C,
                       int64_t d, int64_t K, double *out, void *stream);
int rn_hg_scale_z(const double *boxes, const float *heights, const double *H, const double *P_orig, int64_t d,
                  double granularity, double max_scale, int max_iters, double *trace, double *out, int32_t *info,
                  void *stream);
int rn_fit_homography(const double *src, const double *dst, int64_t rows, const int64_t *offsets, int64_t problems, int refine,
                      double *H, int32_t *status, void *stream);

#define RN_REINTERP_TILE 1024
#define RN_REINTERP_BAD_OFFSETS 1
#define RN_REINTERP_BAD_PAIR 2
#define RN_REINTERP_BAD_MATE 4
#define RN_REINTERP_BAD_PREFIX 8
#define RN_REINTERP_BAD_MAT_INDEX 16
int rn_reinterp_mate(const int64_t *offsets, const int64_t *ids, int64_t F, int64_t R, int32_t *mate, int32_t *status,
                     void *stream);
int rn_reinterp_offsets(const int64_t *offsets, const int32_t *mate, int64_t F, int64_t R, const int32_t *inst_a, int64_t T,
                        int32_t *frame_count, int32_t *count, int64_t *prefix, int32_t *status, void *stream);
int rn_reinterp_rows(const int64_t *offsets, const double *frame_ts, const double *fields, const int32_t *mate,
// ... 163 lines not shown
```

Measured before the change: 134.8 images/sec.

## Restrict regression-head output conv forward to label-flagged Winograd tiles

Adds a kernel that marks the Winograd tiles covering anchors with IoU of at least 0.5 against any ground-truth box, then builds tile lists from those flags. The regression head's final conv forward runs its input transform and output transform only on the listed tiles, and writes zeros into V for unflagged tiles. Only positive anchors feed the regression loss, so this skips work whose result the loss never reads. The cost is an extra anchor-matching pass and list build per step. Regression outputs at non-positive anchors are no longer computed, and guards raise an error if the forward and backward sparse settings disagree.

```diff
diff --git a/3d-playground_amd/csrc/conv_wino.hip b/3d-playground_amd/csrc/conv_wino.hip
--- a/3d-playground_amd/csrc/conv_wino.hip
+++ b/3d-playground_amd/csrc/conv_wino.hip
@@ -69,14 +69,26 @@
     _Pragma("unroll") for (int i_ = 1; i_ < RN_MAX_GROUP; ++i_) \
         if (q == i_) { pr = g.p[i_]; EXTRA }
 
+template <bool LIST = false>
 __global__ __launch_bounds__(256) void wino_in_kernel(const WinoTable g, float *__restrict__ V, int C, int64_t t0, int64_t Tpad,
-                                                      unsigned *__restrict__ row_amax, unsigned *__restrict__ tensor_amax) {
+                                                      unsigned *__restrict__ row_amax, unsigned *__restrict__ tensor_amax,
+                                                      const unsigned char *__restrict__ flags = nullptr,
+                                                      const int *__restrict__ units = nullptr,
+                                                      const int *__restrict__ n_units = nullptr) {
     wino_tensor_word(g, tensor_amax, WINO_GAIN_BT);
     const int cq = C >> 2;
-    const int64_t id = (int64_t)xcd_remap(blockIdx.x, gridDim.x) * 256 + threadIdx.x;
-    const int64_t gt_raw = id / cq, t_last = g.tile_end[g.n - 1];
+    const int64_t id = (int64_t)(LIST ? (int)blockIdx.x : xcd_remap(blockIdx.x, gridDim.x)) * 256 + threadIdx.x;
+    const int64_t slot = id / cq, t_last = g.tile_end[g.n - 1];
+    int64_t gt_raw = slot;
+    if constexpr (LIST) {
+        const int nu_raw = *n_units, nu_max = (int)(Tpad >> 4);
+        const int64_t rows = 16 * (int64_t)(nu_raw < 0 ? 0 : (nu_raw < nu_max ? nu_raw : nu_max));
+        if ((id - threadIdx.x) >= rows * cq) return;
+        gt_raw = slot < rows ? (int64_t)units[slot >> 4] * 16 + (slot & 15) - t0 : t_last;
+        if (gt_raw < 0) gt_raw = t_last;
+    }
     const int64_t gt = gt_raw < t_last ? gt_raw : t_last - 1;
-    const int c4 = (int)(id - gt_raw * cq) * 4;
+    const int c4 = (int)(id - slot * cq) * 4;
     int64_t tile;
     const int q = wino_locate(g, gt, tile);
     const float *x = g.src[0];
@@ -93,6 +105,14 @@
         if (gt_raw < t_last && c4 == 0) row_amax[t0 + gt] = rn_amax_word_of_exp(e_img, WINO_GAIN_BT);
     }
     if (gt_raw >= t_last) return;
+    if constexpr (LIST) {
+        if (flags[t0 + gt] == 0) {
+            float *vb0 = V + (t0 + gt) * C + c4;
+#pragma unroll
+            for (int p = 0; p < 36; ++p) st_stream(vb0 + (int64_t)p * Tpad * C, f4(0.f));
+            return;
+        }
+    }
     float4 t[6][6];
 #pragma unroll
     for (int j = 0; j < 6; ++j) {
@@ -122,15 +142,25 @@
     }
 }
 
-template <bool PBITS, bool PADD, bool FLAGS = false>
+template <bool PBITS, bool PADD, bool FLAGS = false, bool LIST = false>
 __global__ __launch_bounds__(256, 2) void wino_out_kernel(const WinoTable g, const float *__restrict__ M, int Cout, int64_t t0,
                                                        int64_t Tpad, const float *__restrict__ scale,
                                                        const float *__restrict__ shift, int mask_mode, int act, int64_t y_bs,
                                                        const unsigned char *__restrict__ fin = nullptr,
-                                                       unsigned char *__restrict__ fout = nullptr) {
+                                                       unsigned char *__restrict__ fout = nullptr,
+                                                       const int *__restrict__ tiles = nullptr,
+                                                       const int *__restrict__ n_tiles = nullptr) {
     const int cq = Cout >> 2;
     const int64_t id = (int64_t)blockIdx.x * 256 + threadIdx.x;
-    const int64_t gt = id / cq;
+    const int64_t slot = id / cq;
+    int64_t gt = slot;
+    if constexpr (LIST) {
+        const int nt_raw = *n_tiles;
+        const int64_t nt = nt_raw < 0 ? 0 : (nt_raw < Tpad ? nt_raw : Tpad);
+        if ((id - threadIdx.x) >= nt * cq) return;
+        gt = slot < nt ? (int64_t)tiles[slot] - t0 : g.tile_end[g.n - 1];
+        if (gt < 0) gt = g.tile_end[g.n - 1];
+    }
     float am = 0.f;
     unsigned *yam = nullptr;
     int n_img = 0;
@@ -138,7 +168,7 @@
     do {
     if (gt >= g.tile_end[g.n - 1]) break;
     live = true;
-    const int c4 = (int)(id - gt * cq) * 4;
+    const int c4 = (int)(id - slot * cq) * 4;
     int64_t tile;
     const int q = wino_locate(g, gt, tile);
     float *y = g.dst[0];
@@ -541,8 +571,27 @@
     if (dy_form && row_amax != nullptr) return RN_EINVAL;
     if (dy_form) hipLaunchKernelGGL(wino_dy_kernel, grid, dim3(256), 0, (hipStream_t)stream, t, V, C, tile_offset, Tpad,
                                     reinterpret_cast<unsigned *>(tensor_amax));
-    else hipLaunchKernelGGL(wino_in_kernel, grid, dim3(256), 0, (hipStream_t)stream, t, V, C, tile_offset, Tpad,
-                            reinterpret_cast<unsigned *>(row_amax), reinterpret_cast<unsigned *>(tensor_amax));
+    else hipLaunchKernelGGL(wino_in_kernel<false>, grid, dim3(256), 0, (hipStream_t)stream, t, V, C, tile_offset, Tpad,
+                            reinterpret_cast<unsigned *>(row_amax), reinterpret_cast<unsigned *>(tensor_amax),
+                            (const unsigned char *)nullptr, (const int *)nullptr, (const int *)nullptr);
+    RN_LAUNCH_CHECK();
+    return RN_OK;
+}
+
+extern "C" int rn_wino_input_group_lists(const rn_wino_group *g, float *V, int C, int64_t tile_offset, int64_t Tpad, void *row_amax,
+                                         void *tensor_amax, const void *flags, const void *units, const void *n_units, void *stream) {
+    WinoTable t;
+    const int rc = wino_table(g, t);
+    if (rc) return rc;
+    if (!V || C <= 0 || (C & 3) || tile_offset < 0 || tile_offset + t.tile_end[t.n - 1] > Tpad) return RN_EINVAL;
+    if (!flags || !units || !n_units || ((uintptr_t)flags & 15) || ((uintptr_t)units & 3) || ((uintptr_t)n_units & 3) || (Tpad & 15)) return RN_EINVAL;
+    for (int i = 0; i < t.n; ++i)
+        if (!t.src[i]) return RN_EINVAL;
+    const dim3 grid(rn_blocks(t.tile_end[t.n - 1] * (C >> 2), 256));
+    hipLaunchKernelGGL(wino_in_kernel<true>, grid, dim3(256), 0, (hipStream_t)stream, t, V, C, tile_offset, Tpad,
+                       reinterpret_cast<unsigned *>(row_amax), reinterpret_cast<unsigned *>(tensor_amax),
+                       reinterpret_cast<const unsigned char *>(flags), reinterpret_cast<const int *>(units),
+                       reinterpret_cast<const int *>(n_units));
     RN_LAUNCH_CHECK();
     return RN_OK;
 }
@@ -602,9 +651,9 @@
     return rn_wino_input_both_group_flags(g, V, Z, C, tile_offset, Tpad, v_row_amax, z_tensor_amax, nullptr, stream);
 }
 
-extern "C" int rn_wino_output_group_flags(const rn_wino_group *g, const float *M, int Cout, int64_t tile_offset, int64_t Tpad,
+extern "C" int rn_wino_output_group_lists(const rn_wino_group *g, const float *M, int Cout, int64_t tile_offset, int64_t Tpad,
                                           const float *scale, const float *shift, int mask_mode, int act, int64_t y_batch_stride,
-                                          const void *flags_in, void *flags_out, void *stream) {
+                                          const void *flags_in, void *flags_out, const void *tiles, const void *n_tiles, void *stream) {
     WinoTable t;
     const int rc = wino_table(g, t);
     if (rc) return rc;
@@ -622,6 +671,21 @@
     const dim3 grid(rn_blocks(t.tile_end[t.n - 1] * (Cout >> 2), 256));
     const unsigned char *fin = reinterpret_cast<const unsigned char *>(flags_in);
     unsigned char *fout = reinterpret_cast<unsigned char *>(flags_out);
+    if ((tiles != nullptr) != (n_tiles != nullptr)) return RN_EINVAL;
+    if (tiles != nullptr) {
+        if (fin == nullptr || (((uintptr_t)tiles | (uintptr_t)n_tiles) & 3)) return RN_EINVAL;
+        for (int i = 0; i < t.n; ++i)
+            if (t.add[i] != nullptr || t.sign[i] != nullptr || t.amax[i] != nullptr) return RN_EINVAL;
+        const int *tl = reinterpret_cast<const int *>(tiles), *ntl = reinterpret_cast<const int *>(n_tiles);
+        if ((mask_mode & RN_MASK_BITS) != 0)
+            hipLaunchKernelGGL((wino_out_kernel<true, false, true, true>), grid, dim3(256), 0, (hipStream_t)stream, t, M, Cout, tile_offset, Tpad,
+                               scale, shift, mask_mode, act, y_batch_stride, fin, fout, tl, ntl);
+        else
+            hipLaunchKernelGGL((wino_out_kernel<false, false, true, true>), grid, dim3(256), 0, (hipStream_t)stream, t, M, Cout, tile_offset, Tpad,
+                               scale, shift, mask_mode, act, y_batch_stride, fin, fout, tl, ntl);
+        RN_LAUNCH_CHECK();
+        return RN_OK;
+    }
 #define RN_WINO_OUT(B, A, F) hipLaunchKernelGGL((wino_out_kernel<B, A, F>), grid, dim3(256), 0, (hipStream_t)stream, t, M, Cout, tile_offset, Tpad, \
                                                 scale, shift, mask_mode, act, y_batch_stride, fin, fout)
     if (fin != nullptr || fout != nullptr) {
@@ -637,6 +701,12 @@
     RN_LAUNCH_CHECK();
     return RN_OK;
 }
+extern "C" int rn_wino_output_group_flags(const rn_wino_group *g, const float *M, int Cout, int64_t tile_offset, int64_t Tpad,
+                                          const float *scale, const float *shift, int mask_mode, int act, int64_t y_batch_stride,
+                                          const void *flags_in, void *flags_out, void *stream) {
+    return rn_wino_output_group_lists(g, M, Cout, tile_offset, Tpad, scale, shift, mask_mode, act, y_batch_stride, flags_in, flags_out,
+                                      nullptr, nullptr, stream);
+}
 extern "C" int rn_wino_output_group(const rn_wino_group *g, const float *M, int Cout, int64_t tile_offset, int64_t Tpad,
                                     const float *scale, const float *shift, int mask_mode, int act, int64_t y_batch_stride,
                                     void *stream) {
diff --git a/3d-playground_amd/csrc/focal_loss.hip b/3d-playground_amd/csrc/focal_loss.hip
--- a/3d-playground_amd/csrc/focal_loss.hip
+++ b/3d-playground_amd/csrc/focal_loss.hip
@@ -840,6 +840,74 @@
     return RN_OK;
 }
 
+struct LabelFlagLevels {
+    int n, na;
+    int H[RN_MAX_GROUP], W[RN_MAX_GROUP];
+    int64_t pix_end[RN_MAX_GROUP];
+    int64_t tile_base[RN_MAX_GROUP];
+};
+template <bool DIR>
+__global__ __launch_bounds__(NTHR) void label_flags_kernel(const float4 *__restrict__ anchors, const float *__restrict__ ann, int N,
+                                                           const LabelFlagLevels lv, unsigned char *__restrict__ flags) {
+    constexpr int COLS = DIR ? 27 : 5;
+    __shared__ LabelLds L;
+    const int j = blockIdx.y;
+    load_labels<DIR>(ann + (int64_t)j * N * COLS, N, L);
+    const int64_t p = (int64_t)blockIdx.x * NTHR + threadIdx.x;
+    if (p >= lv.pix_end[lv.n - 1] || L.count == 0) return;
+    bool pos = false;
+    for (int a = 0; a < lv.na; ++a) {
+        float best; int arg;
+        match_anchor(anchors[p * lv.na + a], L, best, arg);
+        if (best >= 0.5f) pos = true;
+    }
+    if (!pos) return;
+    int H = lv.H[0], W = lv.W[0];
+    int64_t first = 0, base = lv.tile_base[0];
+#pragma unroll
+    for (int i = 1; i < RN_MAX_GROUP; ++i)
+        if (i < lv.n && p >= lv.pix_end[i - 1]) { H = lv.H[i]; W = lv.W[i]; first = lv.pix_end[i - 1]; base = lv.tile_base[i]; }
+    const int local = (int)(p - first);
+    const int h = local / W, w = local - h * W;
+    const int TH = (H + 3) >> 2, TW = (W + 3) >> 2, th = h >> 2, tw = w >> 2;
+    unsigned char *f = flags + base + (int64_t)j * TH * TW;
+#pragma unroll
+    for (int a = -1; a <= 1; ++a)
+#pragma unroll
+        for (int b = -1; b <= 1; ++b) {
+            const bool row_ok = a == 0 || (a < 0 ? ((h & 3) == 0 && th > 0) : ((h & 3) == 3 && th + 1 < TH));
+            const bool col_ok = b == 0 || (b < 0 ? ((w & 3) == 0 && tw > 0) : ((w & 3) == 3 && tw + 1 < TW));
+            if (row_ok && col_ok) f[(th + a) * TW + (tw + b)] = 1;
+        }
+}
+
+extern "C" int rn_label_tile_flags(const float *anchors, const float *ann, int B, int64_t A, int N, int directional, int n_levels,
+                                   const int *H, const int *W, int anchors_per_pixel, void *flags, int64_t flags_len, void *stream) {
+    const int rc = check_args(B, A, 1, N);
+    if (rc) return rc;
+    if (!anchors || !flags || !H || !W || n_levels < 1 || n_levels > RN_MAX_GROUP || anchors_per_pixel < 1 || (N > 0 && !ann)) return RN_EINVAL;
+    LabelFlagLevels lv = {};
+    lv.n = n_levels; lv.na = anchors_per_pixel;
+    int64_t pix = 0, tiles = 0;
+    for (int i = 0; i < RN_MAX_GROUP; ++i) {
+        const int k = i < n_levels ? i : n_levels - 1;
+        if (H[k] <= 0 || W[k] <= 0) return RN_EINVAL;
+        lv.H[i] = H[k]; lv.W[i] = W[k];
+        lv.tile_base[i] = tiles;
+        if (i < n_levels) { pix += (int64_t)H[k] * W[k]; tiles += (int64_t)B * ((H[k] + 3) / 4) * ((W[k] + 3) / 4); }
+        lv.pix_end[i] = pix;
+    }
+    if (pix * anchors_per_pixel != A || tiles > flags_len) return RN_EINVAL;
+    const dim3 grid((unsigned)((pix + NTHR - 1) / NTHR), B), block(NTHR);
+    const float4 *anc = reinterpret_cast<const float4 *>(anchors);
+    if (directional)
+        hipLaunchKernelGGL(label_flags_kernel<true>, grid, block, 0, (hipStream_t)stream, anc, ann, N, lv, reinterpret_cast<unsigned char *>(flags));
+    else
+        hipLaunchKernelGGL(label_flags_kernel<false>, grid, block, 0, (hipStream_t)stream, anc, ann, N, lv, reinterpret_cast<unsigned char *>(flags));
+    RN_LAUNCH_CHECK();
+    return RN_OK;
+}
+
 __global__ void pairwise_iou_kernel(const float4 *__restrict__ a, const float4 *__restrict__ b, float *__restrict__ out,
                                     int64_t A, int N) {
     const int64_t i = (int64_t)blockIdx.x * 256 + threadIdx.x;
diff --git a/3d-playground_amd/retinanet_mi355x/_hip.py b/3d-playground_amd/retinanet_mi355x/_hip.py
--- a/3d-playground_amd/retinanet_mi355x/_hip.py
+++ b/3d-playground_amd/retinanet_mi355x/_hip.py
@@ -192,6 +192,9 @@
     "rn_wino_input_both_group_flags": (c_i32, [ctypes.POINTER(WinoGroup), c_vp, c_vp, c_i32, c_i64, c_i64, c_vp, c_vp, c_vp, c_vp]),
     "rn_tile_lists": (c_i32, [c_vp, c_i64, c_vp, c_vp, c_vp, c_vp, c_vp]),
     "rn_wino_input_both_group_lists": (c_i32, [ctypes.POINTER(WinoGroup), c_vp, c_vp, c_i32, c_i64, c_i64, c_vp, c_vp, c_vp, c_vp, c_vp, c_vp]),
+    "rn_wino_output_group_lists": (c_i32, [ctypes.POINTER(WinoGroup), c_vp, c_i32, c_i64, c_i64, c_vp, c_vp, c_i32, c_i32, c_i64, c_vp, c_vp, c_vp, c_vp, c_vp]),
+    "rn_wino_input_group_lists": (c_i32, [ctypes.POINTER(WinoGroup), c_vp, c_i32, c_i64, c_i64, c_vp, c_vp, c_vp, c_vp, c_vp, c_vp]),
+    "rn_label_tile_flags": (c_i32, [c_vp, c_vp, c_i32, c_i64, c_i32, c_i32, c_i32, ctypes.POINTER(c_i32), ctypes.POINTER(c_i32), c_i32, c_vp, c_i64, c_vp]),
     "rn_wino_output_group_flags": (c_i32, [ctypes.POINTER(WinoGroup), c_vp, c_i32, c_i64, c_i64, c_vp, c_vp, c_i32, c_i32, c_i64, c_vp, c_vp, c_vp]),
     "rn_wino_output_group": (c_i32, [ctypes.POINTER(WinoGroup), c_vp, c_i32, c_i64, c_i64, c_vp, c_vp, c_i32, c_i32, c_i64, c_vp]),
     "rn_conv_igemm_grouped": (c_i32, [ctypes.POINTER(ConvGroup), c_vp, c_vp, c_vp, c_vp]),
diff --git a/3d-playground_amd/retinanet_mi355x/conv.py b/3d-playground_amd/retinanet_mi355x/conv.py
--- a/3d-playground_amd/retinanet_mi355x/conv.py
+++ b/3d-playground_amd/retinanet_mi355x/conv.py
@@ -375,8 +375,9 @@
     return g
 
 
-def _wino_transform_in(xs, V, C, Tpad, dy_form, want_rows=False, want_tensor=False):
-    lib = _hip.load()
+def _wino_transform_in(xs, V, C, Tpad, dy_form, want_rows=False, want_tensor=False, lists=None):
+    lib = _hip.load()
+    assert lists is None or (dy_form == 0 and len(xs) <= _hip.RN_MAX_GROUP)
     off = 0
     am = want_amax() and (want_rows or want_tensor)
     rows = torch.zeros(Tpad, dtype=torch.int32, device=V.device) if am and want_rows else None
@@ -386,6 +387,11 @@
         t = sum(x.shape[0] * ((x.shape[1] + 3) // 4) * ((x.shape[2] + 3) // 4) for x in part)
         g = _wino_group(part, srcs=part, amaxs=[amax_words(x) for x in part] if am else None)
         nb = 4.0 * (sum(x.numel() for x in part) + 36 * t * C)
+        if lists is not None:
+            _hip.check(prof.timed("wino_input", nb, lambda: lib.rn_wino_input_group_lists(
+                ctypes.byref(g), V.data_ptr(), C, off, Tpad, _hip.ptr(rows), _hip.ptr(tword), lists.flags.data_ptr(), lists.units.data_ptr(),
+                lists.counts.data_ptr() + 4, _hip.stream())), "rn_wino_input_group_lists")
+            break
         _hip.check(prof.timed("wino_input", nb, lambda: lib.rn_wino_input_group(
             ctypes.byref(g), V.data_ptr(), C, off, Tpad, dy_form, _hip.ptr(rows), _hip.ptr(tword), _hip.stream())), "rn_wino_input_group")
         off += t
@@ -434,13 +440,25 @@
     return tl
 
 
+def label_tile_flags(anchors, ann, B, A, hws, anchors_per_pixel, directional, flags):
+    lib = _hip.load()
+    assert flags.dtype == torch.uint8 and flags.is_contiguous() and anchors.dtype == torch.float32 and anchors.is_contiguous()
+    assert anchors.numel() == 4 * A and (ann.numel() == 0 or (ann.dtype == torch.float32 and ann.is_contiguous() and ann.shape[0] == B))
+    n = len(hws)
+    H = (ctypes.c_int * n)(*[int(h) for h, _ in hws])
+    W = (ctypes.c_int * n)(*[int(w) for _, w in hws])
+    _hip.check(lib.rn_label_tile_flags(anchors.data_ptr(), _hip.ptr(ann) if ann.numel() else None, B, A, ann.shape[1], int(bool(directional)), n,
+                                       H, W, anchors_per_pixel, flags.data_ptr(), flags.numel(), _hip.stream()), "rn_label_tile_flags")
+    return flags
+
+
 def wino_flags_ok(T, C, cout):
     lib = _hip.load()
     return bool(get_fp32_mfma() != "native" and lib.rn_get_option(OPT_WGRAD_ONCE) and C > 64 and cout > 64 and T < 32000)
 
 
 def wino_conv_group(xs, U, outs=None, scale=None, shift=None, act=ACT_NONE, adds=None, masks=None, mask_mode=2,
-                    flops=0.0, keep_v=False, y_batch_stride=0, V_in=None, V_ready=None, sign=False, flags_out=None):
+                    flops=0.0, keep_v=False, y_batch_stride=0, V_in=None, V_ready=None, sign=False, flags_out=None, read_lists=None):
     lib = _hip.load()
     dev = xs[0].device
     C = xs[0].shape[3]
@@ -448,6 +466,8 @@
     tiles = [x.shape[0] * ((x.shape[1] + 3) // 4) * ((x.shape[2] + 3) // 4) for x in xs]
     T = sum(tiles)
     Tpad = wino_tpad(T)
+    keep_t = keep_v if isinstance(keep_v, torch.Tensor) else None
+    keep_v = bool(keep_t is not None or keep_v)
     V, M = _wino_workspace(dev, 0 if keep_v else 36 * Tpad * C, 36 * Tpad * cout)
     shapes = tuple(tuple(x.shape) for x in xs)
     reuse = keep_v and V_in is not None and V_in[1] == shapes and V_in[0].numel() == 36 * Tpad * C
@@ -456,6 +476,9 @@
         V, reuse = V_ready[0], True
     elif reuse:
         V = V_in[0]
+    elif keep_t is not None:
+        assert keep_t.dtype == torch.float32 and keep_t.numel() == 36 * Tpad * C and keep_t.is_contiguous()
+        V = keep_t
     elif keep_v:
         V = torch.empty(36 * Tpad * C, dtype=torch.float32, device=dev)
     assert all(x.is_contiguous() for x in xs)
@@ -464,9 +487,15 @@
         src = V_ready if ready else V_in
         v_am = src[2] if len(src) > 2 and src[2] is not None else (None, None)
     else:
-        v_am = _wino_transform_in(xs, V, C, Tpad, 0, want_rows=True, want_tensor=keep_v)
+        v_am = _wino_transform_in(xs, V, C, Tpad, 0, want_rows=True, want_tensor=keep_v, lists=read_lists)
     flags = V_ready[3] if ready and len(V_ready) > 3 else None
     lists = V_ready[4] if ready and len(V_ready) > 4 else None
+    if read_lists is not None:
+        if ready or adds is not None or sign or flags_out is not None or len(xs) > _hip.RN_MAX_GROUP:
+            raise ValueError("wino_conv_group(read_lists=...): a plain forward of one group")
+        assert read_lists.flags.numel() >= Tpad
+        flags, lists = read_lists.flags, read_lists
+    partial_v = read_lists is not None and not reuse
     if flags_out is not None:
         assert flags_out.dtype == torch.uint8 and flags_out.numel() >= Tpad and len(xs) <= _hip.RN_MAX_GROUP
     Vv = V[:36 * Tpad * C].view(36, 1, Tpad, C)
@@ -494,7 +523,12 @@
         nops = 1 + (pa is not None and pa[0] is not None) + (1.0 / 32 if mbits else 1.0) * has_mask + (1.0 / 32 if signs[0] is not None else 0.0)
         nb = 4.0 * (36 * t * cout + nops * sum(x.shape[0] * x.shape[1] * x.shape[2] for x in part) * cout)
         mm = (mask_mode | (MASK_BITS if mbits else 0)) if has_mask else 0
-        if flags is not None or flags_out is not None:
+        if read_lists is not None:
+            assert yams is None and all(s_ is None for s_ in signs)
+            _hip.check(prof.timed("wino_output", nb, lambda: lib.rn_wino_output_group_lists(
+                ctypes.byref(g), M.data_ptr(), cout, off, Tpad, _hip.ptr(scale), _hip.ptr(shift), mm, act, y_batch_stride, flags.data_ptr(),
+                None, lists.tiles.data_ptr(), lists.counts.data_ptr(), _hip.stream())), "rn_wino_output_group_lists")
+        elif flags is not None or flags_out is not None:
             _hip.check(prof.timed("wino_output", nb, lambda: lib.rn_wino_output_group_flags(
                 ctypes.byref(g), M.data_ptr(), cout, off, Tpad, _hip.ptr(scale), _hip.ptr(shift), mm,
                 act, y_batch_stride, _hip.ptr(flags), _hip.ptr(flags_out), _hip.stream())), "rn_wino_output_group_flags")
@@ -506,6 +540,8 @@
             for o, w_ in zip(outs[sl], yams):
                 amax_attach(o, w_)
         off += t
+    if keep_v and partial_v:
+        return outs, (V, tuple(tuple(x.shape) for x in xs), v_am, flags)
     return (outs, (V, tuple(tuple(x.shape) for x in xs), v_am)) if keep_v else outs
 
 
@@ -542,6 +578,9 @@
     Tpad = wino_tpad(T)
     have_v = V is not None and V[1] == tuple(tuple(x.shape) for x in xs) and V[0].numel() == 36 * Tpad * C
     v_tw = V[2][1] if have_v and len(V) > 2 and V[2] is not None else None
+    v_partial = V[3] if have_v and len(V) > 3 else None
+    if V is not None and len(V) > 3 and V[3] is not None and not have_v:
+        raise RuntimeError("a partial Winograd transform was kept for other inputs than these")
     V = V[0] if have_v else None
     Vw, Z = _wino_workspace(dev, 0 if have_v else 36 * Tpad * C, 36 * Tpad * cout)
     if not have_v:
@@ -568,6 +607,8 @@
             lists = None
         elif not isinstance(lists, TileLists):
             lists = tile_lists(flags, Tpad, buf=None if lists is True else lists)
+        if v_partial is not None and flags is None:
+            raise RuntimeError("a partial Winograd transform of the forward (read_lists) reached a reduction that reads every row")
         if lists is not None:
             assert lists.flags.data_ptr() == flags.data_ptr()
             _hip.check(prof.timed("wino_input", nb, lambda: lib.rn_wino_input_both_group_lists(
@@ -580,6 +621,8 @@
         v_dy = (Vd, tuple(tuple(t.shape) for t in gs), (vd_rows, None)) + ((flags,) if flags is not None else ()) \
             + ((lists,) if lists is not None else ())
     else:
+        if v_partial is not None:
+            raise RuntimeError("a partial Winograd transform of the forward (read_lists) reached a reduction that reads every row")
         flags = None
         z_tw = _wino_transform_in(gs, Z, cout, Tpad, 1, want_tensor=True)[1]
     am = (z_tw, v_tw) if (want_amax() and z_tw is not None and v_tw is not None) else (None, None)
diff --git a/3d-playground_amd/retinanet_mi355x/engine.py b/3d-playground_amd/retinanet_mi355x/engine.py
--- a/3d-playground_amd/retinanet_mi355x/engine.py
+++ b/3d-playground_amd/retinanet_mi355x/engine.py
@@ -8,6 +8,7 @@
 FUSE_DY = os.environ.get("RN_WINO_FUSE_DY", "1") != "0"
 SPARSE_REG = os.environ.get("RN_SPARSE_REG", "1") != "0"
 SPARSE_REG_LISTS = os.environ.get("RN_SPARSE_REG_LISTS", "1") != "0"
+SPARSE_REG_FWD = os.environ.get("RN_SPARSE_REG_FWD", "1") != "0"
 GROUPED_WGRAD_BF16 = os.environ.get("RN_GROUPED_WGRAD_BF16", "1") != "0"
 S2_SHORTCUT_COMPACT = os.environ.get("RN_S2_SHORTCUT_COMPACT", "1") != "0"
 STEM_BF16_PRODUCTS = os.environ.get("RN_STEM_BF16_PRODUCTS", "1") != "0"
@@ -201,9 +202,12 @@
                                  add=add, add_mode=add_mode, add_hw=add_hw, act=act, y_batch_stride=y_batch_stride,
                                  out_scale=self.out_scale, flops=self.flops(x.shape[0], Ho, Wo))
 
-    def fwd_group(self, xs, act=cv.ACT_NONE, outs=None, y_batch_stride=None, wino=False, shared_v=None):
+    def fwd_group(self, xs, act=cv.ACT_NONE, outs=None, y_batch_stride=None, wino=False, shared_v=None, read_lists=None):
         s = self.spec
         mode = self.mode()
+        if read_lists is not None and not (mode == "fp32" and (wino or self.wino_active) and self.wino_ok and y_batch_stride is not None
+                                           and shared_v is None):
+            raise RuntimeError("fwd_group(read_lists=...): this layer does not take the Winograd path")
         if self.fp8:
             xs = [_AS[mode](x) for x in xs]
         if mode == "fp8":
@@ -241,7 +245,7 @@
             fl = sum(self.flops(x.shape[0], x.shape[1], x.shape[2]) for x in xs)
             r = cv.wino_conv_group(xs, self.wino_weights(0), outs=outs, scale=self.scale, shift=self.shift, act=act, flops=fl,
                                    keep_v=self.keep_v, y_batch_stride=y_batch_stride or 0, V_in=shared_v if self.keep_v else None,
-                                   sign=self.sign and act == cv.ACT_RELU)
+                                   sign=self.sign and act == cv.ACT_RELU, read_lists=read_lists)
             ys, self.saved_v = r if self.keep_v else (r, None)
             return ys
         probs, ys, fl = [], [], 0.0
@@ -806,7 +810,7 @@
                 on.append(n)
         return on
 
-    def forward(self, P, img, save, x4=None):
+    def forward(self, P, img, save, x4=None, labels=None):
         Ls = self.layers
         if save and os.environ.get("RN_BATCHED_PREP", "1") != "0":
             self._prepare_training(P)
@@ -928,7 +932,12 @@
                 for cnt in counts:
                     views.append(out.view(B, -1)[:, off * width:])
                     off += cnt
-                Ls[prefix + ".output"].fwd_group(ts, act=act, outs=views, y_batch_stride=A * width)
+                Lout = Ls[prefix + ".output"]
+                rl = None
+                if ti == 0 and labels is not None and save and self._sparse_reg_ok(Lout, B, pyramid, x4.device):
+                    rl = self._label_lists(labels, B, A, pyramid, x4.device)
+                    S["reg_v_partial"] = True
+                Lout.fwd_group(ts, act=act, outs=views, y_batch_stride=A * width, read_lists=rl)
             if save:
                 S["towers"][prefix] = [[acts[i][li] for i in range(4)] for li in range(5)]
         if side is not None:
@@ -940,11 +949,33 @@
             L.saved_v = None
         return reg, cls, S
 
+    def _sparse_reg_ok(self, Lout, B, pyramid, device, fwd=True):
+        T = sum(B * ((f.shape[1] + 3) // 4) * ((f.shape[2] + 3) // 4) for f in pyramid)
+        ok = SPARSE_REG and self.use_wino and not self.bwd16 and not self.bf16 and not self.fp8 and device.type == "cuda" \
+            and Lout.wino_active and Lout.wino_ok and FUSE_DY and len(pyramid) <= _hip.RN_MAX_GROUP \
+            and cv.wino_flags_ok(T, Lout.spec.cin, Lout.spec.cout) and Lout.cout_pad == Lout.spec.cout
+        return bool(ok and (SPARSE_REG_FWD or not fwd))
+
+    def _label_lists(self, labels, B, A, pyramid, device):
+        ann, anc, directional = labels
+        T = sum(B * ((f.shape[1] + 3) // 4) * ((f.shape[2] + 3) // 4) for f in pyramid)
+        Tpad = cv.wino_tpad(T)
+        buf = getattr(self, "_label_flags", None)
+        if buf is None or buf.numel() != Tpad or buf.device != device:
+            buf = self._label_flags = torch.empty(Tpad, dtype=torch.uint8, device=device)
+            self._label_list_buf = torch.empty(cv.tile_lists_numel(Tpad), dtype=torch.int32, device=device)
+        buf.zero_()
+        cv.label_tile_flags(anc, ann, B, A, [(f.shape[1], f.shape[2]) for f in pyramid], arch.NUM_ANCHORS, directional, buf)
+        return cv.tile_lists(buf, Tpad, buf=self._label_list_buf)
+
     def backward(self, S, dreg, dcls, cls):
         Ls = self.layers
         grads = {}
         sparse_reg = SPARSE_REG and self.use_wino and not self.bwd16 and not self.bf16 and not self.fp8 and dreg.is_cuda
         reg_tiles = [dreg.shape[0] * ((f.shape[1] + 3) // 4) * ((f.shape[2] + 3) // 4) for f in S["pyramid"]]
+        if S.get("reg_v_partial") and not self._sparse_reg_ok(Ls["regressionModel.output"], dreg.shape[0], S["pyramid"], dreg.device, fwd=False):
+            raise RuntimeError("the forward kept the regression head's input transform on the label-flagged tiles only, and this backward "
+                               "would reduce over all of them: the sparse switches changed between the two")
         self._zero_grad_accumulators(dreg.device, cv.wino_tpad(sum(reg_tiles)) if sparse_reg else 0, 5 if sparse_reg else 0)
         for L in Ls.values():
             L.saved_v = L.dy_v = None
diff --git a/3d-playground_amd/retinanet_mi355x/modules.py b/3d-playground_amd/retinanet_mi355x/modules.py
--- a/3d-playground_amd/retinanet_mi355x/modules.py
+++ b/3d-playground_amd/retinanet_mi355x/modules.py
@@ -134,10 +134,10 @@
     def forward(ctx, net, img, ann, *params):
         eng = net._engine
         P = net._tensor_dict()
-        reg, cls, S = eng.forward(P, img, save=True)
         anc = eng.anchors(img.shape[2], img.shape[3], img.device)
         lib = _hip.load()
         ann_c = _hip.f32c(ann)
+        reg, cls, S = eng.forward(P, img, save=True, labels=(ann_c, anc, bool(net.directional)))
         B, A, C = cls.shape
         ws = ops.focal_workspace(B, A, img.device)
         losses = torch.empty(3, dtype=torch.float32, device=img.device)
diff --git a/include/retinanet_mi355x.h b/include/retinanet_mi355x.h
--- a/include/retinanet_mi355x.h
+++ b/include/retinanet_mi355x.h
@@ -362,6 +362,13 @@
 int rn_wino_input_both_group_lists(const rn_wino_group *g, float *V, float *Z, int C, int64_t tile_offset, int64_t Tpad,
                                    void *v_row_amax, void *z_tensor_amax, const void *flags, const void *units, const void *n_units,
                                    void *stream);
+int rn_wino_output_group_lists(const rn_wino_group *g, const float *M, int Cout, int64_t tile_offset, int64_t Tpad,
+                               const float *scale, const float *shift, int mask_mode, int act, int64_t y_batch_stride,
+                               const void *flags_in, void *flags_out, const void *tiles, const void *n_tiles, void *stream);
+int rn_wino_input_group_lists(const rn_wino_group *g, float *V, int C, int64_t tile_offset, int64_t Tpad, void *row_amax,
+                              void *tensor_amax, const void *flags, const void *units, const void *n_units, void *stream);
+int rn_label_tile_flags(const float *anchors, const float *ann, int B, int64_t A, int N, int directional, int n_levels,
+                        const int *H, const int *W, int anchors_per_pixel, void *flags, int64_t flags_len, void *stream);
 int rn_wino_input(const float *x, float *V, int N, int H, int W, int C, int64_t tile_offset, int64_t Tpad, void *stream);
 int rn_wino_output(const float *M, float *y, int N, int H, int W, int Cout, int64_t tile_offset, int64_t Tpad,
                    const float *scale, const float *shift, const float *add, const float *mask, int mask_mode, int act,
```

Result: no change. 135.8 images/sec, median of 6 (+0.7%).
